# jurgisp/pydreamer

Measured on AMD Instinct MI355X. Metric: grad-steps/sec (world-model+AC) at B=50,T=50,H=15, 64×64 obs, 1/2/4/8 GPU, higher is better.
Workload: dtype f32; 1 GPU; atari-literal: defaults+atari, batch_size 50, batch_length 50, imag_horizon 15, deter_dim 600, stoch 32x32, hidden 1000, cnn_depth 48, action_dim 18, fp32; fwd + 4 bwd + clip + 4 AdamW per step; replay resident in HBM; global_batch=50, batch_length=50, imag_horizon=15, parallelism=dp1 (batch-sharded [50])

## Files before the change

### include/dreamer_hip.h

```cpp
#ifndef DREAMER_HIP_H
#define DREAMER_HIP_H

#include <stddef.h>
#include <stdint.h>

#ifdef __cplusplus
extern "C" {
#endif

#define DM_OK 0
#define DM_E_SHAPE (-1)
#define DM_E_WORKSPACE (-2)
#define DM_E_HIP (-3)
#define DM_E_DEVICE (-4)
#define DM_E_NULL (-5)

#define DM_MAX_MLP_LAYERS 8

typedef struct dm_shape {
  int32_t T, B, I;
  int32_t H;
  int32_t D, Hd;
  int32_t S, C;
  int32_t E;
// ... 45 lines not shown
int dm_rssm_lds_status(void);
int dm_rssm_lds_status_ack(void);
int dm_rssm_lds_gave_up(void);
int dm_rssm_lds_prof(unsigned long long* out16, int reset);

int dm_ln_elu_fwd(int rows, int n, const float* x, int ldx, const float* gamma, const float* beta, float eps,
                  float* y, int ldy, float* stats, void* stream);
int dm_ln_elu_bwd(int rows, int n, const float* x, int ldx, const float* y, int ldy, const float* stats,
                  const float* gamma, const float* dy, int lddy, float* dx, int lddx,
                  float* dgamma, float* dbeta, void* ws, size_t ws_bytes, void* stream);
int dm_colsum(int rows, int n, const float* x, int ld, float* out, void* ws, size_t ws_bytes, void* stream);

int dm_gru_gates_fwd(int rows, int D, const float* gi, const float* gh, const float* h_in, int ldh,
                     float* h_out, int ldo, void* stream);
int dm_gru_gates_bwd(int rows, int D, const float* gi, const float* gh, const float* h_in, int ldh,
                     const float* dh_out, int lddh, float* dgi, float* dgh, float* dh_in, int lddi, void* stream);

int dm_sample_onehot(int rows, int groups, int C, const float* logits, int ldl, const float* u,
                     const int32_t* forced_idx, float* onehot, int ldo, int32_t* idx, void* stream);

int dm_kl_balance_fwd(int rows, int S, int C, const float* post, const float* prior,
                      float* kl, float* ent_post, float* ent_prior, void* stream);
int dm_kl_balance_bwd(int rows, int S, int C, const float* post, const float* prior,
                      float scale_post, float scale_prior, float* dpost, float* dprior, void* stream);
int dm_kl_free_fwd(int rows, int S, int C, const float* post, const float* prior, float free, float* kl, float* kl_clip,
                   float* closed, float* ent_post, float* ent_prior, void* stream);
int dm_kl_free_bwd(int rows, int S, int C, const float* post, const float* prior, const float* closed, float scale_post,
                   float scale_prior, float* dpost, float* dprior, void* stream);
int dm_st_softmax_bwd(int rows, int groups, int C, const float* logits, int ldl, const float* dz, int lddz,
                      float* dlogits, int lddl, int accum, void* stream);

int dm_kl_sampled_fwd(int rows, int S, int C, const float* post, const float* prior, const int32_t* idx, float* out, void* stream);
int dm_kl_sampled_bwd(int rows, int S, int C, const float* post, const float* prior, const int32_t* idx, float scale,
                      const float* row_w, float* dpost, float* dprior, void* stream);
int dm_kl_sampled_gauss_fwd(int rows, int S, const float* post, const float* prior, const float* z, int ldz, float* out,
                            void* stream);
int dm_kl_sampled_gauss_bwd(int rows, int S, const float* post, const float* prior, const float* z, int ldz, float scale,
                            const float* row_w, float* dpost, float* dprior, float* dz, int lddz, void* stream);
int dm_reduce_i(int TB, int I, int W, const float* x, int mode, float* out, float* w_out, void* stream);
int dm_combine_rows(int count, int64_t n, const float* const* x, const float* w, float* out, void* stream);
int dm_scale_rows(int64_t rows, int n, float* x, int ldx, const float* w, float scale, void* stream);

int dm_mask_rows(int rows, int n, const float* x, int ldx, const uint8_t* reset, float* y, int ldy, void* stream);

int dm_im2col_s2(int n, int hb, int wb, int c, int k, const float* big, int big_nchw, float* col, void* stream);
#define DM_C2I_ELU 1
int dm_col2im_s2(int n, int hb, int wb, int c, int k, const float* col, const float* bias, int flags,
                 const float* elu_ref, float* big, void* stream);

typedef struct dm_mlp_params {
  const float* w[DM_MAX_MLP_LAYERS + 1];
  const float* b[DM_MAX_MLP_LAYERS + 1];
  const float* ln_g[DM_MAX_MLP_LAYERS];
  const float* ln_b[DM_MAX_MLP_LAYERS];
  int32_t precision;
  int32_t reserved_;
} dm_mlp_params;
typedef struct dm_mlp_grads {
  float* w[DM_MAX_MLP_LAYERS + 1];
  float* b[DM_MAX_MLP_LAYERS + 1];
  float* ln_g[DM_MAX_MLP_LAYERS];
  float* ln_b[DM_MAX_MLP_LAYERS];
} dm_mlp_grads;
size_t dm_mlp_acts_floats(int rows, int hidden, int layers);
size_t dm_mlp_ws_floats(int rows, int hidden, int layers);
int dm_mlp_plan_query(int which, int rows, int in_dim, int hidden, int layers, int out_dim, int ldx, int sparse_cols,
                      int base_align, int normed, int precision, int has_acts, int has_wpack, int has_add0, int has_sample,
                      size_t ws_bytes, int32_t out[8]);
int dm_mlp_head_fwd(int rows, int in_dim, int hidden, int layers, int out_dim,
                    const float* x, int ldx, const dm_mlp_params* p, float* acts, float* out,
                    void* ws, size_t ws_bytes, void* stream);
int dm_mlp_head_fwd_sparse(int rows, int in_dim, int sparse_cols, int hidden, int layers, int out_dim,
                           const float* x, int ldx, const dm_mlp_params* p, float* acts, float* out,
                           void* ws, size_t ws_bytes, void* stream);
int dm_mlp_head_fwd_rows(int rows_total, int row0, int rows, int in_dim, int sparse_cols, int hidden, int layers, int out_dim,
                         const float* x, int ldx, const dm_mlp_params* p, float* acts, float* out,
                         void* ws, size_t ws_bytes, void* stream);

int dm_mlp_head_bwd(int rows, int in_dim, int hidden, int layers, int out_dim,
                    const float* x, int ldx, const dm_mlp_params* p, const float* acts, const float* dout,
                    const dm_mlp_grads* g, float* dx, int lddx, int dx_accum,
                    void* ws, size_t ws_bytes, void* stream);

int dm_head_loss(int kind, int rows, const float* out, const float* target, float scale, float loss_const,
                 float* loss, float* dout, float* mean_out, void* stream);

int dm_head_loss_normal_nd(int rows, int V, const float* out, const float* target, float scale, float loss_const,
                           float* loss, float* dout, float* mean_out, void* stream);

int dm_head_loss_catsup(int rows, int I, int K, const float* logits, int ld, const float* support, const float* target, float scale,
                        float* loss, float* dlogits, float* mean_out, int32_t* bin, void* stream);

int dm_disag_reward(int K, int rows, int D, const float* means, int64_t head_stride, int ld, float scale, float* reward,
                    void* stream);
int dm_ensemble_mse(int K, int rows, int D, const float* means, int64_t head_stride, int ld, const float* target, int ldt,
                    const uint8_t* skip, float scale, float* loss, float* dmeans, void* stream);

int dm_cat_target_index(int rows, int C, int cells, const float* onehot, int32_t* idx, void* stream);
int dm_cat_image_loss(int rows, int I, int C, int cells, const float* logits, int ld, const int32_t* target, float* loss,
                      float* dlogits, void* stream);
int dm_cat_image_pred(int groups, int I, int C, int cells, const float* logits, int ld, const int32_t* target,
                      const int32_t* seen, float* logp, float* acc, float* acc_seen, void* stream);
int dm_cat_concat_rows(int rows, int I, int F, int E, const float* x, int ldx, const float* extra, float* out, void* stream);

int dm_dense_image_rows(int rows, int C, int cells, const float* image_f32, const int32_t* class_i32, const float* reward,
                        const float* terminal, float* out, int ldo, void* stream);
int dm_elu_rows_fwd(int rows, int n, const float* x, int ldx, float* y, int ldy, void* stream);
int dm_elu_rows_bwd(int rows, int n, const float* y, int ldy, const float* dy, int lddy, float* dx, int lddx, void* stream);
int dm_cat_image_loss_mix(int rows, int I, int C, int cells, const float* logits, int ld, const int32_t* target, float min_prob,
                          float* loss, float* dlogits, void* stream);

size_t dm_goals_stats_ws_floats(int rows, int G);
int dm_goals_stats(int rows, int G, const float* goals, const float* pred, const float* visage, float* out, void* ws,
                   size_t ws_bytes, void* stream);

int dm_preprocess_image_u8(int64_t n, int hw, int c, const uint8_t* src, float* dst, void* stream);

typedef struct dm_conv_params { const float* w[5]; const float* b[5]; } dm_conv_params;
typedef struct dm_conv_grads { float* w[5]; float* b[5]; } dm_conv_grads;
size_t dm_conv_encoder_acts_floats(const dm_shape* shp);
int dm_conv_encoder_fwd(const dm_shape* shp, const float* image , const dm_conv_params* p,
                        float* acts, float* embed , void* ws, size_t ws_bytes, void* stream);
int dm_conv_encoder_bwd(const dm_shape* shp, const float* image, const dm_conv_params* p, const float* acts,
                        const float* dembed, const dm_conv_grads* g, void* ws, size_t ws_bytes, void* stream);
int dm_conv_encoder_fwd_planes(const dm_shape* shp, const float* image, const dm_conv_params* p, const float* reward,
                               const float* terminal, float* acts, float* embed, int ld_embed, void* ws, size_t ws_bytes,
                               void* stream);
int dm_conv_encoder_bwd_planes(const dm_shape* shp, const float* image, const dm_conv_params* p, const float* reward,
                               const float* terminal, const float* acts, const float* dembed, int ld_dembed,
                               const dm_conv_grads* g, void* ws, size_t ws_bytes, void* stream);

size_t dm_conv_decoder_acts_floats(const dm_shape* shp);
size_t dm_conv_decoder_pred_offset(const dm_shape* shp);
int dm_conv_decoder_mse_fwd(const dm_shape* shp, const float* feat, int ldf, const float* target,
                            const dm_conv_params* p, float* acts, float* loss_image, float* image_rec ,
                            void* ws, size_t ws_bytes, void* stream);
int dm_conv_decoder_mse_bwd_rows(const dm_shape* shp, const float* feat, int ldf, const float* target,
                                 const dm_conv_params* p, const float* acts, float scale, const float* row_scale,
                                 const dm_conv_grads* g, float* dfeat, int lddf, void* ws, size_t ws_bytes, void* stream);
int dm_conv_decoder_mse_bwd(const dm_shape* shp, const float* feat, int ldf, const float* target,
                            const dm_conv_params* p, const float* acts, float scale,
                            const dm_conv_grads* g, float* dfeat, int lddf, void* ws, size_t ws_bytes, void* stream);

enum {
  DM_RSSM_Z_W = 0, DM_RSSM_Z_B, DM_RSSM_A_W, DM_RSSM_IN_G, DM_RSSM_IN_B,
  DM_RSSM_GRU_WIH, DM_RSSM_GRU_WHH, DM_RSSM_GRU_BIH, DM_RSSM_GRU_BHH,
  DM_RSSM_PRIOR_H_W, DM_RSSM_PRIOR_H_B, DM_RSSM_PRIOR_G, DM_RSSM_PRIOR_B, DM_RSSM_PRIOR_W, DM_RSSM_PRIOR_OB,
  DM_RSSM_POST_H_W, DM_RSSM_POST_H_B, DM_RSSM_POST_E_W, DM_RSSM_POST_G, DM_RSSM_POST_B, DM_RSSM_POST_W, DM_RSSM_POST_OB,
  DM_RSSM_GRU_LN_G0, DM_RSSM_GRU_LN_B0, DM_RSSM_GRU_LN_G1, DM_RSSM_GRU_LN_B1, DM_RSSM_GRU_LN_G2, DM_RSSM_GRU_LN_B2,
  DM_RSSM_GRU_L1_WIH, DM_RSSM_GRU_L1_WHH, DM_RSSM_GRU_L1_BIH, DM_RSSM_GRU_L1_BHH,
  DM_RSSM_GRU_L2_WIH, DM_RSSM_GRU_L2_WHH, DM_RSSM_GRU_L2_BIH, DM_RSSM_GRU_L2_BHH,
  DM_RSSM_GRU_L3_WIH, DM_RSSM_GRU_L3_WHH, DM_RSSM_GRU_L3_BIH, DM_RSSM_GRU_L3_BHH,
  DM_RSSM_GRU_L1_LN_G0, DM_RSSM_GRU_L1_LN_B0, DM_RSSM_GRU_L1_LN_G1, DM_RSSM_GRU_L1_LN_B1, DM_RSSM_GRU_L1_LN_G2, DM_RSSM_GRU_L1_LN_B2,
  DM_RSSM_GRU_L2_LN_G0, DM_RSSM_GRU_L2_LN_B0, DM_RSSM_GRU_L2_LN_G1, DM_RSSM_GRU_L2_LN_B1, DM_RSSM_GRU_L2_LN_G2, DM_RSSM_GRU_L2_LN_B2,
  DM_RSSM_GRU_L3_LN_G0, DM_RSSM_GRU_L3_LN_B0, DM_RSSM_GRU_L3_LN_G1, DM_RSSM_GRU_L3_LN_B1, DM_RSSM_GRU_L3_LN_G2, DM_RSSM_GRU_L3_LN_B2,
  DM_RSSM_NPARAMS
};
typedef struct dm_rssm_params { const float* p[DM_RSSM_NPARAMS]; } dm_rssm_params;
typedef struct dm_rssm_grads { float* p[DM_RSSM_NPARAMS]; } dm_rssm_grads;
size_t dm_rssm_acts_floats(const dm_shape* shp);
int dm_rssm_sequence_fwd(const dm_shape* shp, const float* embed, const float* action, const uint8_t* reset,
                         const float* h0, const float* z0, const float* u, const int32_t* forced_idx,
                         const dm_rssm_params* p, float* acts, float* feat, float* post, float* prior, int32_t* idx,
                         void* ws, size_t ws_bytes, void* stream);
int dm_rssm_sequence_bwd(const dm_shape* shp, const float* embed, const float* action, const uint8_t* reset,
                         const dm_rssm_params* p, const float* acts, const float* feat, const float* post,
                         float* dfeat, float* dpost, float* dprior,
                         const dm_rssm_grads* g, float* dembed, void* ws, size_t ws_bytes, void* stream);

#define DM_SCHED_FWD_FUSE_LN 1
#define DM_SCHED_FWD_FUSE_SAMPLE 2
#define DM_SCHED_FWD_FRAG 4
#define DM_SCHED_FWD_WZT 8
#define DM_SCHED_FWD_PSYNC 16
#define DM_SCHED_BWD_FUSE_B 1
#define DM_SCHED_BWD_FOLD 2
#define DM_SCHED_BWD_FOLD_SM 4
#define DM_SCHED_BWD_FRAG 8
#define DM_SCHED_BWD_NCHUNK_SHIFT 8
#define DM_SCHED_BWD_NCHUNK_MASK (15 << DM_SCHED_BWD_NCHUNK_SHIFT)
#define DM_SCHED_ROLL_WZT 1
#define DM_SCHED_ROLL_WAT 2
#define DM_SCHED_ROLL_ACTOR_WPACK 4
#define DM_SCHED_ROLL_ACTOR_ADD0 8
#define DM_SCHED_ROLL_FUSE_ACT 16
#define DM_SCHED_ROLL_TW_ON 32
int dm_rssm_last_schedule(int which);

typedef struct dm_gru_params { const float* w_ih; const float* w_hh; const float* b_ih; const float* b_hh; } dm_gru_params;
typedef struct dm_gru_grads { float* w_ih; float* w_hh; float* b_ih; float* b_hh; } dm_gru_grads;
size_t dm_gru_sequence_acts_floats(int T, int B, int In, int D);
size_t dm_gru_sequence_ws_bytes(int T, int B, int In, int D);
int dm_gru_sequence_fwd(int T, int B, int In, int D, const float* x, int ldx, const float* h0, const uint8_t* reset0,
                        const dm_gru_params* p, float* acts, float* H, int ldh, void* ws, size_t ws_bytes, void* stream);
int dm_gru_sequence_bwd(int T, int B, int In, int D, const float* x, int ldx, const dm_gru_params* p, const float* acts,
                        const float* H, int ldh, const float* dH, int lddh, const dm_gru_grads* g, float* dx, int lddx,
                        void* ws, size_t ws_bytes, void* stream);
int dm_gru_sequence_last_schedule(void);
int dm_gru_sequence_fuse_enable(int on);

int dm_dream_rollout_marks(int n, const int* steps, void* const* events);

int dm_dream_rollout(const dm_shape* shp, int M, const float* start, const dm_rssm_params* cell,
                     const dm_mlp_params* actor, const float* u_act, const float* u_prior,
                     float* feats, float* actions, int32_t* act_idx, float* actor_acts, float* actor_logits,
                     void* ws, size_t ws_bytes, void* stream);

int dm_gae_losses(int H, int M, float gamma, float lambda, const float* reward, const float* terminal,
                  const float* value_t, float* advantage, float* advantage_gae, float* value_target, float* weight,
                  void* stream);
int dm_actor_loss(int rows, int A, const float* logits, const int32_t* act_idx, const float* adv_gae,
                  const float* weight, float ent_w, float scale, float* loss, float* entropy, float* dlogits, void* stream);
int dm_sample_continuous(int kind, int rows, int A, const float* params, const float* eps, float* action, void* stream);
int dm_actor_loss_continuous(int kind, int rows, int A, const float* params, const float* actions, const float* adv_gae,
                             const float* weight, float ent_w, float scale, float* loss, float* entropy, float* dparams,
                             void* stream);
size_t dm_policy_draw_ws_floats(int rows);
int dm_policy_draw(int kind, int rows, int A, const float* params, int ldp, const float* noise, const float* value, float* action,
                   int lda, int32_t* act_idx, float* log_prob, float* entropy, float* stats, void* ws, size_t ws_bytes,
                   void* stream);
int dm_policy_draw_mode(int kind, int mode, float amount, int rows, int A, const float* params, int ldp, const float* noise,
                        const float* noise2, const float* value, float* action, int lda, int32_t* act_idx, float* log_prob,
                        float* entropy, float* stats, void* ws, size_t ws_bytes, void* stream);
int dm_cem_draw(int kind, int B, int J, int Hp, int A, const float* prop, const float* noise, float* actions, int32_t* act_idx,
                void* stream);
int dm_cem_update(int kind, int B, int J, int K, int Hp, int A, float gamma, const float* reward, const float* terminal,
                  const float* value, const float* actions, const int32_t* act_idx, const float* prop_in, float alpha, float floor,
                  float* prop_out, float* ret, int32_t* elite, float* first_action, float* stats, void* stream);
int dm_twohot_decode(int rows, int K, const float* logits, int ld, const float* bins, float* value, void* stream);
int dm_twohot_loss(int rows, int rows_total, int K, const float* logits, int ld, const float* bins, const float* target,
                   const float* weight, float scale, float* loss, float* dlogits, float* value, void* stream);
int dm_return_norm(int n, const float* x, float q_lo, float q_hi, float decay, float limit, int update, float* state, float* out,
                   float* adv, int n_adv, void* stream);
int dm_twohot_head_loss(int rows, int I, int K, const float* logits, int ld, const float* bins, const float* target, float scale,
                        float* loss, float* dlogits, float* mean, void* stream);
int dm_critic_loss(int rows, const float* value, const float* value_target, const float* weight, float scale,
                   float* loss, float* dvalue, void* stream);

typedef struct dm_reduce_item {
  const float* x; int64_t n; float scale;
  int32_t mode;
  const float* center;
} dm_reduce_item;
int dm_multi_sum(int count, const dm_reduce_item* items , float* out, void* stream);
int dm_combine(int count, const float* x, const float* w, float* out, void* stream);

int dm_multi_tensor_norm_clip(const float* grad, int64_t n, float max_norm, float* norm_out,
                              void* ws, size_t ws_bytes, void* stream);
int dm_scale_inplace(float* x, int64_t n, const float* coef, void* stream);
int dm_adamw_step(float* param, const float* grad, float* exp_avg, float* exp_avg_sq, int64_t n,
                  float lr, float beta1, float beta2, float eps, float weight_decay, int step,
                  const float* clip_coef, void* stream);
int dm_copy_params(float* dst, const float* src, int64_t n, void* stream);
int dm_mlp_chain_min_rows(int rows);
int dm_rollout_fuse_act_enable(int on);
int dm_prof_begin(int max_launches);
int dm_prof_end(double* out, int nkinds);
int dm_prof_rows(double* rows, int max_rows);
#define DM_REPLAY_MAX_FIELDS 16
typedef struct dm_replay_field {
  void* dst; int64_t row_bytes; int32_t is_reset; int32_t reserved_;
} dm_replay_field;
int dm_replay_gather(int T, int B, int nfields, const dm_replay_field* fields , const int32_t* pieces,
                     const void* const* src, void* stream);
int dm_axpby(int64_t n, float a, const float* x, float b, float* y, void* stream);

int dm_metric_accum(int n, const float* vals, const uint8_t* rules, double* sum, double* maxv, int64_t* count, void* stream);
int dm_batch_stats(int n, const float* reward, const uint8_t* reset, const float* terminal, float* out4, void* stream);
int dm_masked_mean(int T, int B, const float* x, int ldx, int take_rows, const uint8_t* col_keep, int skip_nan, float* out,
                   void* stream);
int dm_export_image_u8(int T, int B, int take_b, int C, int H, int W, const float* src, uint8_t* dst, void* stream);

#ifdef __cplusplus
}
#endif
#endif
```

### pydreamer_amd/csrc/common.h

```cpp
#pragma once
#include <hip/hip_runtime.h>
#include <stdint.h>
#include <stddef.h>
#include "dreamer_hip.h"

int dm_fail(int code, const char* fmt, ...);

#define DM_MAX_DEVICES 16

#define DM_LAUNCH_CHECK()                                                                      \
  do {                                                                                         \
    hipError_t e__ = hipGetLastError();                                                        \
    if (e__ != hipSuccess) return dm_fail(DM_E_HIP, "%s:%d: %s", __FILE__, __LINE__, hipGetErrorString(e__)); \
  } while (0)

#define DM_TRY(expr)                 \
  do {                               \
    int rc__ = (expr);               \
    if (rc__ != DM_OK) return rc__;  \
  } while (0)

#define DM_REQUIRE(cond, code, ...)                     \
  do {                                                  \
    if (!(cond)) return dm_fail(code, __VA_ARGS__);     \
// ... 134 lines not shown
                            const float* gamma, const float* dy, int lddy, float* dx, int lddx, hipStream_t st);
int dm_ln_elu_bwd_params_launch(int rows, int n, const float* x, int ldx, const float* y, int ldy, const float* stats,
                                const float* dy, int lddy, float* dgamma, float* dbeta, void* ws, size_t ws_bytes,
                                hipStream_t st);
int dm_gru_norm_fwd_launch(int kind, int rows, int D, const float* gi, const float* gh, const float* h_in, int ldh,
                           const float* const* ln_g, const float* const* ln_b, float* h_out, int ldo, float* gs, float* gst,
                           float* h_next, const uint8_t* next_reset, hipStream_t st, int ldg = 0, int ldst = 0, int ldn = 0);
int dm_gru_norm_bwd_launch(int kind, int rows, int D, const float* gh, const float* h_in, int ldh, const float* gs,
                           const float* gst, const float* const* ln_g, const float* const* ln_b, const float* dh_out, int lddh,
                           float* dgi, float* dgh, float* dg, float* dh_in, int lddi, const uint8_t* row_zero, hipStream_t st,
                           int ldg = 0, int ldst = 0);
int dm_gru_norm_param_grads_launch(int kind, int rows, int D, const float* gs, const float* gst, const float* dg, float* dgam,
                                   float* dbet, hipStream_t st, int ldg = 0, int ldst = 0);
int dm_gru_gates_fwd_launch(int rows, int D, const float* gi, const float* gh, const float* h_in, int ldh, float* h_out,
                            int ldo, float* h_next, const uint8_t* next_reset, float* h_frag, float* h_next_frag,
                            hipStream_t st, int ldg = 0, int ldn = 0);
int dm_gru_gates_bwd_launch(int rows, int D, const float* gi, const float* gh, const float* h_in, int ldh,
                            const float* dh_out, int lddh, float* dgi, float* dgh, float* dh_in, int lddi, int accum,
                            const uint8_t* row_zero, hipStream_t st, int ldg = 0);
int dm_sample_onehot_launch(int rows, int groups, int C, const float* logits, int ldl, const float* u,
                            const int32_t* forced, float* onehot, int ldo, int32_t* idx, float* z_next,
                            const uint8_t* next_reset, hipStream_t st);
int dm_gauss_sample_bwd_launch(int rows, int S, const float* par, int ldp, const float* z, int ldz, const float* dz,
                               int lddz, float* dpar, int lddp, int accum, hipStream_t st);
int dm_kl_fwd_launch(int rows, int S, int C, const float* post, const float* prior, float* kl, float* ep, float* eq,
                     hipStream_t st);
int dm_kl_bwd_launch(int rows, int S, int C, const float* post, const float* prior, float sp, float sq, float* dpost,
                     float* dprior, hipStream_t st);
int dm_st_softmax_bwd_launch(int rows, int groups, int C, const float* logits, int ldl, const float* dz, int lddz,
                             float* dlogits, int lddl, int accum, hipStream_t st);
int dm_mask_rows_launch(int rows, int n, const float* x, int ldx, const uint8_t* reset, float* y, int ldy, hipStream_t st);
int dm_mask_rows2_launch(int rows, int n1, const float* x1, int ldx1, float* y1, int ldy1, int n2, const float* x2,
                         int ldx2, float* y2, int ldy2, const uint8_t* reset, hipStream_t st);
int dm_sample_continuous_launch(int kind, int rows, int A, const float* params, const float* eps, float* action,
                                hipStream_t st);
int dm_mul_elu_grad_launch(size_t n, const float* dy, const float* yact, float* out, hipStream_t st);

int dm_im2col_s2_launch(int n, int hb, int wb, int c, int k, const float* big, int big_nchw, float* col, hipStream_t st);
int dm_col2im_s2_launch(int n, int hb, int wb, int c, int k, const float* col, const float* bias, int flags,
                        const float* elu_ref, float* big, hipStream_t st);
int dm_permute4_launch(const float* src, float* dst, int d0, int d1, int d2, int d3, int p0, int p1, int p2, int p3,
                       hipStream_t st);

bool dm_enc_l1_direct_ok(int ch, int d, int img);
int dm_enc_l1_fwd_launch(int frames, int d, int u8, const void* image, const float* w, const float* bias, float* wt, float* y,
                         unsigned short* y_h, hipStream_t st);
size_t dm_enc_l1_wgrad_part_floats(int frames, int d);
int dm_enc_l1_wgrad_launch(int frames, int d, int u8, const void* image, const float* G, float* part, float* dW, void* ws,
                           size_t ws_bytes, hipStream_t st);
int dm_enc_l1_fwd_planes_launch(int frames, int d, int u8, const void* image, const float* w5, const float* bias,
                                const float* reward, const float* terminal, float* wt, float* fb, float* y,
                                unsigned short* y_h, hipStream_t st);
size_t dm_enc_l1_planes_part_floats(int frames, int d);
int dm_enc_l1_planes_bwd_launch(int frames, int d, const float* G, const float* reward, const float* terminal,
                                const float* dw3, float* part, float* db, float* dW5, hipStream_t st);
bool dm_dec_l4_direct_ok(int ch, int d, int hs, int k);
size_t dm_dec_l4_w4_floats(int d);
int dm_dec_l4_fwd_launch(int frames, int d, const float* x, const float* w, const float* bias, float* w4, float* out,
                         hipStream_t st);
bool dm_dec_l4_bwd_direct_ok(int ch, int d, int hs, int k);
size_t dm_dec_l4_wp_floats(int d);
size_t dm_dec_l4_wgrad_part_floats(int frames, int d);
int dm_dec_l4_dgrad_launch(int frames, int d, const float* G4, const float* w, float* wp, const float* x3, float* dx,
                           unsigned short* dx_h, hipStream_t st);
int dm_dec_l4_wgrad_launch(int frames, int d, const float* G4, const float* x3, float* part, float* dW, void* ws,
                           size_t ws_bytes, hipStream_t st);

struct DmChainSample {
  const float* u;
  float* onehot;
  int ldo;
  int32_t* idx;
};
struct DmMlpFwd {
  int rows = 0, in_dim = 0, hidden = 0, layers = 0, out_dim = 0;
  const float* x = nullptr; int ldx = 0;
  const dm_mlp_params* p = nullptr;
  float* acts = nullptr; int acts_total_rows = 0, acts_row_off = 0;
  float* out = nullptr; int ldout = 0;
  int sparse_cols = 0;
  const float* wpack = nullptr;
  const float* add0 = nullptr;
  const DmChainSample* sample = nullptr;
};
enum { DM_MLP_PANEL = 0, DM_MLP_CHAIN = 1, DM_MLP_PER_LAYER = 2 };
int dm_mlp_fwd_launch(const DmMlpFwd& q, void* ws, size_t ws_bytes, hipStream_t st);
int dm_mlp_fwd_path(const DmMlpFwd& q, int* k0 = nullptr);

bool dm_panel_ok(int rows, int hidden);
int dm_panel_count(int rows);
int dm_panel_ln_fwd_launch(int rows, int hidden, int kin, const float* x, int ldx, const float* W, const float* b,
                           const float* gamma, const float* beta, float eps, float* xpre, float* stats, float* y,
                           const float* wout, const float* bout, float* out, int out_dim, int ldout, hipStream_t st,
                           const unsigned short* Wh = nullptr, int ldw = 0, const float* addm = nullptr);
int dm_panel_bf16_weights_launch(int count, const float* const* w, unsigned short* const* dst, const int* rows, const int* cols,
                                 int transpose, hipStream_t st);
int dm_panel_ln_bwd_launch(int rows, int hidden, int kup, const float* dup, int lddup, const float* W, const float* xpre,
                           const float* stats, const float* gamma, const float* beta, float* dx, float* colpart, float* wt,
                           hipStream_t st, const unsigned short* Wth = nullptr);
int dm_panel_colsum_final_launch(int count, const float* const* part, float* const* out, int n, int npanels, int pstride,
                                 hipStream_t st);

bool dm_mlp_chain_ok(int rows, int in_dim, int hidden, int layers, int out_dim, const float* x, int ldx,
                     const dm_mlp_params* p);
size_t dm_mlp_chain_pack_floats(int in_dim, int layers);
int dm_mlp_chain_pack_launch(int in_dim, int layers, const dm_mlp_params* p, float* wpack, hipStream_t st, int k0 = 0);
int dm_mlp_chain_fwd_launch(int rows, int in_dim, int layers, int out_dim, const float* x, int ldx, const dm_mlp_params* p,
                            float* const* xpre, float* const* stats, float* const* y, float* out, int ldout, const float* wpack,
                            hipStream_t st, int k0 = 0, const float* add0 = nullptr, const DmChainSample* sample = nullptr);
bool dm_mlp_chain_sparse_ok(int in_dim, int sparse_cols);

int dm_prof_slot_begin(int kind, double flops, double bytes, hipStream_t st);
void dm_prof_slot_end(int slot, hipStream_t st);
void dm_prof_slot_shape(int slot, int M, int N, int K, int nsplit, int flags);
extern "C" int dm_mlp_chain_min_rows(int rows);
bool dm_prof_active();

static const size_t DM_SPLITK_FLOATS = (size_t)16 * 1024 * 1024;
size_t dm_conv_ws_floats(const dm_shape* s, size_t parts[4] = nullptr);
size_t dm_rssm_ws_floats(const dm_shape* s, size_t parts[2] = nullptr);
size_t dm_rollout_ws_floats(const dm_shape* s);

typedef __bf16 bf16x8 __attribute__((ext_vector_type(8)));
typedef __bf16 bf16x2 __attribute__((ext_vector_type(2)));
typedef float dm_f32x2 __attribute__((ext_vector_type(2)));
__device__ __forceinline__ unsigned dm_pack_bf16x2(float lo, float hi) {
  const dm_f32x2 v = {lo, hi};
  return __builtin_bit_cast(unsigned, __builtin_convertvector(v, bf16x2));
}
__device__ __forceinline__ unsigned dm_f2bf(float x) { return dm_pack_bf16x2(x, 0.f) & 0xFFFFu; }
__device__ __forceinline__ uint2 dm_pack_bf16x4(float4 v) {
  return make_uint2(dm_pack_bf16x2(v.x, v.y), dm_pack_bf16x2(v.z, v.w));
}

__device__ __forceinline__ float dm_elu(float v) { return v > 0.f ? v : expm1f(v); }
__device__ __forceinline__ float dm_elu_grad_from_y(float y) { return y > 0.f ? 1.f : y + 1.f; }

__device__ __forceinline__ float dm_wave_sum(float v) {
#pragma unroll
  for (int off = 32; off > 0; off >>= 1) v += __shfl_xor(v, off, 64);
  return v;
}
__device__ __forceinline__ float dm_wave_max(float v) {
#pragma unroll
  for (int off = 32; off > 0; off >>= 1) v = fmaxf(v, __shfl_xor(v, off, 64));
  return v;
}
```

### pydreamer_amd/csrc/elementwise.hip

```cpp
#include "common.h"

template <bool CACHE>
__global__ void __launch_bounds__(256) ln_elu_fwd_kernel(int rows, int n, const float* __restrict__ x, int ldx,
                                                         const float* __restrict__ gamma, const float* __restrict__ beta,
                                                         float eps, float* __restrict__ y, int ldy, float* __restrict__ stats,
                                                         unsigned short* __restrict__ y_h) {
  const int row = blockIdx.x * 4 + (threadIdx.x >> 6);
  const int lane = threadIdx.x & 63;
  if (row >= rows) return;
  const float* xr = x + (size_t)row * ldx;
  unsigned short* yh = y_h ? y_h + (size_t)row * ldy : nullptr;
  float xc[16];
  float s = 0.f;
  if (CACHE) {
#pragma unroll
    for (int j = 0; j < 16; ++j) {
      const int c = lane + 64 * j;
      xc[j] = c < n ? xr[c] : 0.f;
      s += xc[j];
    }
  } else {
    for (int c = lane; c < n; c += 64) s += xr[c];
  }
  const float mean = dm_wave_sum(s) / (float)n;
// ... 566 lines not shown
      dgir[D + d] = ds_u; dghr[D + d] = ds_u;
    }
  }
}

__global__ void __launch_bounds__(256) gru_norm_param_grads_kernel(int kind, int rows, int D, const float* __restrict__ gs,
                                                                   const float* __restrict__ gst, const float* __restrict__ dg,
                                                                   float* __restrict__ dgam, float* __restrict__ dbet, int ldg,
                                                                   int ldst) {
  __shared__ float red[2][4][64];
  const int cx = threadIdx.x & 63, ry = threadIdx.x >> 6;
  const int col = blockIdx.x * 64 + cx;
  float a = 0.f, b = 0.f;
  if (col < 3 * D) {
    const int q = kind == 1 ? col / D : 0;
    for (int r = ry; r < rows; r += 4) {
      const float v = dg[(size_t)r * ldg + col];
      const float xh = (gs[(size_t)r * ldg + col] - gst[(size_t)r * ldst + 2 * q]) * gst[(size_t)r * ldst + 2 * q + 1];
      a += v * xh;
      b += v;
    }
  }
  red[0][ry][cx] = a; red[1][ry][cx] = b;
  __syncthreads();
  if (ry == 0 && col < 3 * D) {
    dgam[col] = (red[0][0][cx] + red[0][1][cx]) + (red[0][2][cx] + red[0][3][cx]);
    dbet[col] = (red[1][0][cx] + red[1][1][cx]) + (red[1][2][cx] + red[1][3][cx]);
  }
}

int dm_gru_norm_fwd_launch(int kind, int rows, int D, const float* gi, const float* gh, const float* h_in, int ldh,
                           const float* const* ln_g, const float* const* ln_b, float* h_out, int ldo, float* gs, float* gst,
                           float* h_next, const uint8_t* next_reset, hipStream_t st, int ldg, int ldst, int ldn) {
  if (rows <= 0) return DM_OK;
  if (ldg <= 0) ldg = 3 * D;
  if (ldst <= 0) ldst = 6;
  if (ldn <= 0) ldn = D;
  GruLnParams lp;
  for (int i = 0; i < 3; ++i) { lp.g[i] = ln_g[i]; lp.b[i] = ln_b[i]; }
  if (kind == 1)
    hipLaunchKernelGGL((gru_norm_fwd_kernel<1>), dim3(dm_cdiv(rows, 4)), dim3(256), 0, st, rows, D, gi, gh, h_in, ldh, lp, h_out,
                       ldo, gs, gst, h_next, next_reset, ldg, ldst, ldn);
  else
    hipLaunchKernelGGL((gru_norm_fwd_kernel<2>), dim3(dm_cdiv(rows, 4)), dim3(256), 0, st, rows, D, gi, gh, h_in, ldh, lp, h_out,
                       ldo, gs, gst, h_next, next_reset, ldg, ldst, ldn);
  DM_LAUNCH_CHECK();
  return DM_OK;
}
int dm_gru_norm_bwd_launch(int kind, int rows, int D, const float* gh, const float* h_in, int ldh, const float* gs,
                           const float* gst, const float* const* ln_g, const float* const* ln_b, const float* dh_out, int lddh,
                           float* dgi, float* dgh, float* dg, float* dh_in, int lddi, const uint8_t* row_zero, hipStream_t st,
                           int ldg, int ldst) {
  if (rows <= 0) return DM_OK;
  if (ldg <= 0) ldg = 3 * D;
  if (ldst <= 0) ldst = 6;
  GruLnParams lp;
  for (int i = 0; i < 3; ++i) { lp.g[i] = ln_g[i]; lp.b[i] = ln_b[i]; }
  if (kind == 1)
    hipLaunchKernelGGL((gru_norm_bwd_kernel<1>), dim3(dm_cdiv(rows, 4)), dim3(256), 0, st, rows, D, gh, h_in, ldh, gs, gst, lp,
                       dh_out, lddh, dgi, dgh, dg, dh_in, lddi, row_zero, ldg, ldst);
  else
    hipLaunchKernelGGL((gru_norm_bwd_kernel<2>), dim3(dm_cdiv(rows, 4)), dim3(256), 0, st, rows, D, gh, h_in, ldh, gs, gst, lp,
                       dh_out, lddh, dgi, dgh, dg, dh_in, lddi, row_zero, ldg, ldst);
  DM_LAUNCH_CHECK();
  return DM_OK;
}
int dm_gru_norm_param_grads_launch(int kind, int rows, int D, const float* gs, const float* gst, const float* dg, float* dgam,
                                   float* dbet, hipStream_t st, int ldg, int ldst) {
  if (ldg <= 0) ldg = 3 * D;
  if (ldst <= 0) ldst = 6;
  hipLaunchKernelGGL(gru_norm_param_grads_kernel, dim3(dm_cdiv(3 * D, 64)), dim3(256), 0, st, kind, rows, D, gs, gst, dg, dgam,
                     dbet, ldg, ldst);
  DM_LAUNCH_CHECK();
  return DM_OK;
}

static inline int ew_blocks(size_t total) {
  size_t b = (total + 255) / 256;
  if (b > 4096) b = 4096;
  if (b < 1) b = 1;
  return (int)b;
}

__global__ void __launch_bounds__(256) z_embed_kernel(int rows, int n, int S, int C, const int32_t* __restrict__ idx,
                                                      const uint8_t* __restrict__ row_zero, const float* __restrict__ Wt,
                                                      const float* __restrict__ bias, const float* __restrict__ add,
                                                      int ldadd, const int32_t* __restrict__ idx2,
                                                      const float* __restrict__ Wt2, float* __restrict__ x, int ldx,
                                                      float* __restrict__ x_frag,
                                                      const float* __restrict__ gamma, const float* __restrict__ beta,
                                                      float eps, float* __restrict__ y, int ldy,
                                                      unsigned short* __restrict__ y_h) {
  const int row = blockIdx.x * 4 + (threadIdx.x >> 6);
  const int lane = threadIdx.x & 63;
  if (row >= rows) return;
  float4 acc[4];
  bool in[4];
  int off[4];
#pragma unroll
  for (int j = 0; j < 4; ++j) {
    const int c = (lane + 64 * j) * 4;
    in[j] = c < n;
    off[j] = in[j] ? c : 0;
    acc[j] = bias ? *reinterpret_cast<const float4*>(bias + off[j]) : make_float4(0.f, 0.f, 0.f, 0.f);
  }
  if (add) {
#pragma unroll
    for (int j = 0; j < 4; ++j) {
      const float4 a = *reinterpret_cast<const float4*>(add + (size_t)row * ldadd + off[j]);
      acc[j].x += a.x; acc[j].y += a.y; acc[j].z += a.z; acc[j].w += a.w;
    }
  }
  if (idx2) {
    const float* wr = Wt2 + (size_t)idx2[row] * n;
#pragma unroll
    for (int j = 0; j < 4; ++j) {
      const float4 a = *reinterpret_cast<const float4*>(wr + off[j]);
      acc[j].x += a.x; acc[j].y += a.y; acc[j].z += a.z; acc[j].w += a.w;
    }
  }
  if (!(row_zero && row_zero[row])) {
    const int32_t* ir = idx + (size_t)row * S;
    for (int s0 = 0; s0 < S; s0 += 64) {
      const int mine = ir[min(s0 + lane, S - 1)];
      const int cnt = min(64, S - s0);
      int t = 0;
      for (; t + 8 <= cnt; t += 8) {
        float4 w[8][4];
#pragma unroll
        for (int u = 0; u < 8; ++u) {
          const float* wr = Wt + ((size_t)(s0 + t + u) * C + __shfl(mine, t + u, 64)) * n;
#pragma unroll
          for (int j = 0; j < 4; ++j) w[u][j] = *reinterpret_cast<const float4*>(wr + off[j]);
        }
        __builtin_amdgcn_sched_barrier(0);
#pragma unroll
        for (int u = 0; u < 8; ++u)
#pragma unroll
          for (int j = 0; j < 4; ++j) {
            acc[j].x += w[u][j].x; acc[j].y += w[u][j].y; acc[j].z += w[u][j].z; acc[j].w += w[u][j].w;
          }
      }
      for (; t < cnt; ++t) {
        const float* wr = Wt + ((size_t)(s0 + t) * C + __shfl(mine, t, 64)) * n;
#pragma unroll
        for (int j = 0; j < 4; ++j) {
          const float4 w = *reinterpret_cast<const float4*>(wr + off[j]);
          acc[j].x += w.x; acc[j].y += w.y; acc[j].z += w.z; acc[j].w += w.w;
        }
      }
    }
  }
#pragma unroll
  for (int j = 0; j < 4; ++j)
    if (in[j]) {
      const int c = (lane + 64 * j) * 4;
      if (x) *reinterpret_cast<float4*>(x + (size_t)row * ldx + c) = acc[j];
      if (x_frag) *reinterpret_cast<float4*>(x_frag + dm_frag_off(row, c)) = acc[j];
    }
  if (!y) return;
  if (!gamma) {
#pragma unroll
    for (int j = 0; j < 4; ++j)
      if (in[j]) {
        float4 o;
        o.x = dm_elu(acc[j].x); o.y = dm_elu(acc[j].y); o.z = dm_elu(acc[j].z); o.w = dm_elu(acc[j].w);
        *reinterpret_cast<float4*>(y + (size_t)row * ldy + (lane + 64 * j) * 4) = o;
      }
    return;
  }
  float s1 = 0.f;
#pragma unroll
  for (int j = 0; j < 4; ++j)
    if (in[j]) s1 += (acc[j].x + acc[j].y) + (acc[j].z + acc[j].w);
  const float mean = dm_wave_sum(s1) / (float)n;
  float s2 = 0.f;
#pragma unroll
  for (int j = 0; j < 4; ++j)
    if (in[j]) {
      const float dx = acc[j].x - mean, dy = acc[j].y - mean, dz = acc[j].z - mean, dw = acc[j].w - mean;
      s2 += (dx * dx + dy * dy) + (dz * dz + dw * dw);
    }
  const float rstd = 1.0f / sqrtf(dm_wave_sum(s2) / (float)n + eps);
#pragma unroll
  for (int j = 0; j < 4; ++j)
    if (in[j]) {
      const int c = (lane + 64 * j) * 4;
      const float4 g = *reinterpret_cast<const float4*>(gamma + c), b = *reinterpret_cast<const float4*>(beta + c);
      float4 o;
      o.x = dm_elu((acc[j].x - mean) * rstd * g.x + b.x);
      o.y = dm_elu((acc[j].y - mean) * rstd * g.y + b.y);
      o.z = dm_elu((acc[j].z - mean) * rstd * g.z + b.z);
      o.w = dm_elu((acc[j].w - mean) * rstd * g.w + b.w);
      *reinterpret_cast<float4*>(y + (size_t)row * ldy + c) = o;
      if (y_h) *reinterpret_cast<uint2*>(y_h + (size_t)row * ldy + c) = dm_pack_bf16x4(o);
    }
}
template <int NJ>
__global__ void __launch_bounds__(256) sparse_rows_kernel(int rows, int n, int Zc, const float* __restrict__ z, int ldz,
                                                          const float* __restrict__ Wt, float* __restrict__ x, int ldx) {
  const int row = blockIdx.x * 4 + (threadIdx.x >> 6);
  const int lane = threadIdx.x & 63;
  if (row >= rows) return;
  float4 acc[NJ];
  int off[NJ];
#pragma unroll
  for (int j = 0; j < NJ; ++j) {
    const int c = (lane + 64 * j) * 4;
    off[j] = c < n ? c : 0;
    acc[j] = make_float4(0.f, 0.f, 0.f, 0.f);
  }
  const float* zr = z + (size_t)row * ldz;
  for (int e0 = 0; e0 < Zc; e0 += 256) {
    float v[4];
    unsigned long long m[4];
#pragma unroll
    for (int u = 0; u < 4; ++u) v[u] = zr[min(e0 + 64 * u + lane, Zc - 1)];
#pragma unroll
    for (int u = 0; u < 4; ++u) m[u] = __ballot(e0 + 64 * u + lane < Zc && v[u] != 0.f);
#pragma unroll
    for (int u = 0; u < 4; ++u) {
      unsigned long long mm = m[u];
      while (mm) {
        const int b = __builtin_ctzll(mm);
        mm &= mm - 1;
        const float ze = __shfl(v[u], b, 64);
        const float* wr = Wt + (size_t)(e0 + 64 * u + b) * n;
#pragma unroll
        for (int j = 0; j < NJ; ++j) {
          const float4 w = *reinterpret_cast<const float4*>(wr + off[j]);
          acc[j].x += ze * w.x; acc[j].y += ze * w.y; acc[j].z += ze * w.z; acc[j].w += ze * w.w;
        }
      }
    }
  }
#pragma unroll
  for (int j = 0; j < NJ; ++j) {
    const int c = (lane + 64 * j) * 4;
    if (c < n) *reinterpret_cast<float4*>(x + (size_t)row * ldx + c) = acc[j];
  }
}
int dm_sparse_rows_launch(int rows, int n, int Zc, const float* z, int ldz, const float* Wt, float* x, int ldx,
                          hipStream_t st) {
  if (rows <= 0) return DM_OK;
  DM_REQUIRE(n >= 4 && n <= 1024 && (n & 3) == 0 && (ldx & 3) == 0 && Zc >= 1, DM_E_SHAPE, "sparse_rows: n=%d Zc=%d", n, Zc);
  const dim3 grid(dm_cdiv(rows, 4)), blk(256);
  if (n <= 256) hipLaunchKernelGGL((sparse_rows_kernel<1>), grid, blk, 0, st, rows, n, Zc, z, ldz, Wt, x, ldx);
  else if (n <= 512) hipLaunchKernelGGL((sparse_rows_kernel<2>), grid, blk, 0, st, rows, n, Zc, z, ldz, Wt, x, ldx);
  else hipLaunchKernelGGL((sparse_rows_kernel<4>), grid, blk, 0, st, rows, n, Zc, z, ldz, Wt, x, ldx);
  DM_LAUNCH_CHECK();
  return DM_OK;
}

bool dm_z_embed_ok(int n) { return n <= 1024 && (n & 3) == 0; }
__global__ void __launch_bounds__(256) z_embed_wide_kernel(int n, int S, int C, const int32_t* __restrict__ idx,
                                                           const uint8_t* __restrict__ row_zero, const float* __restrict__ Wt,
                                                           const float* __restrict__ bias, const float* __restrict__ add, int ldadd,
                                                           const int32_t* __restrict__ idx2, const float* __restrict__ Wt2,
                                                           float* __restrict__ x, int ldx, float* __restrict__ x_frag) {
  const int row = blockIdx.x;
  const int lane = threadIdx.x & 63;
  const int c = threadIdx.x * 4;
  const bool in = c < n;
  const int off = in ? c : 0;
  float4 acc = bias ? *reinterpret_cast<const float4*>(bias + off) : make_float4(0.f, 0.f, 0.f, 0.f);
  if (add) {
    const float4 a = *reinterpret_cast<const float4*>(add + (size_t)row * ldadd + off);
    acc.x += a.x; acc.y += a.y; acc.z += a.z; acc.w += a.w;
// ... 23 lines not shown

__global__ void __launch_bounds__(256) z_embed_wide_ln_kernel(int n, int S, int C, const int32_t* __restrict__ idx,
                                                              const uint8_t* __restrict__ row_zero, const float* __restrict__ Wt,
                                                              const float* __restrict__ bias, const float* __restrict__ add, int ldadd,
                                                              const int32_t* __restrict__ idx2, const float* __restrict__ Wt2,
                                                              float* __restrict__ x, int ldx, const float* __restrict__ gamma,
                                                              const float* __restrict__ beta, float eps, float* __restrict__ y, int ldy,
                                                              float* __restrict__ y_frag, float* __restrict__ stats) {
  __shared__ float red[8];
  const int row = blockIdx.x;
  const int lane = threadIdx.x & 63, wave = threadIdx.x >> 6;
  const int c = threadIdx.x * 4;
  const bool in = c < n;
  const int off = in ? c : 0;
  float4 acc = bias ? *reinterpret_cast<const float4*>(bias + off) : make_float4(0.f, 0.f, 0.f, 0.f);
  if (add) {
    const float4 a = *reinterpret_cast<const float4*>(add + (size_t)row * ldadd + off);
    acc.x += a.x; acc.y += a.y; acc.z += a.z; acc.w += a.w;
  }
  if (idx2) {
    const float4 a = *reinterpret_cast<const float4*>(Wt2 + (size_t)idx2[row] * n + off);
    acc.x += a.x; acc.y += a.y; acc.z += a.z; acc.w += a.w;
  }
  if (!(row_zero && row_zero[row])) {
    const int mine = idx[(size_t)row * S + min(lane, S - 1)];
    float4 w[32];
#pragma unroll
    for (int s = 0; s < 32; ++s) {
      const int sc = s < S ? s : S - 1;
      w[s] = *reinterpret_cast<const float4*>(Wt + ((size_t)sc * C + __shfl(mine, sc, 64)) * n + off);
    }
    __builtin_amdgcn_sched_barrier(0);
#pragma unroll
    for (int s = 0; s < 32; ++s)
      if (s < S) { acc.x += w[s].x; acc.y += w[s].y; acc.z += w[s].z; acc.w += w[s].w; }
  }
  if (in && x) *reinterpret_cast<float4*>(x + (size_t)row * ldx + c) = acc;
  const float s1 = dm_wave_sum(in ? (acc.x + acc.y) + (acc.z + acc.w) : 0.f);
  if (lane == 0) red[wave] = s1;
  __syncthreads();
  const float mean = ((red[0] + red[1]) + (red[2] + red[3])) / (float)n;
  const float4 d = make_float4(acc.x - mean, acc.y - mean, acc.z - mean, acc.w - mean);
  const float s2 = dm_wave_sum(in ? (d.x * d.x + d.y * d.y) + (d.z * d.z + d.w * d.w) : 0.f);
  if (lane == 0) red[4 + wave] = s2;
  __syncthreads();
  const float rstd = 1.0f / sqrtf(((red[4] + red[5]) + (red[6] + red[7])) / (float)n + eps);
  if (stats && threadIdx.x == 0) { stats[2 * (size_t)row] = mean; stats[2 * (size_t)row + 1] = rstd; }
  if (in) {
    const float4 ga = make_float4(gamma[c], gamma[c + 1], gamma[c + 2], gamma[c + 3]);
    const float4 be = make_float4(beta[c], beta[c + 1], beta[c + 2], beta[c + 3]);
    const float4 o = make_float4(dm_elu(d.x * rstd * ga.x + be.x), dm_elu(d.y * rstd * ga.y + be.y), dm_elu(d.z * rstd * ga.z + be.z),
                                 dm_elu(d.w * rstd * ga.w + be.w));
    if (y) *reinterpret_cast<float4*>(y + (size_t)row * ldy + c) = o;
    if (y_frag) *reinterpret_cast<float4*>(y_frag + dm_frag_off(row, c)) = o;
  }
}

int dm_z_embed_launch(int rows, int n, int S, int C, const int32_t* idx, const uint8_t* row_zero, const float* Wt,
                      const float* bias, const float* add, int ldadd, const int32_t* idx2, const float* Wt2, float* x, int ldx,
                      float* x_frag, const float* gamma, const float* beta, float eps, float* y, int ldy, hipStream_t st,
                      float* y_frag, float* stats) {
  if (rows <= 0) return DM_OK;
  DM_REQUIRE(!idx2 || Wt2, DM_E_NULL, "z_embed: second index list without its table");
  DM_REQUIRE(dm_z_embed_ok(n) && idx && Wt && (x || y), DM_E_SHAPE, "z_embed: n=%d needs n <= 1024, n %% 4 == 0", n);
  DM_REQUIRE((ldx & 3) == 0 && (ldy & 3) == 0 && (ldadd & 3) == 0, DM_E_SHAPE, "z_embed: leading dims must be multiples of 4");
  DM_REQUIRE(!x_frag || rows <= 64, DM_E_SHAPE, "z_embed: the fragment-major copy needs rows <= 64");
  DM_REQUIRE(!y || (gamma != nullptr) == (beta != nullptr), DM_E_NULL, "z_embed: LayerNorm gain without its bias");
  if (!y && x && rows <= 64 && S <= 32) {
    hipLaunchKernelGGL(z_embed_wide_kernel, dim3(rows), dim3(256), 0, st, n, S, C, idx, row_zero, Wt, bias, add, ldadd, idx2, Wt2, x,
                       ldx, x_frag);
    DM_LAUNCH_CHECK();
    return DM_OK;
  }
  if (y_frag) {
    DM_REQUIRE(y && gamma && beta && rows <= 64 && S <= 32 && !x_frag, DM_E_SHAPE,
               "z_embed: the row-per-workgroup LayerNorm form needs y, gamma / beta, rows <= 64, S <= 32");
    hipLaunchKernelGGL(z_embed_wide_ln_kernel, dim3(rows), dim3(256), 0, st, n, S, C, idx, row_zero, Wt, bias, add, ldadd, idx2, Wt2, x,
                       ldx, gamma, beta, eps, y, ldy, y_frag, stats);
    DM_LAUNCH_CHECK();
    return DM_OK;
  }
  unsigned short* y_h = (y && gamma) ? dm_twin_of(y, false) : nullptr;
  if (y_h) dm_twin_mark(y);
  hipLaunchKernelGGL(z_embed_kernel, dim3(dm_cdiv(rows, 4)), dim3(256), 0, st, rows, n, S, C, idx, row_zero, Wt, bias, add,
                     ldadd, idx2, Wt2, x, ldx, x_frag, gamma, beta, eps, y, ldy, y_h);
  DM_LAUNCH_CHECK();
  return DM_OK;
}

int dm_frag_pack_launch(int rows, int K, const float* X, int ldx, float* Xf, hipStream_t st) {
  DM_REQUIRE(rows >= 0 && rows <= 64 && K >= 1 && X && Xf, DM_E_SHAPE, "frag_pack: rows %d (<= 64), K %d", rows, K);
  if (rows == 0) return DM_OK;
  hipLaunchKernelGGL(frag_pack_kernel, dim3(ew_blocks((size_t)rows * K)), dim3(256), 0, st, rows, K, X, ldx, Xf);
  DM_LAUNCH_CHECK();
  return DM_OK;
}
int dm_gru_gates_fwd_launch(int rows, int D, const float* gi, const float* gh, const float* h_in, int ldh, float* h_out,
                            int ldo, float* h_next, const uint8_t* next_reset, float* h_frag, float* h_next_frag,
                            hipStream_t st, int ldg, int ldn) {
  if (rows <= 0) return DM_OK;
  DM_REQUIRE((!h_frag && !h_next_frag) || rows <= 64, DM_E_SHAPE, "gru_gates_fwd: fragment-major copies need rows <= 64");
  unsigned short* h_out_h = dm_twin_of(h_out, false);
  if (h_out_h) dm_twin_mark(h_out);
  hipLaunchKernelGGL(gru_gates_fwd_kernel, dim3(ew_blocks((size_t)rows * D)), dim3(256), 0, st, rows, D, gi, gh, h_in,
                     ldh, h_out, ldo, h_next, next_reset, h_frag, h_next_frag, ldg > 0 ? ldg : 3 * D, ldn > 0 ? ldn : D, h_out_h);
  DM_LAUNCH_CHECK();
  return DM_OK;
}
int dm_gru_gates_bwd_launch(int rows, int D, const float* gi, const float* gh, const float* h_in, int ldh,
                            const float* dh_out, int lddh, float* dgi, float* dgh, float* dh_in, int lddi, int accum,
                            const uint8_t* row_zero, hipStream_t st, int ldg) {
  if (rows <= 0) return DM_OK;
  hipLaunchKernelGGL(gru_gates_bwd_kernel, dim3(ew_blocks((size_t)rows * D)), dim3(256), 0, st, rows, D, gi, gh, h_in,
                     ldh, dh_out, lddh, dgi, dgh, dh_in, lddi, accum, row_zero, ldg > 0 ? ldg : 3 * D);
  DM_LAUNCH_CHECK();
  return DM_OK;
}
extern "C" int dm_gru_gates_fwd(int rows, int D, const float* gi, const float* gh, const float* h_in, int ldh,
                                float* h_out, int ldo, void* stream) {
  DM_REQUIRE(gi && gh && h_in && h_out, DM_E_NULL, "gru_gates_fwd: null pointer");
  return dm_gru_gates_fwd_launch(rows, D, gi, gh, h_in, ldh, h_out, ldo, nullptr, nullptr, nullptr, nullptr,
                                 (hipStream_t)stream);
}
extern "C" int dm_gru_gates_bwd(int rows, int D, const float* gi, const float* gh, const float* h_in, int ldh,
                                const float* dh_out, int lddh, float* dgi, float* dgh, float* dh_in, int lddi,
                                void* stream) {
  DM_REQUIRE(gi && gh && h_in && dh_out && dgi && dgh && dh_in, DM_E_NULL, "gru_gates_bwd: null pointer");
  return dm_gru_gates_bwd_launch(rows, D, gi, gh, h_in, ldh, dh_out, lddh, dgi, dgh, dh_in, lddi, 0, nullptr,
                                 (hipStream_t)stream);
}

__global__ void __launch_bounds__(256) sample_onehot_kernel(int rows, int groups, int C, const float* __restrict__ logits,
                                                            int ldl, const float* __restrict__ u,
                                                            const int32_t* __restrict__ forced, float* __restrict__ onehot,
                                                            int ldo, int32_t* __restrict__ idx_out) {
  const int total = rows * groups;
  for (int i = blockIdx.x * 256 + threadIdx.x; i < total; i += gridDim.x * 256) {
    const int r = i / groups, gq = i % groups;
    const float* x = logits + (size_t)r * ldl + (size_t)gq * C;
    int idx;
    if (forced) {
      idx = forced[i];
    } else {
      float mx = x[0];
      for (int k = 1; k < C; ++k) mx = fmaxf(mx, x[k]);
      float sum = 0.f;
      for (int k = 0; k < C; ++k) sum += expf(x[k] - mx);
      float total_p = 0.f;
      for (int k = 0; k < C; ++k) total_p += expf(x[k] - mx) / sum;
      const float target = u[i] * total_p;
      float cdf = 0.f;
      idx = 0;
      for (int k = 0; k < C; ++k) {
        cdf += expf(x[k] - mx) / sum;
        idx += (cdf <= target) ? 1 : 0;
      }
      if (idx > C - 1) idx = C - 1;
    }
    float* o = onehot + (size_t)r * ldo + (size_t)gq * C;
    for (int k = 0; k < C; ++k) o[k] = (k == idx) ? 1.f : 0.f;
    if (idx_out) idx_out[i] = idx;
  }
}

template <int LPG>
__global__ void __launch_bounds__(256) sample_onehot_wave_kernel(int rows, int groups, int C,
                                                                 const float* __restrict__ logits, int ldl,
                                                                 const float* __restrict__ u,
// ... 1166 lines not shown
```

### pydreamer_amd/csrc/mlp.hip

```cpp
#include "common.h"

static bool al16(const void* p) { return ((uintptr_t)p & 15) == 0; }
static const size_t MLP_SKB = DM_SPLITK_FLOATS * sizeof(float);

struct MlpActs {
  float* xpre[DM_MAX_MLP_LAYERS];
  float* stats[DM_MAX_MLP_LAYERS];
  float* y[DM_MAX_MLP_LAYERS];
};
static size_t mlp_carve(int rows, int hidden, int layers, float* base, MlpActs* a) {
  DmArena ar(base, (size_t)1 << 62);
  for (int l = 0; l < layers; ++l) {
    float* xp = ar.take((size_t)rows * hidden);
    float* st = ar.take((size_t)rows * 2);
    float* yy = ar.take((size_t)rows * hidden);
    if (a) { a->xpre[l] = xp; a->stats[l] = st; a->y[l] = yy; }
  }
  return ar.off;
}
extern "C" size_t dm_mlp_acts_floats(int rows, int hidden, int layers) {
  if (rows < 0 || hidden < 0 || layers < 0 || layers > DM_MAX_MLP_LAYERS) return 0;
  return mlp_carve(rows, hidden, layers, nullptr, nullptr);
}

static size_t mlp_ws_floats(int rows, int hidden, int layers) {
  const size_t rh = dm_align_up((size_t)rows * hidden, 64);
  return DM_SPLITK_FLOATS + 3 * rh + dm_align_up((size_t)layers * dm_panel_count(rows) * 3 * hidden, 64) +
         dm_align_up((size_t)hidden * hidden, 64) + 256 +
         dm_align_up((size_t)hidden * 2048 + (size_t)layers * hidden * hidden / 2 + 64, 64) +
         rh + dm_align_up((size_t)hidden * 4096, 64);
}
extern "C" size_t dm_mlp_ws_floats(int rows, int hidden, int layers) {
  if (rows < 0 || hidden < 0 || layers < 0 || layers > DM_MAX_MLP_LAYERS) return 0;
  return mlp_ws_floats(rows, hidden, layers);
}

enum { MLP_ADD_NONE = 0, MLP_ADD_HERE = 1, MLP_ADD_CALLER = 2 };
struct MlpFwdPlan {
  int path;
  int k0;
  int addend;
  bool pack_here;
  bool bf16_copies;
  bool fuse_out;
  bool normed;
  size_t need_floats;
};
struct MlpFwdWs {
  float *splitk, *t0, *t1, *t2, *stats, *g, *w0t;
  unsigned short* wh[DM_MAX_MLP_LAYERS];
};
static size_t mlp_fwd_layout(DmArena ar, const DmMlpFwd& q, bool bf16_copies, bool addend, MlpFwdWs* w) {
  const size_t rh = (size_t)q.rows * q.hidden;
  *w = {};
  w->splitk = ar.take(DM_SPLITK_FLOATS);
  w->t0 = ar.take(rh); w->t1 = ar.take(rh); w->t2 = ar.take(rh); w->stats = ar.take((size_t)q.rows * 2);
  for (int l = 0; l < q.layers && bf16_copies; ++l)
    w->wh[l] = (unsigned short*)ar.take(dm_half_floats((size_t)q.hidden * (l == 0 ? q.in_dim : q.hidden)));
  if (addend) { w->g = ar.take(rh); w->w0t = ar.take((size_t)q.in_dim * q.hidden); }
  return ar.off;
}

static int mlp_fwd_plan(const DmMlpFwd& q, const void* ws, size_t ws_bytes, MlpFwdPlan* out) {
  const dm_mlp_params* p = q.p;
  DM_REQUIRE(q.layers >= 1 && q.layers <= DM_MAX_MLP_LAYERS, DM_E_SHAPE, "mlp: layers=%d", q.layers);
  DM_REQUIRE(q.sparse_cols >= 0 && q.sparse_cols < q.in_dim, DM_E_SHAPE, "mlp: sparse_cols=%d of in_dim=%d", q.sparse_cols, q.in_dim);
  DM_REQUIRE(!q.add0 || q.wpack, DM_E_NULL, "mlp_fwd: a caller's sparse addend comes with the weights the caller packed for it");
  DM_REQUIRE(ws_bytes >= MLP_SKB, DM_E_WORKSPACE, "mlp_fwd: workspace too small");
  const size_t cap = ws_bytes / sizeof(float);
  MlpFwdWs sized;
  MlpFwdPlan pl = {};
  pl.need_floats = q.acts ? DM_SPLITK_FLOATS : mlp_fwd_layout(DmArena(nullptr, 0), q, false, false, &sized);
  DM_REQUIRE(pl.need_floats <= cap, DM_E_WORKSPACE,
             "mlp_fwd: workspace too small for the activation ping-pong (need %zu floats)", pl.need_floats);
  pl.normed = p->ln_g[0] != nullptr;
  for (int l = 0; l < q.layers; ++l)
    DM_REQUIRE((p->ln_g[l] != nullptr) == pl.normed && (p->ln_b[l] != nullptr) == pl.normed, DM_E_NULL,
               "mlp: layer %d mixes LayerNorm and NoNorm parameters", l);
  const bool split_ok = dm_mlp_chain_sparse_ok(q.in_dim, q.sparse_cols);
  const int dense = q.in_dim - q.sparse_cols;
  bool want_copies = false, want_addend = false;
  pl.k0 = q.in_dim;
  if (pl.normed && dm_panel_ok(q.rows, q.hidden) && (q.in_dim & 3) == 0 && al16(p->w[0])) {
    pl.path = DM_MLP_PANEL;
    pl.fuse_out = q.out_dim <= 32;
    want_copies = dm_cur_precision() && q.in_dim <= 4096 && (q.in_dim & 7) == 0;
    want_addend = split_ok && (q.ldx & 3) == 0;
  } else if (dm_mlp_chain_ok(q.rows, q.in_dim, q.hidden, q.layers, q.out_dim, q.x, q.ldx, p)) {
    pl.path = DM_MLP_CHAIN;
    if (q.wpack) {
      if (q.add0 && split_ok) { pl.addend = MLP_ADD_CALLER; pl.k0 = dense; }
    } else if (dm_mlp_chain_pack_floats(q.in_dim, q.layers) <= DM_SPLITK_FLOATS && al16(ws)) {
      pl.pack_here = true;
      want_addend = split_ok;
    }
  } else {
    pl.path = DM_MLP_PER_LAYER;
  }
  DM_REQUIRE(!q.sample || pl.path == DM_MLP_CHAIN, DM_E_SHAPE,
             "mlp_fwd: the fused sampler rides in the whole-MLP kernel only (rows %d)", q.rows);
  if (want_copies || want_addend) {
    const size_t full = mlp_fwd_layout(DmArena(nullptr, 0), q, want_copies, want_addend, &sized);
    if (full <= cap) {
      pl.need_floats = full;
      pl.bf16_copies = want_copies;
      if (want_addend) { pl.addend = MLP_ADD_HERE; pl.k0 = dense; }
    }
  }
  *out = pl;
  return DM_OK;
}

int dm_mlp_fwd_path(const DmMlpFwd& q, int* k0) {
  MlpFwdPlan pl;
  DM_TRY(mlp_fwd_plan(q, nullptr, ~(size_t)0, &pl));
  if (k0) *k0 = pl.k0;
  return pl.path;
}

struct MlpFwdCtx {
  const DmMlpFwd& q;
  MlpFwdPlan pl;
  MlpFwdWs w;
  MlpActs a;
  hipStream_t st;
};

static int mlp_sparse_addend(const MlpFwdCtx& c) {
  const DmMlpFwd& q = c.q;
  DM_TRY(dm_permute4_launch(q.p->w[0], c.w.w0t, 1, 1, q.hidden, q.in_dim, 0, 1, 3, 2, c.st));
  return dm_sparse_rows_launch(q.rows, q.hidden, q.sparse_cols, q.x + c.pl.k0, q.ldx, c.w.w0t + (size_t)c.pl.k0 * q.hidden,
                               c.w.g, q.hidden, c.st);
}

static int mlp_out_layer(const MlpFwdCtx& c, const float* in) {
  const DmMlpFwd& q = c.q;
  DmGemm g;
  g.M = q.rows; g.N = q.out_dim; g.K = q.hidden;
  g.A = in; g.lda = q.hidden;
  g.B = q.p->w[q.layers]; g.ldb = q.hidden;
  g.C = q.out; g.ldc = q.ldout;
  g.bias = q.p->b[q.layers];
  return dm_gemm_launch(g, c.w.splitk, MLP_SKB, c.st);
}

static int mlp_fwd_chain(const MlpFwdCtx& c) {
  const DmMlpFwd& q = c.q;
  const float* wpack = q.wpack;
  const float* add0 = c.pl.addend == MLP_ADD_CALLER ? q.add0 : nullptr;
  if (c.pl.addend == MLP_ADD_HERE) {
    DM_TRY(mlp_sparse_addend(c));
    add0 = c.w.g;
  }
  if (c.pl.pack_here) {
    DM_TRY(dm_mlp_chain_pack_launch(q.in_dim, q.layers, q.p, c.w.splitk, c.st, c.pl.k0));
    wpack = c.w.splitk;
  }
  return dm_mlp_chain_fwd_launch(q.rows, q.in_dim, q.layers, q.out_dim, q.x, q.ldx, q.p, q.acts ? c.a.xpre : nullptr,
                                 q.acts ? c.a.stats : nullptr, q.acts ? c.a.y : nullptr, q.out, q.ldout, wpack, c.st, c.pl.k0,
                                 add0, q.sample);
}

static int mlp_fwd_panel(const MlpFwdCtx& c) {
  const DmMlpFwd& q = c.q;
  const dm_mlp_params* p = q.p;
  const int layers = q.layers;
  if (c.pl.bf16_copies) {
    const float* src[DM_MAX_MLP_LAYERS];
    int rws[DM_MAX_MLP_LAYERS], cls[DM_MAX_MLP_LAYERS];
    for (int l = 0; l < layers; ++l) { src[l] = p->w[l]; rws[l] = q.hidden; cls[l] = l == 0 ? q.in_dim : q.hidden; }
    DM_TRY(dm_panel_bf16_weights_launch(layers, src, c.w.wh, rws, cls, 0, c.st));
  }
  if (c.pl.addend == MLP_ADD_HERE) DM_TRY(mlp_sparse_addend(c));
  const float* in = q.x;
  int ldin = q.ldx, kin = c.pl.k0;
  for (int l = 0; l < layers; ++l) {
    const bool fo = l == layers - 1 && c.pl.fuse_out;
    DM_TRY(dm_panel_ln_fwd_launch(q.rows, q.hidden, kin, in, ldin, p->w[l], p->b[l], p->ln_g[l], p->ln_b[l], 1e-3f,
                                  q.acts ? c.a.xpre[l] : nullptr, q.acts ? c.a.stats[l] : nullptr,
                                  (fo && !q.acts) ? nullptr : c.a.y[l], fo ? p->w[layers] : nullptr,
                                  fo ? p->b[layers] : nullptr, q.out, q.out_dim, q.ldout, c.st, c.w.wh[l], l == 0 ? q.in_dim : 0,
                                  l == 0 ? c.w.g : nullptr));
    in = c.a.y[l]; ldin = q.hidden; kin = q.hidden;
  }
  return c.pl.fuse_out ? DM_OK : mlp_out_layer(c, in);
}

static int mlp_fwd_layers(const MlpFwdCtx& c) {
  const DmMlpFwd& q = c.q;
  const dm_mlp_params* p = q.p;
  const float* in = q.x;
  int ldin = q.ldx, kin = q.in_dim;
  for (int l = 0; l < q.layers; ++l) {
    DmGemm g;
    g.M = q.rows; g.N = q.hidden; g.K = kin;
    g.A = in; g.lda = ldin;
    g.B = p->w[l]; g.ldb = kin;
    g.C = c.a.xpre[l]; g.ldc = q.hidden;
    g.bias = p->b[l];
    DM_TRY(dm_gemm_launch(g, c.w.splitk, MLP_SKB, c.st));
    if (c.pl.normed)
      DM_TRY(dm_ln_elu_fwd_launch(q.rows, q.hidden, c.a.xpre[l], q.hidden, p->ln_g[l], p->ln_b[l], 1e-3f, c.a.y[l], q.hidden,
                                  c.a.stats[l], c.st));
    else DM_TRY(dm_elu_fwd_launch(q.rows, q.hidden, c.a.xpre[l], q.hidden, c.a.y[l], q.hidden, c.st));
    in = c.a.y[l]; ldin = q.hidden; kin = q.hidden;
  }
  return mlp_out_layer(c, in);
}

int dm_mlp_fwd_launch(const DmMlpFwd& q, void* ws, size_t ws_bytes, hipStream_t st) {
  MlpFwdCtx c = {q, {}, {}, {}, st};
  DM_TRY(mlp_fwd_plan(q, ws, ws_bytes, &c.pl));
  mlp_fwd_layout(DmArena(ws, ws_bytes), q, c.pl.bf16_copies, c.pl.addend == MLP_ADD_HERE, &c.w);
  if (q.acts) {
    DM_REQUIRE(q.acts_row_off >= 0 && q.acts_row_off + q.rows <= q.acts_total_rows, DM_E_SHAPE, "mlp_fwd: acts row window");
    mlp_carve(q.acts_total_rows, q.hidden, q.layers, q.acts, &c.a);
    for (int l = 0; l < q.layers; ++l) {
      c.a.xpre[l] += (size_t)q.acts_row_off * q.hidden;
      c.a.stats[l] += (size_t)q.acts_row_off * 2;
      c.a.y[l] += (size_t)q.acts_row_off * q.hidden;
    }
  } else {
    for (int l = 0; l < q.layers; ++l) { c.a.xpre[l] = c.w.t2; c.a.stats[l] = c.w.stats; c.a.y[l] = (l & 1) ? c.w.t1 : c.w.t0; }
  }
  switch (c.pl.path) {
    case DM_MLP_PANEL: return mlp_fwd_panel(c);
    case DM_MLP_CHAIN: return mlp_fwd_chain(c);
    default: return mlp_fwd_layers(c);
  }
}

static int mlp_head_fwd(int rows_total, int row0, int rows, int in_dim, int sparse_cols, int hidden, int layers, int out_dim,
                        const float* x, int ldx, const dm_mlp_params* p, float* acts, float* out, void* ws, size_t ws_bytes,
                        void* stream) {
  DmPrecisionScope prec(p->precision);
  DmMlpFwd q;
  q.rows = rows; q.in_dim = in_dim; q.hidden = hidden; q.layers = layers; q.out_dim = out_dim;
  q.x = x + (size_t)row0 * ldx; q.ldx = ldx; q.p = p;
  q.acts = acts; q.acts_total_rows = rows_total; q.acts_row_off = row0;
  q.out = out + (size_t)row0 * out_dim; q.ldout = out_dim;
  q.sparse_cols = sparse_cols;
  return dm_mlp_fwd_launch(q, ws, ws_bytes, (hipStream_t)stream);
}

extern "C" int dm_mlp_head_fwd(int rows, int in_dim, int hidden, int layers, int out_dim, const float* x, int ldx,
                               const dm_mlp_params* p, float* acts, float* out, void* ws, size_t ws_bytes, void* stream) {
  DM_REQUIRE(x && p && out && ws, DM_E_NULL, "mlp_head_fwd: null pointer");
  return mlp_head_fwd(rows, 0, rows, in_dim, 0, hidden, layers, out_dim, x, ldx, p, acts, out, ws, ws_bytes, stream);
}

extern "C" int dm_mlp_head_fwd_sparse(int rows, int in_dim, int sparse_cols, int hidden, int layers, int out_dim,
                                      const float* x, int ldx, const dm_mlp_params* p, float* acts, float* out, void* ws,
                                      size_t ws_bytes, void* stream) {
  DM_REQUIRE(x && p && out && ws, DM_E_NULL, "mlp_head_fwd_sparse: null pointer");
  return mlp_head_fwd(rows, 0, rows, in_dim, sparse_cols, hidden, layers, out_dim, x, ldx, p, acts, out, ws, ws_bytes, stream);
}

extern "C" int dm_mlp_head_fwd_rows(int rows_total, int row0, int rows, int in_dim, int sparse_cols, int hidden, int layers,
                                    int out_dim, const float* x, int ldx, const dm_mlp_params* p, float* acts, float* out,
                                    void* ws, size_t ws_bytes, void* stream) {
  DM_REQUIRE(x && p && out && ws, DM_E_NULL, "mlp_head_fwd_rows: null pointer");
  DM_REQUIRE(row0 >= 0 && rows >= 1 && row0 + rows <= rows_total, DM_E_SHAPE, "mlp_head_fwd_rows: window [%d, %d) of %d rows", row0,
             row0 + rows, rows_total);
  return mlp_head_fwd(rows_total, row0, rows, in_dim, sparse_cols, hidden, layers, out_dim, x, ldx, p, acts, out, ws, ws_bytes,
                      stream);
}

struct MlpBwdPlan {
  int path;
  bool normed;
  bool bf16;
  bool bf16_copies;
  size_t need_floats;
};
struct MlpBwdWs {
  float *splitk, *dy, *dxp, *colpart, *wt;
  unsigned short* wth[DM_MAX_MLP_LAYERS];
};
static size_t mlp_bwd_layout(DmArena ar, int rows, int hidden, int layers, const MlpBwdPlan& pl, MlpBwdWs* w) {
  const bool panel = pl.path == DM_MLP_PANEL;
  *w = {};
  w->splitk = ar.take(DM_SPLITK_FLOATS);
  w->dy = ar.take((size_t)rows * hidden); w->dxp = ar.take((size_t)rows * hidden);
  w->colpart = ar.take(panel ? (size_t)layers * dm_panel_count(rows) * 3 * hidden : 0);
  if (pl.bf16) w->wt = ar.take((size_t)hidden * hidden);
  for (int l = 1; l < layers && pl.bf16_copies; ++l) w->wth[l - 1] = (unsigned short*)ar.take(dm_half_floats((size_t)hidden * hidden));
  return ar.off;
}
static int mlp_bwd_plan(int rows, int hidden, int layers, const dm_mlp_params* p, size_t ws_bytes, MlpBwdPlan* out) {
  DM_REQUIRE(layers >= 1 && layers <= DM_MAX_MLP_LAYERS, DM_E_SHAPE, "mlp: layers=%d", layers);
  const size_t cap = ws_bytes / sizeof(float);
  MlpBwdWs sized;
  MlpBwdPlan pl = {};
  pl.normed = p->ln_g[0] != nullptr;
  pl.path = pl.normed && dm_panel_ok(rows, hidden) && al16(p->w[layers]) ? DM_MLP_PANEL : DM_MLP_PER_LAYER;
  pl.bf16 = pl.path == DM_MLP_PANEL && dm_cur_precision();
  pl.need_floats = mlp_bwd_layout(DmArena(nullptr, 0), rows, hidden, layers, pl, &sized);
  DM_REQUIRE(pl.need_floats <= cap, DM_E_WORKSPACE, "mlp_head_bwd: workspace too small (need %zu floats)", pl.need_floats);
  if (pl.bf16 && (hidden & 7) == 0 && layers > 1) {
    pl.bf16_copies = true;
    const size_t full = mlp_bwd_layout(DmArena(nullptr, 0), rows, hidden, layers, pl, &sized);
    if (full <= cap) pl.need_floats = full;
    else pl.bf16_copies = false;
  }
  *out = pl;
  return DM_OK;
}

struct MlpBwdCtx {
  int rows, in_dim, hidden, layers, out_dim;
  const float* x; int ldx;
  const dm_mlp_params* p; const float* dout; const dm_mlp_grads* g;
  float* dx; int lddx, dx_accum;
  hipStream_t st;
  MlpBwdPlan pl;
  MlpBwdWs w;
  MlpActs a;
};
static int mlp_wgrad(const MlpBwdCtx& c, int n_out, int n_in, const float* dy, const float* in, int ldin, float* dW) {
  DmGemm g;
  g.a_layout = 1; g.b_layout = 1;
  g.M = n_out; g.N = n_in; g.K = c.rows;
  g.A = dy; g.lda = n_out;
  g.B = in; g.ldb = ldin;
  g.C = dW; g.ldc = n_in;
  return dm_gemm_launch(g, c.w.splitk, MLP_SKB, c.st);
}
static int mlp_dgrad(const MlpBwdCtx& c, int n_out, int n_in, const float* dy, const float* W, float* din, int ldd, int accum = 0) {
  DmGemm g;
  g.a_layout = 0; g.b_layout = 1;
  g.M = c.rows; g.N = n_in; g.K = n_out;
  g.A = dy; g.lda = n_out;
  g.B = W; g.ldb = n_in;
  g.C = din; g.ldc = ldd; g.flags = accum ? DM_GEMM_ACCUM : 0;
  return dm_gemm_launch(g, c.w.splitk, MLP_SKB, c.st);
}
static int mlp_bwd_out_params(const MlpBwdCtx& c) {
  DM_TRY(mlp_wgrad(c, c.out_dim, c.hidden, c.dout, c.a.y[c.layers - 1], c.hidden, c.g->w[c.layers]));
  return dm_colsum_launch(c.rows, c.out_dim, c.dout, c.out_dim, c.g->b[c.layers], c.w.splitk, MLP_SKB, c.st);
}

static int mlp_bwd_panel(const MlpBwdCtx& c) {
  const dm_mlp_params* p = c.p;
  const int rows = c.rows, hidden = c.hidden, layers = c.layers, npanels = dm_panel_count(rows);
  const size_t cstride = (size_t)npanels * 3 * hidden;
  if (c.pl.bf16_copies) {
    const float* src[DM_MAX_MLP_LAYERS];
    int rws[DM_MAX_MLP_LAYERS], cls[DM_MAX_MLP_LAYERS];
// ... 102 lines not shown
```

### pydreamer_amd/csrc/rssm.hip

```cpp
#include "common.h"

static inline int rssm_gru_kind(const dm_shape* s) { return (s->flags & DM_FLAG_GRU_MASK) >> DM_FLAG_GRU_SHIFT; }
static inline int rssm_gru_layers(const dm_shape* s) {
  return 1 + ((s->flags & DM_FLAG_GRU_LAYERS_MASK) >> DM_FLAG_GRU_LAYERS_SHIFT);
}
struct RssmDims {
  int T, B, N, D, Hd, S, C, Z, ZP, F, E, A, kind, layers;
  bool gauss;
};
static void rssm_dims(const dm_shape* s, RssmDims* d) {
  d->T = s->T; d->B = s->B; d->N = s->T * s->B; d->D = s->D; d->Hd = s->Hd; d->S = s->S; d->C = s->C;
  d->Z = s->S * (s->C ? s->C : 1); d->ZP = s->S * (s->C ? s->C : 2); d->F = d->D + d->Z; d->E = s->E; d->A = s->A;
  d->gauss = s->C == 0; d->kind = rssm_gru_kind(s); d->layers = rssm_gru_layers(s);
}

struct RssmActs {
  float *ea, *ee, *hin, *zin, *x1, *st1, *za, *gi, *gh, *x2, *st2, *pin, *x3, *st3, *prin;
  float *gs, *gst;
};
static size_t rssm_carve(const RssmDims& d, float* base, RssmActs* a) {
  const size_t N = (size_t)d.T * d.B, Hd = d.Hd, D = d.D, Z = d.Z;
  DmArena ar(base, (size_t)1 << 62);
  RssmActs t;
  t.ea = ar.take(N * Hd); t.ee = ar.take(N * Hd);
// ... 610 lines not shown
                                    void* ws, size_t ws_bytes, void* stream) {
  DM_REQUIRE(s && embed && action && reset && P && acts && feat && post && dfeat && dpost && dprior && G && ws, DM_E_NULL,
             "rssm_sequence_bwd: null pointer");
  DmPrecisionScope prec(s->flags & DM_FLAG_BF16);
  DM_TRY(rssm_check(s));
  BpttCtx c = {};
  rssm_dims(s, &c);
  rssm_carve(c, const_cast<float*>(acts), &c.a);
  c.p = P->p; c.g = G->p; c.st = (hipStream_t)stream; c.sw = dm_wgrad_side_stream(c.st);
  c.embed = embed; c.action = action; c.feat = feat; c.post = post; c.reset = reset; c.dfeat = dfeat; c.dpost = dpost;
  DM_TRY(gru_stack(s, c.p, c.g, &c.gk));
  DM_TRY(c.plan(ws, ws_bytes));
  tl_last_schedule[1] = (c.fuse_b ? DM_SCHED_BWD_FUSE_B : 0) | (c.fold ? DM_SCHED_BWD_FOLD : 0) | (c.fold_sm ? DM_SCHED_BWD_FOLD_SM : 0) |
                        (c.dgif ? DM_SCHED_BWD_FRAG : 0) | (c.nchunk << DM_SCHED_BWD_NCHUNK_SHIFT);
  const RssmActs& a = c.a;
  const float* const* p = c.p;
  float* const* g = c.g;
  const int N = c.N, D = c.D, Hd = c.Hd, Z = c.Z, ZP = c.ZP, F = c.F;
  hipStream_t st = c.st, sw = c.sw;
  float *sk = c.sk, *sk_w = c.sk_w;
  const size_t skb = c.skb;

  DM_TRY(dgrad(st, sk, skb, N, ZP, Hd, dprior, ZP, p[DM_RSSM_PRIOR_W], c.dprin, Hd, 0, nullptr));
  DM_TRY(norm_elu_bwd_dx(N, Hd, a.x3, Hd, a.prin, Hd, a.st3, p[DM_RSSM_PRIOR_G], c.dprin, Hd, c.dx3, Hd, st));
  DM_TRY(dgrad(st, sk, skb, N, Hd, D, c.dx3, Hd, p[DM_RSSM_PRIOR_H_W], dfeat, F, 1, nullptr));
  DM_TRY(dm_wgrad_side_fork(st, sw));
  DM_TRY(wgrad(sw, sk_w, skb, N, ZP, Hd, dprior, ZP, a.prin, Hd, g[DM_RSSM_PRIOR_W]));
  DM_TRY(dm_colsum_launch(N, ZP, dprior, ZP, g[DM_RSSM_PRIOR_OB], sk_w, skb, sw));
  DM_TRY(norm_elu_bwd_params(N, Hd, a.x3, Hd, a.prin, Hd, a.st3, c.dprin, Hd, g[DM_RSSM_PRIOR_G], g[DM_RSSM_PRIOR_B], sk_w, skb, sw));
  DM_TRY(wgrad(sw, sk_w, skb, N, Hd, D, c.dx3, Hd, feat, F, g[DM_RSSM_PRIOR_H_W]));
  DM_TRY(dm_colsum_launch(N, Hd, c.dx3, Hd, g[DM_RSSM_PRIOR_H_B], sk_w, skb, sw));

  DM_TRY(transpose(st, p[DM_RSSM_POST_W], c.wt_post, ZP, Hd));
  DM_TRY(transpose(st, p[DM_RSSM_POST_H_W], c.wt_post_h, Hd, D));
  if (c.gk.L == 1) {
    DM_TRY(transpose(st, p[DM_RSSM_GRU_WIH], c.wt_ih, 3 * D, Hd));
    DM_TRY(transpose(st, p[DM_RSSM_GRU_WHH], c.wt_hh, 3 * D, D));
  }
  DM_TRY(transpose(st, p[DM_RSSM_Z_W], c.wt_z, Hd, Z));
  if (c.fold) {
    DM_TRY(dgrad(st, sk, skb, N, Hd, D, a.x2, Hd, p[DM_RSSM_POST_H_W], c.xw2, D, 0, nullptr));
    DM_TRY(dgrad(st, sk, skb, N, Hd, Z, a.x1, Hd, p[DM_RSSM_Z_W], c.xwz, Z, 0, nullptr));
    DM_TRY(dm_colsum_launch(Hd, D, p[DM_RSSM_POST_H_W], D, c.cs2, sk, skb, st));
    DM_TRY(dm_colsum_launch(Hd, Z, p[DM_RSSM_Z_W], Z, c.csz, sk, skb, st));
  }
  for (int t = c.T - 1; t >= 0; --t) {
    DM_TRY(c.fuse_b ? c.bptt_step_fused(t) : c.gk.L > 1 ? c.bptt_step_stacked(t) : c.bptt_step_single(t));
    DM_TRY(c.side_chunk(t));
  }
  if (c.fuse_b) DM_TRY(c.post_norm_bwd(0, N, c.dx2, st));
  if (dembed) DM_TRY(dgrad(st, sk, skb, N, Hd, c.E, c.dx2, Hd, p[DM_RSSM_POST_E_W], dembed, c.E, 0, nullptr));
  return c.param_tail();
}

static thread_local int tl_marks_n = 0;
static thread_local int tl_mark_step[4];
static thread_local hipEvent_t tl_mark_ev[4];
extern "C" int dm_dream_rollout_marks(int n, const int* steps, void* const* events) {
  DM_REQUIRE(n >= 0 && n <= 4 && (n == 0 || (steps && events)), DM_E_SHAPE, "dream_rollout_marks: n=%d (0..4)", n);
  for (int i = 0; i < n; ++i) {
    DM_REQUIRE(events[i], DM_E_NULL, "dream_rollout_marks: null event %d", i);
    tl_mark_step[i] = steps[i];
    tl_mark_ev[i] = (hipEvent_t)events[i];
  }
  tl_marks_n = n;
  return DM_OK;
}
struct DmRolloutMarks {
  int n;
  bool done[4] = {false, false, false, false};
  hipStream_t caller;
  explicit DmRolloutMarks(hipStream_t st) : n(tl_marks_n), caller(st) { tl_marks_n = 0; }
  void at_step(int i, hipStream_t st, bool eager) {
    if (!eager) return;
    for (int k = 0; k < n; ++k)
      if (!done[k] && tl_mark_step[k] == i) { (void)hipEventRecord(tl_mark_ev[k], st); done[k] = true; }
  }
  ~DmRolloutMarks() {
    for (int k = 0; k < n; ++k)
      if (!done[k]) (void)hipEventRecord(tl_mark_ev[k], caller);
  }
};

static int g_rollout_fuse_act = 1;
extern "C" int dm_rollout_fuse_act_enable(int on) {
  if (on >= 0) g_rollout_fuse_act = on ? 1 : 0;
  return g_rollout_fuse_act;
}

struct RolloutDims : RssmDims {
  int M, H, Hm, L, adist, AO;
};
struct RolloutWs {
  float *sk, *macts, *logits_ws, *ea, *x1, *za, *stats, *gi, *gh, *prior, *gsw, *gstw;
  unsigned short *wih_h, *whh_h, *wph_h, *wp_h, *za_h, *feats_h;
  size_t must;
  float *wzt, *wat; int32_t *pidx, *aidx;
  float *actor_wpack, *actor_w0t, *actor_add0;
};
static size_t rollout_layout(DmArena ar, const RolloutDims& d, bool keep_acts, bool tw_on, bool want_z, bool want_pack,
                             bool want_add0, RolloutWs* w) {
  const size_t M = d.M, D = d.D, Hd = d.Hd, ZP = d.ZP, F = d.F;
  *w = {};
  w->sk = ar.take(DM_SPLITK_FLOATS);
  w->macts = ar.take(keep_acts ? 0 : dm_mlp_acts_floats(d.M, d.Hm, d.L)); w->logits_ws = ar.take(keep_acts ? 0 : M * d.AO);
  w->ea = ar.take(M * Hd); w->x1 = ar.take(M * Hd); w->za = ar.take(M * Hd); w->stats = ar.take(M * 2);
  w->gi = ar.take(M * 3 * D); w->gh = ar.take(M * 3 * D); w->prior = ar.take(M * ZP);
  w->gsw = ar.take(d.kind ? M * 3 * D : 0); w->gstw = ar.take(d.kind ? M * 6 * d.layers : 0);
  w->wih_h = (unsigned short*)ar.take(tw_on ? dm_half_floats(3 * D * Hd) : 0);
  w->whh_h = (unsigned short*)ar.take(tw_on ? dm_half_floats(3 * D * D) : 0);
  w->wph_h = (unsigned short*)ar.take(tw_on ? dm_half_floats(Hd * D) : 0);
  w->wp_h = (unsigned short*)ar.take(tw_on ? dm_half_floats(ZP * Hd) : 0);
  w->za_h = (unsigned short*)ar.take(tw_on ? dm_half_floats(M * Hd) : 0);
  w->feats_h = (unsigned short*)ar.take(tw_on ? dm_half_floats((size_t)(d.H + 1) * M * F) : 0);
  w->must = ar.off;
  if (want_z) {
    const size_t mark = ar.off;
    w->wzt = ar.take((size_t)d.Z * Hd);
    w->wat = ar.take((size_t)d.A * Hd);
    w->pidx = reinterpret_cast<int32_t*>(ar.take(M * d.S));
    w->aidx = reinterpret_cast<int32_t*>(ar.take(M));
    want_z = ar.fits();
    if (!want_z) { w->wzt = nullptr; w->pidx = nullptr; ar.give_back(mark); }
    if (!want_z || d.adist != 0) { w->wat = nullptr; w->aidx = nullptr; }
  }
  if (want_pack) {
    w->actor_wpack = ar.take(dm_mlp_chain_pack_floats(d.F, d.L));
    if (ar.fits() && want_z && want_add0) {
      const size_t mark = ar.off;
      w->actor_w0t = ar.take(F * d.Hm);
      w->actor_add0 = ar.take(M * d.Hm);
      if (!ar.fits()) { w->actor_w0t = w->actor_add0 = nullptr; ar.give_back(mark); }
    }
  }
  return ar.off;
}

struct RolloutCtx : RolloutDims, RolloutWs {
  GruStack gk;
  const float* const* p; const dm_mlp_params* actor; hipStream_t st; size_t skb;
  const float *u_act, *u_prior; float *feats, *actions; int32_t* act_idx; float *actor_acts, *actor_logits;
  bool tw_on;
  bool fuse_act;

  int plan(void* ws, size_t ws_bytes) {
    tw_on = dm_twins_on() && kind == 0 && layers == 1 && p[DM_RSSM_IN_G] && p[DM_RSSM_PRIOR_G] && (F & 7) == 0;
    skb = DM_SPLITK_FLOATS * sizeof(float);
    const bool chain = dm_mlp_fwd_path(actor_call(0)) == DM_MLP_CHAIN;
    rollout_layout(DmArena(ws, ws_bytes), *this, actor_acts != nullptr, tw_on, C != 0 && H > 1 && dm_z_embed_ok(Hd), chain,
                   C != 0 && dm_z_embed_ok(Hm), this);
    DM_REQUIRE(must <= ws_bytes / sizeof(float), DM_E_WORKSPACE, "dream_rollout: workspace too small (need %zu floats)", must);
    if (actor_add0) {
      int k0 = F;
      dm_mlp_fwd_path(actor_call(0), &k0);
      if (k0 == F) actor_w0t = actor_add0 = nullptr;
    }
    fuse_act = adist == 0 && actor_wpack && g_rollout_fuse_act;
    return DM_OK;
  }

  int32_t* act_idx_of(int i) const { return act_idx ? act_idx + (size_t)i * M : aidx; }

  DmMlpFwd actor_call(int i) const {
    const bool keep = actor_acts != nullptr;
    DmMlpFwd q;
    q.rows = M; q.in_dim = F; q.hidden = Hm; q.layers = L; q.out_dim = AO;
    q.x = feats + (size_t)i * M * F; q.ldx = F; q.p = actor;
    q.acts = keep ? actor_acts : macts; q.acts_total_rows = keep ? H * M : M; q.acts_row_off = keep ? i * M : 0;
    q.out = keep ? actor_logits + (size_t)i * M * AO : logits_ws; q.ldout = AO;
    q.wpack = actor_wpack; q.add0 = actor_add0; q.sparse_cols = actor_add0 ? Z : 0;
    return q;
  }
  int rollout_actor(int i) const {
    const float* cur = feats + (size_t)i * M * F;
    float* act = actions + (size_t)i * M * A;
    if (actor_add0) {
      if (i == 0) DM_TRY(dm_sparse_rows_launch(M, Hm, Z, cur + D, F, actor_w0t + (size_t)D * Hm, actor_add0, Hm, st));
      else DM_TRY(dm_z_embed_launch(M, Hm, S, C, pidx, nullptr, actor_w0t + (size_t)D * Hm, nullptr, nullptr, 0, nullptr, nullptr,
                                    actor_add0, Hm, nullptr, nullptr, nullptr, 0.f, nullptr, 0, st));
    }
    int32_t* ai = act_idx_of(i);
    const DmChainSample samp = {u_act + (size_t)i * M, act, A, ai};
    DmMlpFwd q = actor_call(i);
    if (fuse_act) q.sample = &samp;
    const float* logits = q.out;
    DM_TRY(dm_mlp_fwd_launch(q, sk, skb, st));
    if (fuse_act) return DM_OK;
    if (adist == 0)
      return dm_sample_onehot_launch(M, 1, A, logits, A, u_act + (size_t)i * M, nullptr, act, A, ai, nullptr, nullptr, st);
    return dm_sample_continuous_launch(adist, M, A, logits, u_act + (size_t)i * M * A, act, st);
  }
  int rollout_cell(int i) const {
    const float* cur = feats + (size_t)i * M * F;
    float* nxt = feats + (size_t)(i + 1) * M * F;
    const float* act = actions + (size_t)i * M * A;
    const int32_t* ai = act_idx_of(i);
    const bool embed = wzt && i > 0, embed_a = embed && wat && ai;
    if (!embed_a) DM_TRY(linear(st, sk, skb, M, Hd, A, act, A, p[DM_RSSM_A_W], nullptr, nullptr, 0, ea, Hd));
    if (embed) {
      DM_TRY(dm_z_embed_launch(M, Hd, S, C, pidx, nullptr, wzt, p[DM_RSSM_Z_B], embed_a ? nullptr : ea, Hd,
                               embed_a ? ai : nullptr, wat, nullptr, Hd, nullptr, p[DM_RSSM_IN_G], p[DM_RSSM_IN_B], 1e-3f,
                               za, Hd, st));
    } else {
      DM_TRY(linear(st, sk, skb, M, Hd, Z, cur + D, F, p[DM_RSSM_Z_W], p[DM_RSSM_Z_B], ea, Hd, x1, Hd));
      DM_TRY(norm_elu_fwd(M, Hd, x1, Hd, p[DM_RSSM_IN_G], p[DM_RSSM_IN_B], 1e-3f, za, Hd, stats, st));
    }
    if (gk.L > 1) {
      DM_TRY(gru_stack_fwd(st, sk, skb, gk, M, Hd, D, za, cur, F, gi, gh, nxt, F, nullptr, nullptr, gsw, gstw));
    } else {
      DM_TRY(linear(st, sk, skb, M, 3 * D, Hd, za, Hd, p[DM_RSSM_GRU_WIH], p[DM_RSSM_GRU_BIH], nullptr, 0, gi, 3 * D));
      DM_TRY(linear(st, sk, skb, M, 3 * D, D, cur, F, p[DM_RSSM_GRU_WHH], p[DM_RSSM_GRU_BHH], nullptr, 0, gh, 3 * D));
      if (kind == 0) DM_TRY(dm_gru_gates_fwd_launch(M, D, gi, gh, cur, F, nxt, F, nullptr, nullptr, nullptr, nullptr, st));
      else DM_TRY(dm_gru_norm_fwd_launch(kind, M, D, gi, gh, cur, F, gk.lng[0], gk.lnb[0], nxt, F, gsw, gstw, nullptr, nullptr, st));
    }
    DM_TRY(linear(st, sk, skb, M, Hd, D, nxt, F, p[DM_RSSM_PRIOR_H_W], p[DM_RSSM_PRIOR_H_B], nullptr, 0, x1, Hd));
    DM_TRY(norm_elu_fwd(M, Hd, x1, Hd, p[DM_RSSM_PRIOR_G], p[DM_RSSM_PRIOR_B], 1e-3f, za, Hd, stats, st));
    DM_TRY(linear(st, sk, skb, M, ZP, Hd, za, Hd, p[DM_RSSM_PRIOR_W], p[DM_RSSM_PRIOR_OB], nullptr, 0, prior, ZP));
    return dm_sample_onehot_launch(M, S, C, prior, ZP, u_prior + (size_t)i * M * S, nullptr, nxt + D, F, pidx, nullptr, nullptr, st);
  }
};

extern "C" int dm_dream_rollout(const dm_shape* s, int M, const float* start, const dm_rssm_params* P,
                                const dm_mlp_params* actor, const float* u_act, const float* u_prior, float* feats,
                                float* actions, int32_t* act_idx, float* actor_acts, float* actor_logits, void* ws,
                                size_t ws_bytes, void* stream) {
  DM_REQUIRE(s && start && P && actor && u_act && u_prior && feats && actions && ws, DM_E_NULL,
             "dream_rollout: null pointer");
  DmPrecisionScope prec(s->flags & DM_FLAG_BF16);
  DM_TRY(rssm_check(s));
  DM_REQUIRE(M >= 1 && s->H >= 1, DM_E_SHAPE, "dream_rollout: M=%d H=%d", M, s->H);
  RolloutCtx c = {};
  rssm_dims(s, &c);
  c.M = M; c.H = s->H; c.Hm = s->mlp_hidden; c.L = s->mlp_layers; c.adist = s->flags & 3;
  DM_REQUIRE(c.adist <= 2, DM_E_SHAPE, "dream_rollout: unknown actor distribution %d", c.adist);
  c.AO = c.adist == 0 ? c.A : 2 * c.A;
  DM_REQUIRE((actor_acts == nullptr) == (actor_logits == nullptr), DM_E_NULL,
             "dream_rollout: actor_acts and actor_logits must be given together");
  c.p = P->p; c.actor = actor; c.st = (hipStream_t)stream;
  c.u_act = u_act; c.u_prior = u_prior; c.feats = feats; c.actions = actions; c.act_idx = act_idx;
  c.actor_acts = actor_acts; c.actor_logits = actor_logits;
  DmTwinScope tw((s->flags & DM_FLAG_BF16) != 0);
  DM_TRY(c.plan(ws, ws_bytes));
  tl_last_schedule[2] = (c.wzt ? DM_SCHED_ROLL_WZT : 0) | (c.wat ? DM_SCHED_ROLL_WAT : 0) | (c.actor_wpack ? DM_SCHED_ROLL_ACTOR_WPACK : 0) |
                        (c.actor_add0 ? DM_SCHED_ROLL_ACTOR_ADD0 : 0) | (c.fuse_act ? DM_SCHED_ROLL_FUSE_ACT : 0) |
                        (c.tw_on ? DM_SCHED_ROLL_TW_ON : 0);
  const float* const* p = c.p;
  const int H = c.H, D = c.D, Hd = c.Hd, Z = c.Z, ZP = c.ZP, F = c.F;
  hipStream_t st = c.st;
  DmRolloutMarks marks(st);
  const bool marks_eager = st == (hipStream_t)stream;
  DM_TRY(gru_stack(s, p, nullptr, &c.gk));

  if (c.tw_on) {
    const DmCvtSeg sg[4] = {{p[DM_RSSM_GRU_WIH], c.wih_h, (size_t)3 * D * Hd}, {p[DM_RSSM_GRU_WHH], c.whh_h, (size_t)3 * D * D},
                            {p[DM_RSSM_PRIOR_H_W], c.wph_h, (size_t)Hd * D}, {p[DM_RSSM_PRIOR_W], c.wp_h, (size_t)ZP * Hd}};
    DM_TRY(dm_to_bf16_multi_launch(sg, 4, st));
    for (int i = 0; i < 4; ++i) dm_twin_add(sg[i].src, sg[i].n, sg[i].dst, true);
    dm_twin_add(c.za, (size_t)M * Hd, c.za_h, false);
    for (int i = 1; i <= H && i < 40; ++i)
      dm_twin_add(feats + (size_t)i * M * F, (size_t)M * F, c.feats_h + (size_t)i * M * F, false);
  }
  if (c.wzt) DM_TRY(transpose(st, p[DM_RSSM_Z_W], c.wzt, Hd, Z));
  if (c.wat) DM_TRY(transpose(st, p[DM_RSSM_A_W], c.wat, Hd, c.A));
  if (c.actor_w0t) DM_TRY(transpose(st, actor->w[0], c.actor_w0t, c.Hm, F));
  if (c.actor_wpack) DM_TRY(dm_mlp_chain_pack_launch(F, c.L, actor, c.actor_wpack, st, c.actor_w0t ? D : 0));
  hipError_t e = hipMemcpyAsync(feats, start, (size_t)M * F * sizeof(float), hipMemcpyDeviceToDevice, st);
  if (e != hipSuccess) return dm_fail(DM_E_HIP, "dream_rollout: %s", hipGetErrorString(e));
  for (int i = 0; i < H; ++i) {
    DM_TRY(c.rollout_actor(i));
    DM_TRY(c.rollout_cell(i));
    marks.at_step(i, st, marks_eager);
  }
  return DM_OK;
}

static RolloutDims rollout_dims(const dm_shape* s) {
  dm_shape e = *s;
  e.B = s->B * (s->I > 0 ? s->I : 1); e.I = 1;
  RolloutDims d = {};
  rssm_dims(&e, &d);
  d.M = d.N; d.H = s->H > 0 ? s->H : 1; d.Hm = s->mlp_hidden; d.L = s->mlp_layers; d.adist = s->flags & 3;
  d.AO = d.adist == 0 ? d.A : 2 * d.A;
  return d;
}
size_t dm_rssm_ws_floats(const dm_shape* s, size_t parts[2]) {
  if (!s) return 0;
  const RolloutDims d = rollout_dims(s);
  const bool chain64 = !d.gauss && d.kind == 0 && d.layers == 1 && d.B <= 64;
  const bool wzt = !d.gauss && d.T > 1 && dm_z_embed_ok(d.Hd);
  PostWs pw;
  BpttWs bw;
  const size_t fwd = post_layout(DmArena(nullptr, 0), d, wzt, chain64 && d.C == 32, chain64 && wzt && (d.F & 3) == 0 && d.T >= 3, &pw);
  const size_t bwd = bptt_layout(DmArena(nullptr, 0), d, chain64, chain64, &bw);
  if (parts) { parts[0] = fwd; parts[1] = bwd; }
  return fwd > bwd ? fwd : bwd;
}
size_t dm_rollout_ws_floats(const dm_shape* s) {
  if (!s) return 0;
  const RolloutDims d = rollout_dims(s);
  const bool tw = (s->flags & DM_FLAG_BF16) && d.kind == 0 && d.layers == 1 && (d.F & 7) == 0;
  RolloutWs w;
  return rollout_layout(DmArena(nullptr, 0), d, false, tw, true, true, true, &w);
}
```

### pydreamer_amd/hip.py

```python
import ctypes
import os
from ctypes import POINTER, Structure, c_char_p, c_float, c_int, c_int32, c_int64, c_size_t, c_void_p

import torch

_HERE = os.path.dirname(os.path.abspath(__file__))
LIB_PATH = os.environ.get('DM_LIB_PATH') or os.path.join(_HERE, 'libdreamer_hip.so')

DM_MAX_MLP_LAYERS = 8
DM_GEMM_ACCUM = 1
DM_GEMM_ELU = 2
DM_C2I_ELU = 1
DM_FLAG_IMAGE_U8 = 16
DM_FLAG_BF16 = 128
DM_GEMM_BF16 = 256

RSSM_PARAM_ORDER = [
    'z_mlp.weight', 'z_mlp.bias', 'a_mlp.weight', 'in_norm.weight', 'in_norm.bias',
    'gru.layers.0.weight_ih', 'gru.layers.0.weight_hh', 'gru.layers.0.bias_ih', 'gru.layers.0.bias_hh',
    'prior_mlp_h.weight', 'prior_mlp_h.bias', 'prior_norm.weight', 'prior_norm.bias', 'prior_mlp.weight', 'prior_mlp.bias',
    'post_mlp_h.weight', 'post_mlp_h.bias', 'post_mlp_e.weight', 'post_norm.weight', 'post_norm.bias',
    'post_mlp.weight', 'post_mlp.bias',
]
GRU_KINDS = {'gru': 0, 'gru_layernorm': 1, 'gru_layernorm_dv2': 2}
DM_FLAG_GRU_SHIFT = 5
_LN_SLOTS = {
    'gru': [None] * 6,
    'gru_layernorm': ['ln_reset.weight', 'ln_reset.bias', 'ln_update.weight', 'ln_update.bias', 'ln_newval.weight', 'ln_newval.bias'],
    'gru_layernorm_dv2': ['lnorm.weight', 'lnorm.bias', None, None, None, None],
}


DM_FLAG_GRU_LAYERS_SHIFT = 8
SCHED_FWD = {'fuse_ln': 1, 'fuse_sample': 2, 'frag': 4, 'wzt': 8, 'psync': 16}
SCHED_BWD = {'fuse_b': 1, 'fold': 2, 'fold_sm': 4, 'frag': 8}
SCHED_BWD_NCHUNK_SHIFT = 8
SCHED_ROLL = {'wzt': 1, 'wat': 2, 'actor_wpack': 4, 'actor_add0': 8, 'fuse_act': 16, 'tw_on': 32}
DM_MAX_GRU_LAYERS = 4


def rssm_param_names(gru_type='gru', gru_layers=1):
    names = list(RSSM_PARAM_ORDER)
    if gru_type != 'gru':
        ren = {'gru.layers.0.weight_ih': 'gru.layers.0.weight_ih.weight', 'gru.layers.0.weight_hh': 'gru.layers.0.weight_hh.weight',
               'gru.layers.0.bias_ih': None, 'gru.layers.0.bias_hh': None}
        names = [ren.get(n, n) for n in names]
    ln = lambda i: [n and f'gru.layers.{i}.{n}' for n in _LN_SLOTS[gru_type]]
    names = names + ln(0)
    cell = ('weight_ih', 'weight_hh', 'bias_ih', 'bias_hh') if gru_type == 'gru' else ('weight_ih.weight', 'weight_hh.weight', None, None)
    for i in range(1, DM_MAX_GRU_LAYERS):
        names += [f'gru.layers.{i}.{n}' if (n and i < gru_layers) else None for n in cell]
    for i in range(1, DM_MAX_GRU_LAYERS):
        names += ln(i) if i < gru_layers else [None] * 6
    return names


DM_RSSM_NPARAMS = len(RSSM_PARAM_ORDER) + 6 + (4 + 6) * (DM_MAX_GRU_LAYERS - 1)


class DreamerHipError(RuntimeError):
    pass


class dm_shape(Structure):
    _fields_ = [(n, c_int32) for n in ('T', 'B', 'I', 'H', 'D', 'Hd', 'S', 'C', 'E', 'A', 'mlp_hidden', 'mlp_layers',
                                       'cnn_depth', 'img', 'img_ch', 'flags')]


class dm_mlp_params(Structure):
    _fields_ = [('w', c_void_p * (DM_MAX_MLP_LAYERS + 1)), ('b', c_void_p * (DM_MAX_MLP_LAYERS + 1)),
                ('ln_g', c_void_p * DM_MAX_MLP_LAYERS), ('ln_b', c_void_p * DM_MAX_MLP_LAYERS),
                ('precision', c_int32), ('reserved_', c_int32)]


class dm_mlp_grads(Structure):
    _fields_ = [('w', c_void_p * (DM_MAX_MLP_LAYERS + 1)), ('b', c_void_p * (DM_MAX_MLP_LAYERS + 1)),
                ('ln_g', c_void_p * DM_MAX_MLP_LAYERS), ('ln_b', c_void_p * DM_MAX_MLP_LAYERS)]


class dm_conv_params(Structure):
    _fields_ = [('w', c_void_p * 5), ('b', c_void_p * 5)]


dm_conv_grads = dm_conv_params


class dm_rssm_params(Structure):
    _fields_ = [('p', c_void_p * DM_RSSM_NPARAMS)]


dm_rssm_grads = dm_rssm_params


class dm_reduce_item(Structure):
    _fields_ = [('x', c_void_p), ('n', c_int64), ('scale', c_float), ('mode', c_int32), ('center', c_void_p)]


class dm_replay_field(Structure):
    _fields_ = [('dst', c_void_p), ('row_bytes', c_int64), ('is_reset', c_int32), ('reserved_', c_int32)]


DM_REPLAY_MAX_FIELDS = 16


class dm_gru_params(Structure):
    _fields_ = [('w_ih', c_void_p), ('w_hh', c_void_p), ('b_ih', c_void_p), ('b_hh', c_void_p)]


dm_gru_grads = dm_gru_params


def gru_struct(w_ih, w_hh, b_ih, b_hh):
    s = dm_gru_params()
    s.w_ih, s.w_hh, s.b_ih, s.b_hh = w_ih.data_ptr(), w_hh.data_ptr(), b_ih.data_ptr(), b_hh.data_ptr()
    return s

_P = c_void_p
_SIGNATURES = {
    'dm_version': (c_int, []),
    'dm_last_error': (c_char_p, []),
# ... 31 lines not shown
    'dm_mlp_head_fwd': (c_int, [c_int, c_int, c_int, c_int, c_int, _P, c_int, POINTER(dm_mlp_params), _P, _P, _P,
                                c_size_t, _P]),
    'dm_mlp_head_fwd_sparse': (c_int, [c_int, c_int, c_int, c_int, c_int, c_int, _P, c_int, POINTER(dm_mlp_params), _P, _P, _P, c_size_t, _P]),
    'dm_mlp_head_bwd': (c_int, [c_int, c_int, c_int, c_int, c_int, _P, c_int, POINTER(dm_mlp_params), _P, _P,
                                POINTER(dm_mlp_grads), _P, c_int, c_int, _P, c_size_t, _P]),
    'dm_head_loss': (c_int, [c_int, c_int, _P, _P, c_float, c_float, _P, _P, _P, _P]),
    'dm_head_loss_normal_nd': (c_int, [c_int, c_int, _P, _P, c_float, c_float, _P, _P, _P, _P]),
    'dm_head_loss_catsup': (c_int, [c_int, c_int, c_int, _P, c_int, _P, _P, c_float, _P, _P, _P, _P, _P]),
    'dm_disag_reward': (c_int, [c_int, c_int, c_int, _P, c_int64, c_int, c_float, _P, _P]),
    'dm_ensemble_mse': (c_int, [c_int, c_int, c_int, _P, c_int64, c_int, _P, c_int, _P, c_float, _P, _P, _P]),
    'dm_cat_target_index': (c_int, [c_int, c_int, c_int, _P, _P, _P]),
    'dm_cat_image_loss': (c_int, [c_int, c_int, c_int, c_int, _P, c_int, _P, _P, _P, _P]),
    'dm_cat_image_pred': (c_int, [c_int, c_int, c_int, c_int, _P, c_int, _P, _P, _P, _P, _P, _P]),
    'dm_cat_concat_rows': (c_int, [c_int, c_int, c_int, c_int, _P, c_int, _P, _P, _P]),
    'dm_dense_image_rows': (c_int, [c_int, c_int, c_int, _P, _P, _P, _P, _P, c_int, _P]),
    'dm_elu_rows_fwd': (c_int, [c_int, c_int, _P, c_int, _P, c_int, _P]),
    'dm_elu_rows_bwd': (c_int, [c_int, c_int, _P, c_int, _P, c_int, _P, c_int, _P]),
    'dm_cat_image_loss_mix': (c_int, [c_int, c_int, c_int, c_int, _P, c_int, _P, c_float, _P, _P, _P]),
    'dm_goals_stats_ws_floats': (c_size_t, [c_int, c_int]),
    'dm_goals_stats': (c_int, [c_int, c_int, _P, _P, _P, _P, _P, c_size_t, _P]),
    'dm_preprocess_image_u8': (c_int, [c_int64, c_int, c_int, _P, _P, _P]),
    'dm_conv_encoder_acts_floats': (c_size_t, [POINTER(dm_shape)]),
    'dm_conv_encoder_fwd': (c_int, [POINTER(dm_shape), _P, POINTER(dm_conv_params), _P, _P, _P, c_size_t, _P]),
    'dm_conv_encoder_bwd': (c_int, [POINTER(dm_shape), _P, POINTER(dm_conv_params), _P, _P, POINTER(dm_conv_grads), _P,
                                    c_size_t, _P]),
    'dm_conv_encoder_fwd_planes': (c_int, [POINTER(dm_shape), _P, POINTER(dm_conv_params), _P, _P, _P, _P, c_int, _P, c_size_t, _P]),
    'dm_conv_encoder_bwd_planes': (c_int, [POINTER(dm_shape), _P, POINTER(dm_conv_params), _P, _P, _P, _P, c_int,
                                           POINTER(dm_conv_grads), _P, c_size_t, _P]),
    'dm_conv_decoder_acts_floats': (c_size_t, [POINTER(dm_shape)]),
    'dm_conv_decoder_pred_offset': (c_size_t, [POINTER(dm_shape)]),
    'dm_conv_decoder_mse_fwd': (c_int, [POINTER(dm_shape), _P, c_int, _P, POINTER(dm_conv_params), _P, _P, _P, _P,
                                        c_size_t, _P]),
    'dm_conv_decoder_mse_bwd': (c_int, [POINTER(dm_shape), _P, c_int, _P, POINTER(dm_conv_params), _P, c_float,
                                        POINTER(dm_conv_grads), _P, c_int, _P, c_size_t, _P]),
    'dm_conv_decoder_mse_bwd_rows': (c_int, [POINTER(dm_shape), _P, c_int, _P, POINTER(dm_conv_params), _P, c_float, _P,
                                             POINTER(dm_conv_grads), _P, c_int, _P, c_size_t, _P]),
    'dm_rssm_acts_floats': (c_size_t, [POINTER(dm_shape)]),
    'dm_rssm_sequence_fwd': (c_int, [POINTER(dm_shape), _P, _P, _P, _P, _P, _P, _P, POINTER(dm_rssm_params), _P, _P, _P,
                                     _P, _P, _P, c_size_t, _P]),
    'dm_rssm_sequence_bwd': (c_int, [POINTER(dm_shape), _P, _P, _P, POINTER(dm_rssm_params), _P, _P, _P, _P, _P, _P,
                                     POINTER(dm_rssm_grads), _P, _P, c_size_t, _P]),
    'dm_dream_rollout': (c_int, [POINTER(dm_shape), c_int, _P, POINTER(dm_rssm_params), POINTER(dm_mlp_params), _P, _P,
                                 _P, _P, _P, _P, _P, _P, c_size_t, _P]),
    'dm_gae_losses': (c_int, [c_int, c_int, c_float, c_float, _P, _P, _P, _P, _P, _P, _P, _P]),
    'dm_actor_loss': (c_int, [c_int, c_int, _P, _P, _P, _P, c_float, c_float, _P, _P, _P, _P]),
    'dm_critic_loss': (c_int, [c_int, _P, _P, _P, c_float, _P, _P, _P]),
    'dm_sample_continuous': (c_int, [c_int, c_int, c_int, _P, _P, _P, _P]),
    'dm_actor_loss_continuous': (c_int, [c_int, c_int, c_int, _P, _P, _P, _P, c_float, c_float, _P, _P, _P, _P]),
    'dm_multi_sum': (c_int, [c_int, POINTER(dm_reduce_item), _P, _P]),
    'dm_combine': (c_int, [c_int, _P, POINTER(c_float), _P, _P]),
    'dm_multi_tensor_norm_clip': (c_int, [_P, c_int64, c_float, _P, _P, c_size_t, _P]),
    'dm_scale_inplace': (c_int, [_P, c_int64, _P, _P]),
    'dm_adamw_step': (c_int, [_P, _P, _P, _P, c_int64, c_float, c_float, c_float, c_float, c_float, c_int, _P, _P]),
    'dm_copy_params': (c_int, [_P, _P, c_int64, _P]),
    'dm_axpby': (c_int, [c_int64, c_float, _P, c_float, _P, _P]),
    'dm_prof_begin': (c_int, [c_int]),
    'dm_prof_end': (c_int, [POINTER(ctypes.c_double), c_int]),
    'dm_prof_rows': (c_int, [POINTER(ctypes.c_double), c_int]),
    'dm_mlp_chain_min_rows': (c_int, [c_int]),
    'dm_rollout_fuse_act_enable': (c_int, [c_int]),
    'dm_bf16_twins_enable': (c_int, [c_int]),
    'dm_gemm_dma_enable': (c_int, [c_int]),
    'dm_gemm_plan_query': (c_int, [c_int, c_int, c_int, c_int, c_int, c_int, c_int, c_int, c_int, c_int, c_int, c_int, c_size_t,
                                   POINTER(c_int32)]),
    'dm_mlp_plan_query': (c_int, [c_int] * 15 + [c_size_t, POINTER(c_int32)]),
    'dm_convt_kskip_enable': (c_int, [c_int]),
    'dm_conv_plan_query': (c_int, [c_int, POINTER(dm_shape), c_int, POINTER(c_int32), POINTER(c_size_t)]),
    'dm_kl_staged_enable': (c_int, [c_int]),
    'dm_dec_l4_bwd_direct_enable': (c_int, [c_int]),
    'dm_dec_l4_fwd_shared_enable': (c_int, [c_int]),
    'dm_rssm_lds_enable': (c_int, [c_int]),
    'dm_bptt_fold_enable': (c_int, [c_int]),
    'dm_rssm_lds_status': (c_int, []),
    'dm_rssm_lds_status_ack': (c_int, []),
    'dm_rssm_lds_gave_up': (c_int, []),
    'dm_rssm_lds_prof': (c_int, [_P, c_int]),
    'dm_rssm_last_schedule': (c_int, [c_int]),
    'dm_wgrad_side_arm': (c_int, [c_int]),
    'dm_wgrad_side_touch': (c_int, []),
    'dm_wgrad_side_join': (c_int, [_P]),
    'dm_dream_rollout_marks': (c_int, [c_int, POINTER(c_int), POINTER(c_void_p)]),
    'dm_mlp_head_fwd_rows': (c_int, [c_int, c_int, c_int, c_int, c_int, c_int, c_int, c_int, _P, c_int, POINTER(dm_mlp_params), _P, _P, _P,
                                     c_size_t, _P]),
    'dm_replay_gather': (c_int, [c_int, c_int, c_int, POINTER(dm_replay_field), _P, _P, _P]),
    'dm_gru_sequence_acts_floats': (c_size_t, [c_int, c_int, c_int, c_int]),
    'dm_gru_sequence_ws_bytes': (c_size_t, [c_int, c_int, c_int, c_int]),
    'dm_gru_sequence_fwd': (c_int, [c_int, c_int, c_int, c_int, _P, c_int, _P, _P, POINTER(dm_gru_params), _P, _P, c_int,
                                    _P, c_size_t, _P]),
    'dm_gru_sequence_bwd': (c_int, [c_int, c_int, c_int, c_int, _P, c_int, POINTER(dm_gru_params), _P, _P, c_int, _P, c_int,
                                    POINTER(dm_gru_grads), _P, c_int, _P, c_size_t, _P]),
    'dm_gru_sequence_last_schedule': (c_int, []),
    'dm_gru_sequence_fuse_enable': (c_int, [c_int]),
    'dm_policy_draw_ws_floats': (c_size_t, [c_int]),
    'dm_policy_draw': (c_int, [c_int, c_int, c_int, _P, c_int, _P, _P, _P, c_int, _P, _P, _P, _P, _P, c_size_t, _P]),
    'dm_policy_draw_mode': (c_int, [c_int, c_int, c_float, c_int, c_int, _P, c_int, _P, _P, _P, _P, c_int, _P, _P, _P, _P, _P, c_size_t,
                                    _P]),
    'dm_cem_draw': (c_int, [c_int, c_int, c_int, c_int, c_int, _P, _P, _P, _P, _P]),
    'dm_cem_update': (c_int, [c_int, c_int, c_int, c_int, c_int, c_int, c_float, _P, _P, _P, _P, _P, _P, c_float, c_float, _P, _P, _P,
                              _P, _P, _P]),
    'dm_twohot_decode': (c_int, [c_int, c_int, _P, c_int, _P, _P, _P]),
    'dm_twohot_loss': (c_int, [c_int, c_int, c_int, _P, c_int, _P, _P, _P, c_float, _P, _P, _P, _P]),
    'dm_return_norm': (c_int, [c_int, _P, c_float, c_float, c_float, c_float, c_int, _P, _P, _P, c_int, _P]),
    'dm_twohot_head_loss': (c_int, [c_int, c_int, c_int, _P, c_int, _P, _P, c_float, _P, _P, _P, _P]),
    'dm_metric_accum': (c_int, [c_int, _P, _P, _P, _P, _P, _P]),
    'dm_batch_stats': (c_int, [c_int, _P, _P, _P, _P, _P]),
    'dm_masked_mean': (c_int, [c_int, c_int, _P, c_int, c_int, _P, c_int, _P, _P]),
    'dm_export_image_u8': (c_int, [c_int, c_int, c_int, c_int, c_int, c_int, _P, _P, _P]),
}

_lib = None
DM_ABI_VERSION = 17


def lib():
    global _lib
    if _lib is None:
        if not os.path.exists(LIB_PATH):
            raise DreamerHipError(
                f'{LIB_PATH} not found: build it with `python -c "import __graft_entry__ as g; g.build()"` '
                f'(or `make -C pydreamer_amd/csrc`). There is no CPU fallback for the training path.')
        handle = ctypes.CDLL(LIB_PATH)
        for name, (restype, argtypes) in _SIGNATURES.items():
            fn = getattr(handle, name)
            fn.restype = restype
            fn.argtypes = argtypes
        if handle.dm_version() != DM_ABI_VERSION:
            raise DreamerHipError(f'{LIB_PATH} has ABI version {handle.dm_version()}, this binding is written for '
                                  f'{DM_ABI_VERSION}: rebuild it (`make -C pydreamer_amd/csrc`)')
        _lib = handle
    return _lib


def exported_symbols():
    return sorted(_SIGNATURES)


def call(name, *args):
    fn = getattr(lib(), name)
    rc = fn(*args)
    if rc != 0:
        msg = lib().dm_last_error().decode('utf-8', 'replace')
        raise DreamerHipError(f'{name} failed with code {rc}: {msg}')
    return rc


def last_schedule(which):
    word = int(lib().dm_rssm_last_schedule(which))
    if word < 0:
        raise DreamerHipError(f'dm_rssm_last_schedule({which}): no such entry point')
    bits = (SCHED_FWD, SCHED_BWD, SCHED_ROLL)[which]
    out = {k: bool(word & v) for k, v in bits.items()}
    if which == 1:
        out['nchunk'] = (word >> SCHED_BWD_NCHUNK_SHIFT) & 15
    return out


def ptr(t):
    if t is None:
        return None
    if not t.is_cuda:
        raise DreamerHipError(f'expected a CUDA/HIP tensor, got device {t.device} (no CPU path)')
    if not t.is_contiguous():
        raise DreamerHipError(f'expected a contiguous tensor, got strides {t.stride()} for shape {tuple(t.shape)}')
    return c_void_p(t.data_ptr())


# ... 62 lines not shown
```

### pydreamer_amd/models.py

```python
import contextlib
import ctypes
import math

import numpy as np
import torch
import torch.nn as nn

from . import hip as H
from .optim import FusedAdamW

MLP_HIDDEN = 400
ACTOR_KINDS = {'onehot': 0, 'tanh_normal': 1, 'normal_tanh': 2}
REWARD_STD = 0.3989422804
NORMAL_LOSS_CONST = REWARD_STD ** 2 * (math.log(REWARD_STD) + math.log(math.sqrt(2 * math.pi)))


class _Params(nn.Module):
    def forward(self, *a, **k):
        raise RuntimeError('pydreamer_amd modules hold parameters only; compute runs in libdreamer_hip.so')


class LinearP(_Params):
    def __init__(self, in_dim, out_dim, bias=True):
        super().__init__()
# ... 4 lines not shown
            bound = 1 / math.sqrt(in_dim)
            nn.init.uniform_(self.bias, -bound, bound)


class LayerNormP(_Params):
    def __init__(self, dim):
        super().__init__()
        self.weight = nn.Parameter(torch.ones(dim))
        self.bias = nn.Parameter(torch.zeros(dim))


class ConvP(_Params):
    def __init__(self, shape, bias_dim):
        super().__init__()
        self.weight = nn.Parameter(torch.empty(*shape))
        self.bias = nn.Parameter(torch.zeros(bias_dim))
        nn.init.xavier_uniform_(self.weight)


class GRUCellP(_Params):
    def __init__(self, input_size, hidden_size):
        super().__init__()
        self.weight_ih = nn.Parameter(torch.empty(3 * hidden_size, input_size))
        self.weight_hh = nn.Parameter(torch.empty(3 * hidden_size, hidden_size))
        self.bias_ih = nn.Parameter(torch.zeros(3 * hidden_size))
        self.bias_hh = nn.Parameter(torch.zeros(3 * hidden_size))


class _Slot(_Params):
    """Parameter-free placeholder keeping nn.Sequential indices aligned with the reference (LN/ELU/Flatten slots)."""


def init_weights_tf2(m):
    if isinstance(m, (LinearP, ConvP)):
        nn.init.xavier_uniform_(m.weight.data)
        if m.bias is not None:
            nn.init.zeros_(m.bias.data)
    if isinstance(m, GRUCellP):
        nn.init.xavier_uniform_(m.weight_ih.data)
        nn.init.orthogonal_(m.weight_hh.data)
        nn.init.zeros_(m.bias_ih.data)
        nn.init.zeros_(m.bias_hh.data)


class MLP(_Params):

    _base = 0

    def __init__(self, in_dim, out_dim, hidden_dim, hidden_layers, layer_norm=True):
        super().__init__()
        self.in_dim, self.out_dim, self.hidden_dim, self.hidden_layers = in_dim, out_dim, hidden_dim, hidden_layers
        self.layer_norm = bool(layer_norm)
        layers, dim = [_Slot()] * self._base, in_dim
        for _ in range(hidden_layers):
            layers += [LinearP(dim, hidden_dim), LayerNormP(hidden_dim) if layer_norm else _Slot(), _Slot()]
            dim = hidden_dim
        layers += [LinearP(dim, out_dim)]
        if out_dim == 1 or self._base:
            layers += [_Slot()]
        self.model = nn.Sequential(*layers)

    def tensors(self):
        L, o = self.hidden_layers, self._base
        w = [self.model[o + 3 * i].weight for i in range(L)] + [self.model[o + 3 * L].weight]
        b = [self.model[o + 3 * i].bias for i in range(L)] + [self.model[o + 3 * L].bias]
        g = [self.model[o + 3 * i + 1].weight for i in range(L)] if self.layer_norm else []
        be = [self.model[o + 3 * i + 1].bias for i in range(L)] if self.layer_norm else []
        return w, b, g, be

    def param_list(self):
        return list(self.parameters())

    def struct(self):
        return H.mlp_struct(*self.tensors(), precision=getattr(self, 'precision', 0))

    def grad_struct(self, grads_by_param):
        w, b, g, be = self.tensors()
        pick = lambda ts: [grads_by_param[id(t)] for t in ts]
        return H.mlp_struct(pick(w), pick(b), pick(g), pick(be), cls=H.dm_mlp_grads)

    def acts_floats(self, rows):
        return int(H.lib().dm_mlp_acts_floats(rows, self.hidden_dim, self.hidden_layers))

    def fwd(self, x2d, ldx, rows, ws, acts=None, save_acts=True, sparse_cols=0, window=None, out=None):
        need = 4 * int(H.lib().dm_mlp_ws_floats(rows, self.hidden_dim, self.hidden_layers))
        if ws.numel() < need:
            raise H.DreamerHipError(f'MLP.fwd: workspace of {ws.numel()} bytes, need {need} for {rows} rows')
        if window is not None:
            rows_total, row0 = window
            assert out is not None and out.shape[0] == rows_total and (acts is not None or not save_acts)
            st = self.struct()
            H.call('dm_mlp_head_fwd_rows', rows_total, row0, rows, self.in_dim, sparse_cols if 0 < sparse_cols < self.in_dim else 0,
                   self.hidden_dim, self.hidden_layers, self.out_dim, H.fptr(x2d), ldx, ctypes.byref(st),
                   H.fptr(acts) if save_acts else None, H.fptr(out), H.ptr(ws), ws.numel(), H.stream())
            return out, acts
        if acts is None and save_acts:
            acts = torch.empty(self.acts_floats(rows), device=x2d.device)
        out = torch.empty(rows, self.out_dim, device=x2d.device)
        st = self.struct()
        if 0 < sparse_cols < self.in_dim:
            H.call('dm_mlp_head_fwd_sparse', rows, self.in_dim, sparse_cols, self.hidden_dim, self.hidden_layers, self.out_dim,
                   H.fptr(x2d), ldx, ctypes.byref(st), H.fptr(acts), H.fptr(out), H.ptr(ws), ws.numel(), H.stream())
        else:
            H.call('dm_mlp_head_fwd', rows, self.in_dim, self.hidden_dim, self.hidden_layers, self.out_dim, H.fptr(x2d), ldx,
                   ctypes.byref(st), H.fptr(acts), H.fptr(out), H.ptr(ws), ws.numel(), H.stream())
        return out, acts

    def bwd(self, x2d, ldx, rows, acts, dout, ws, dx=None, lddx=0, dx_accum=False, scratch=False):
        plist = self.param_list()
        flat, out, direct = _flat_views(plist, x2d.device, getattr(self, '_fused', None), scratch)
        self.bwd_into({id(p): v for p, v in zip(plist, out)}, x2d, ldx, rows, acts, dout, ws, dx, lddx, dx_accum)
        return out, flat, direct

    def bwd_into(self, gof, x2d, ldx, rows, acts, dout, ws, dx=None, lddx=0, dx_accum=False):
        st, gs = self.struct(), self.grad_struct(gof)
        H.call('dm_mlp_head_bwd', rows, self.in_dim, self.hidden_dim, self.hidden_layers, self.out_dim, H.fptr(x2d), ldx,
               ctypes.byref(st), H.fptr(acts), H.fptr(dout), ctypes.byref(gs), H.fptr(dx), lddx, 1 if dx_accum else 0, H.ptr(ws),
               ws.numel(), H.stream())


class ConvEncoder(_Params):

    def __init__(self, in_channels=3, cnn_depth=32):
        super().__init__()
        self.out_dim = cnn_depth * 32
        d = cnn_depth
        chans = [(in_channels, d), (d, 2 * d), (2 * d, 4 * d), (4 * d, 8 * d)]
        layers = []
        for ci, co in chans:
            layers += [ConvP((co, ci, 4, 4), co), _Slot()]
        layers += [_Slot()]
        self.model = nn.Sequential(*layers)

    def convs(self):
        return [self.model[i] for i in (0, 2, 4, 6)]


VECOBS_EMBED = 256
DENSE_EMBED = 256
DENSE_IMAGE_MAX_SIZE = 16


def dense_image_gate(conf):
    enc, dec = conf.image_encoder, conf.image_decoder
    if enc != 'dense' and dec != 'dense':
        return False
    top = H.DM_MAX_MLP_LAYERS - 1
    min_prob = float(getattr(conf, 'image_decoder_min_prob', 0) or 0)
    checks = [
        (enc == 'dense' and dec == 'dense', f'image_encoder={enc!r} with image_decoder={dec!r} (both must be dense)'),
        (bool(getattr(conf, 'image_categorical', False)), 'image_categorical is off (the decoder is a per-cell cross-entropy)'),
        (1 <= conf.image_size <= DENSE_IMAGE_MAX_SIZE, f'image_size={conf.image_size} (1..{DENSE_IMAGE_MAX_SIZE})'),
        (conf.image_channels >= 2, f'image_channels={conf.image_channels} (>= 2 classes)'),
        (1 <= conf.image_encoder_layers <= top, f'image_encoder_layers={conf.image_encoder_layers} (1..{top})'),
        (1 <= conf.image_decoder_layers <= top, f'image_decoder_layers={conf.image_decoder_layers} (1..{top})'),
        (not conf.vecobs_size, f'vecobs_size={conf.vecobs_size} (must be 0)'),
        (not getattr(conf, 'amp', False), 'amp=True (the dense image path is fp32)'),
        (0.0 <= min_prob < 1.0, f'image_decoder_min_prob={min_prob} (must lie in [0, 1))'),
    ]
    bad = [msg for ok, msg in checks if not ok]
    if bad:
        raise NotImplementedError("image_encoder / image_decoder = 'dense' is built for a categorical image only (both dense, "
                                  f'image_categorical, image_size <= {DENSE_IMAGE_MAX_SIZE}, image_channels >= 2, 1..{top} layers '
                                  'each, vecobs_size = 0, amp off, image_decoder_min_prob in [0, 1)); outside that gate: '
                                  + '; '.join(bad))
    return True


def _empty(x):
    return x is None or x == ''


def imageless_gate(conf):
    enc, dec = _empty(conf.image_encoder), _empty(conf.image_decoder)
# ... 380 lines not shown
        if dense:
            self.image = CatImageDecoder(features_dim, (conf.image_channels, conf.image_size, conf.image_size),
                                         conf.image_decoder_layers, conf.layer_norm, conf.image_decoder_min_prob)
        elif imageless:
            self.image = None
        else:
            self.image = ConvDecoder(in_dim=features_dim, out_channels=conf.image_channels, cnn_depth=conf.cnn_depth)
        if not imageless:
            self.image_shape = (conf.image_channels, conf.image_size, conf.image_size)
        if support is not None:
            self.reward = DenseCategoricalSupportDecoder(features_dim, support, conf.reward_decoder_layers, conf.layer_norm)
        elif twohot is not None:
            self.reward = DenseTwoHotDecoder(features_dim, twohot[0], twohot[1], conf.reward_decoder_layers, conf.layer_norm)
        else:
            self.reward = DenseNormalDecoder(features_dim, conf.reward_decoder_layers, conf.layer_norm)
        self.reward_bins = 0 if support is None else len(support)
        self.terminal = DenseBernoulliDecoder(features_dim, conf.terminal_decoder_layers, conf.layer_norm)
        self.vecobs_weight = conf.vecobs_weight
        if conf.vecobs_size:
            self.vecobs = DenseNormalDecoder(features_dim, 4, conf.layer_norm, out_dim=conf.vecobs_size, nd=True)
        else:
            self.vecobs = None
        self.sparse_cols = conf.stoch_dim * conf.stoch_discrete

    def heads(self):
        hs = [('reward', self.reward, self.reward_weight), ('terminal', self.terminal, self.terminal_weight)]
        return hs + [('vecobs', self.vecobs, self.vecobs_weight)] if self.vecobs is not None else hs

    @staticmethod
    def _targets(names, obs, pk):
        y = {n: pk['vecobs'] if n == 'vecobs' else obs[n].float().contiguous() for n in names}
        return {n: (t, t if pk['I'] == 1 else t.repeat_interleave(pk['I'], dim=int(n != 'vecobs')).contiguous()) for n, t in y.items()}

    def heads_loss(self, pk, obs, ws, gw):
        feat, NE, hs, res, bwd = pk['feat'], pk['T'] * pk['B'], self.heads(), {}, []
        N = feat.shape[0]
        for group in (hs[:2], hs[2:]):
            y = self._targets([n for n, _, _ in group], obs, pk)
            outs = [head.model.fwd(feat, self.features_dim, N, ws, sparse_cols=self.sparse_cols) for _, head, _ in group]
            for (n, head, weight), (out, acts) in zip(group, outs):
                loss, dout, rec, _ = head.loss(out, y[n][head.target_rows], gw * weight / NE, grad=True, I=pk['I'])
                res[n] = (loss, rec, y[n][1])
                bwd.append((head.model, acts, dout))
        return res, bwd

    def predict(self, pk, feat, obs, ws):
        T, B, I, shp = pk['T'], pk['B'], pk['I'], pk['shp']
        NE, N, F_ = T * B, T * B * I, self.features_dim
        tb = lambda x: x.view(T, B, *x.shape[1:])
        red = (lambda x, mode: x) if I == 1 else (lambda x, mode: _reduce_i(x, NE, I, mode))
        li, image_pred = self.decode(shp, feat, pk['image'], ws, target=pk.get('target'), loss=True)
        hs, lp, pred, bins = self.heads(), {}, {}, {}
        outs = [head.model.fwd(feat, F_, N, ws, save_acts=False)[0] for _, head, _ in hs[:2]]
        for n, head, _ in hs[2:]:
            y = self._targets([n], obs, pk)[n]
            l, _, p, _ = head.loss(head.model.fwd(feat, F_, N, ws, save_acts=False)[0], y[head.target_rows], I=I)
            lp[n], pred[n] = red(l, 1), red(p, 0)
        y = self._targets([n for n, _, _ in hs[:2]], obs, pk)
        per_sample = [head.loss(out, y[n][head.target_rows], I=I, bins=True) for (n, head, _), out in zip(hs[:2], outs)]
        if li is not None:
            lp['image'] = red(li, 1)
        for mode, into, k in ((1, lp, 0), (0, pred, 2)):
            for (n, _, _), r in zip(hs[:2], per_sample):
                into[n], bins[n] = red(r[k], mode), r[3]
        if image_pred is not None:
            image_pred = image_pred.view(NE, I, *image_pred.shape[1:])
            pred['image'] = image_pred.mean(1) if I > 1 else image_pred[:, 0]
        metrics, tensors = {}, {}
        for group in ([n for n in ('image', 'reward', 'terminal') if n in lp], *([n] for n, _, _ in hs[2:])):
            tensors.update({f'logprob_{n}': tb(lp[n]) for n in group})
            tensors.update({f'{n}_pred': tb(pred[n]) for n in group})
            metrics.update({f'logprob_{n}': lp[n].mean() for n in group})
        nan = torch.full((), float('nan'), device=feat.device)
        nanmean = lambda x: torch.nansum(x) / (~torch.isnan(x)).sum()
        for n, head, _ in hs:
            for s, mask in head.buckets(obs.get(n), bins.get(n)):
                x = torch.where(mask.view(T, B), tb(lp[n]), nan)
                metrics[f'logprob_{n}{s}'], tensors[f'logprob_{n}{s}'] = nanmean(x), x
        return metrics, tensors

    def dream_buffers(self, rows, device):
        return [torch.empty(rows, head.model.out_dim, device=device) for _, head, _ in self.heads()[:2]]

    def dream_fwd(self, feat, row0, n, ws, bufs):
        for (_, head, _), out in zip(self.heads()[:2], bufs):
            head.model.fwd(feat, self.features_dim, n, ws, save_acts=False, sparse_cols=self.sparse_cols, window=(out.shape[0], row0),
                           out=out)

    def dream_means(self, bufs):
        return self.terminal.loss(bufs[1])[2], self.reward.loss(bufs[0])[2]

    def _conv_fwd(self, shp, feat, image, ws, acts, loss, pred):
        dl = self.image.layers()
        dec_p = H.conv_struct([m.weight for m in dl], [m.bias for m in dl])
        H.call('dm_conv_decoder_mse_fwd', ctypes.byref(shp), H.fptr(feat), self.features_dim, H.ptr(image), ctypes.byref(dec_p),
               H.fptr(acts), H.fptr(loss), H.fptr(pred), H.ptr(ws), ws.numel(), H.stream())

    def _conv_acts(self, shp, device):
        return torch.empty(int(H.lib().dm_conv_decoder_acts_floats(ctypes.byref(shp))), device=device)

    def image_buffers(self, shp, N, device):
        if self.imageless:
            return None, None
        return None if self.dense else self._conv_acts(shp, device), torch.empty(N, device=device)

    def image_loss(self, shp, feat, image, ws, acts, loss, gw):
        if self.imageless:
            return dict(dec_acts=None)
        if not self.dense:
            self._conv_fwd(shp, feat, image, ws, acts, loss, None)
            return dict(dec_acts=acts)
        dec, N, NE = self.image, feat.shape[0], shp.T * shp.B
        train = torch.is_grad_enabled()
        target = dec.target(image, NE)
        logits, acts = dec.fwd(feat, self.features_dim, N, ws, save_acts=train)
        dlogits = torch.empty_like(logits) if train else None
        dec.loss(logits, target, N, loss, dlogits)
        if train:
            scale = torch.full((1,), gw * self.image_weight / NE, device=feat.device)
            H.call('dm_scale_inplace', H.fptr(dlogits), dlogits.numel(), H.fptr(scale), H.stream())
        return dict(target=target, dec_acts=acts, dec_logits=logits, dlogits=dlogits)

    def image_heads(self, pk):
        return [(self.image, pk['dec_acts'], pk['dlogits'])] if self.dense else []

    def image_bwd(self, pk, gof, dfeat, scale, iw, ws):
        if self.dense or self.imageless:
            return
        dl, F_ = self.image.layers(), self.features_dim
        dec_p = H.conv_struct([m.weight for m in dl], [m.bias for m in dl])
        dec_g = H.conv_struct([gof[id(m.weight)] for m in dl], [gof[id(m.bias)] for m in dl], cls=H.dm_conv_grads)
        H.call('dm_conv_decoder_mse_bwd_rows', ctypes.byref(pk['shp']), H.fptr(pk['feat']), F_, H.ptr(pk['image']), ctypes.byref(dec_p),
               H.fptr(pk['dec_acts']), scale, H.fptr(iw), ctypes.byref(dec_g), H.fptr(dfeat), F_, H.ptr(ws), ws.numel(), H.stream())

    def decode(self, shp, feat, image, ws, target=None, loss=False, raw=False):
        if self.imageless:
            return None, None
        N, dev = feat.shape[0], feat.device
        li = torch.empty(N, device=dev) if loss else None
        if self.dense:
            logits, _ = self.image.fwd(feat, self.features_dim, N, ws, save_acts=False)
            if loss:
                self.image.loss(logits, target, N, li, None)
            pred = logits if raw else self.image.logp(logits, target, N)
        else:
            acts = self._conv_acts(shp, dev)
            pred = torch.empty(N, *self.image_shape, device=dev)
            self._conv_fwd(shp, feat, image, ws, acts, li, pred)
        return li, pred.view(N, *self.image_shape)

    def image_rec_thunk(self, pk):
        T, B, I = pk['T'], pk['B'], pk['I']
        Cc, S, _ = self.image_shape
        if self.dense:
            def thunk(logits=pk['dec_logits'], target=pk['target']):
                with torch.no_grad():
                    return self.image.logp(logits, target, T * B).view(T, B, Cc, S, S)
            return thunk
        N, hw = T * B * I, S * S
        pred_off = int(H.lib().dm_conv_decoder_pred_offset(ctypes.byref(pk['shp'])))

        def thunk(acts=pk['dec_acts']):
            with torch.no_grad():
                pred = acts[pred_off:pred_off + N * hw * Cc].view(N, hw, Cc)
                rec = pred.transpose(1, 2).contiguous().view(T, B, I, Cc, S, S)
                return rec[:, :, 0] if I == 1 else rec.mean(2)
        return thunk


class NormGRUCellP(_Params):
# ... 999 lines not shown
        flat, views, direct = _flat_views(plist, grad_loss.device, getattr(owner, '_fused', None))
        gof = {id(p): v for p, v in zip(plist, views)}
        for hp in pk['heads']:
            hp['mlp'].bwd_into(gof, hp['x'], hp['ldx'], hp['rows'], hp['acts'], hp['dout'], hp['ws'])
            for k in ('acts', 'dout', 'x'):
                hp.pop(k, None)
        pk['consumed'] = True
        return (None, None) + _finish_backward(owner, views, flat, direct, grad_loss)


class ActorCritic(_Params):

    def __init__(self, in_dim, out_actions, hidden_dim=400, hidden_layers=4, layer_norm=True, gamma=0.999, lambda_gae=0.95,
                 entropy_weight=1e-3, target_interval=100, actor_grad='reinforce', actor_dist='onehot', critic_dist='mse',
                 critic_bins=255, critic_bin_range=20.0, return_norm='none', return_norm_lo=0.05, return_norm_hi=0.95,
                 return_norm_decay=0.99, return_norm_limit=1.0):
        super().__init__()
        if actor_dist not in ACTOR_KINDS or actor_grad != 'reinforce':
            raise NotImplementedError(f'actor_dist={actor_dist!r} / actor_grad={actor_grad!r}: the HIP path builds onehot, '
                                      f'tanh_normal and normal_tanh actors with actor_grad=reinforce (actor_grad=dynamics '
                                      f'asserts in the reference itself, SURVEY 0.5)')
        if critic_dist not in CRITIC_DISTS:
            raise ValueError(f'critic_dist={critic_dist!r}: one of {CRITIC_DISTS}')
        if return_norm not in RETURN_NORMS:
            raise ValueError(f'return_norm={return_norm!r}: one of {RETURN_NORMS}')
        if int(critic_bins) != critic_bins or not 2 <= critic_bins <= 256:
            raise ValueError(f'critic_bins={critic_bins}: 2 .. 256')
        if not (math.isfinite(critic_bin_range) and critic_bin_range > 0):
            raise ValueError(f'critic_bin_range={critic_bin_range}: a finite number > 0')
        if not 0.0 <= return_norm_lo <= return_norm_hi <= 1.0:
            raise ValueError(f'return_norm_lo={return_norm_lo}, return_norm_hi={return_norm_hi}: 0 <= lo <= hi <= 1')
        if not 0.0 <= return_norm_decay < 1.0:
            raise ValueError(f'return_norm_decay={return_norm_decay}: in [0, 1)')
        if not (math.isfinite(return_norm_limit) and return_norm_limit > 0):
            raise ValueError(f'return_norm_limit={return_norm_limit}: a finite number > 0')
        self.dist_kind = ACTOR_KINDS[actor_dist]
        self.in_dim, self.out_actions = in_dim, out_actions
        self.gamma, self.lambda_, self.entropy_weight = gamma, lambda_gae, entropy_weight
        self.target_interval, self.actor_grad, self.actor_dist = target_interval, actor_grad, actor_dist
        self.critic_dist, self.critic_bins, self.critic_bin_range = critic_dist, int(critic_bins), float(critic_bin_range)
        self.return_norm, self.return_norm_q = return_norm, (float(return_norm_lo), float(return_norm_hi))
        self.return_norm_decay, self.return_norm_limit = float(return_norm_decay), float(return_norm_limit)
        actor_out_dim = out_actions if actor_dist == 'onehot' else 2 * out_actions
        critic_out_dim = self.critic_bins if critic_dist == 'twohot' else 1
        self.actor = MLP(in_dim, actor_out_dim, hidden_dim, hidden_layers, layer_norm)
        self.critic = MLP(in_dim, critic_out_dim, hidden_dim, hidden_layers, layer_norm)
        self.critic_target = MLP(in_dim, critic_out_dim, hidden_dim, hidden_layers, layer_norm)
        self.critic_target.requires_grad_(False)
        if critic_dist == 'twohot':
            out_layer = self.critic.model[3 * hidden_layers]
            nn.init.zeros_(out_layer.weight)
            nn.init.zeros_(out_layer.bias)
            self.register_buffer('bins', torch.linspace(-self.critic_bin_range, self.critic_bin_range, self.critic_bins),
                                 persistent=False)
        if return_norm == 'percentile':
            self.register_buffer('return_range', torch.zeros(2))
        self.train_steps = 0
        self.sparse_cols = 0
        self.defer_target_update = False

    def update_critic_target(self):
        with torch.no_grad():
            for dst, src in zip(self.critic_target.parameters(), self.critic.parameters()):
                H.call('dm_copy_params', H.fptr(dst), H.fptr(src), dst.numel(), H.stream())

    def begin_step(self, log_only=False):
        if not log_only and not self.defer_target_update:
            if self.train_steps % self.target_interval == 0:
                self.update_critic_target()
            self.train_steps += 1

    @staticmethod
    def split_steps(J):
        return (J * 5) // 8 if J >= 9 else J

    def value_buffers(self, rows, device):
        bufs = dict(value_t=torch.empty(rows, 1, device=device), value=torch.empty(rows, 1, device=device),
                    c_acts=torch.empty(self.critic.acts_floats(rows), device=device))
        if self.critic_dist == 'twohot':
            bufs.update(logits_t=torch.empty(rows, self.critic_bins, device=device),
                        logits=torch.empty(rows, self.critic_bins, device=device))
        return bufs

    def value(self, feats, F_, rows, ws, target=False, window=None, out=None, acts=None, save_acts=False, sparse=True, logits=None):
        mlp = self.critic_target if target else self.critic
        sp = self.sparse_cols if sparse else 0
        if self.critic_dist == 'mse':
            return mlp.fwd(feats, F_, rows, ws, acts=acts, save_acts=save_acts, sparse_cols=sp, window=window, out=out)
        K = self.critic_bins
        if window is not None:
            rows_total, row0 = window
            assert logits is not None and tuple(logits.shape) == (rows_total, K) and out is not None
            mlp.fwd(feats, F_, rows, ws, acts=acts, save_acts=save_acts, sparse_cols=sp, window=window, out=logits)
            lg, v = logits[row0:row0 + rows], out[row0:row0 + rows]
        else:
            lg, acts = mlp.fwd(feats, F_, rows, ws, acts=acts, save_acts=save_acts, sparse_cols=sp)
            out = v = torch.empty(rows, 1, device=lg.device)
        H.call('dm_twohot_decode', rows, K, H.fptr(lg), K, H.fptr(self.bins), H.fptr(v), H.stream())
        return out, acts

    def forward_values(self, feats, F_, rows_total, row0, rows, ws, bufs):
        w = (rows_total, row0)
        self.value(feats, F_, rows, ws, target=True, window=w, out=bufs['value_t'], logits=bufs.get('logits_t'))
        self.value(feats, F_, rows, ws, window=w, out=bufs['value'], acts=bufs['c_acts'], save_acts=True, logits=bufs.get('logits'))

    def training_step(self, features, actions, rewards, terminals, log_only=False, act_idx=None, ws=None,
                      actor_acts=None, actor_logits=None, overlap=None, mbuf=None, values=None, _begun=False):
        _require_cuda(features, 'features')
        if not _begun:
            self.begin_step(log_only)
        J, M, F_ = features.shape
        Hh, A, dev = J - 1, self.out_actions, features.device
        feats = features.contiguous().view(J * M, F_)
        rewards, terminals = rewards.contiguous(), terminals.contiguous()
        if self.dist_kind == 0:
            if act_idx is None:
                act_idx = actions.argmax(-1).to(torch.int32)
            act_idx = act_idx.contiguous().view(-1)
        if ws is None:
            raise H.DreamerHipError('ActorCritic.training_step needs the model workspace (called through Dreamer.training_step)')

        sp = self.sparse_cols
        if values is None:
            values = self.value_buffers(J * M, dev)
            r0 = self.split_steps(J) * M
            for a, b in ((0, r0), (r0, J * M)):
                if b > a:
                    self.forward_values(feats, F_, J * M, a, b - a, ws, values)
        value_t, value, c_acts = values['value_t'], values['value'], values['c_acts']
        if actor_acts is not None:
            logits, a_acts = actor_logits, actor_acts
        else:
            logits, a_acts = self.actor.fwd(feats, F_, Hh * M, ws, sparse_cols=sp)
        adv, agae, vtgt, wgt = (torch.empty(Hh, M, device=dev) for _ in range(4))
        H.call('dm_gae_losses', Hh, M, self.gamma, self.lambda_, H.fptr(rewards), H.fptr(terminals), H.fptr(value_t),
               H.fptr(adv), H.fptr(agae), H.fptr(vtgt), H.fptr(wgt), H.stream())
        rows = Hh * M
        lc = torch.empty(rows, device=dev)
        gw = float(getattr(self, 'grad_weight', 1.0))
        if self.critic_dist == 'twohot':
            dvalue = None if log_only else torch.empty(J * M, self.critic_bins, device=dev)
            H.call('dm_twohot_loss', rows, J * M, self.critic_bins, H.fptr(values['logits']), self.critic_bins, H.fptr(self.bins),
                   H.fptr(vtgt), H.fptr(wgt), gw / rows, H.fptr(lc), H.fptr(dvalue), None, H.stream())
        else:
            dvalue = torch.zeros(J * M, 1, device=dev)
            H.call('dm_critic_loss', rows, H.fptr(value), H.fptr(vtgt), H.fptr(wgt), gw / rows, H.fptr(lc), H.fptr(dvalue),
                   H.stream())
        agae_a = agae
        if self.return_norm == 'percentile':
            agae_a, rn_out = agae.clone(), torch.empty(5, device=dev)
            H.call('dm_return_norm', rows, H.fptr(vtgt), self.return_norm_q[0], self.return_norm_q[1], self.return_norm_decay,
                   self.return_norm_limit, int(torch.is_grad_enabled() and not log_only), H.fptr(self.return_range),
                   H.fptr(rn_out), H.fptr(agae_a), rows, H.stream())
        la, ent = torch.empty(rows, device=dev), torch.empty(rows, device=dev)
        dlogits = torch.empty(rows, self.actor.out_dim, device=dev)
        if self.dist_kind == 0:
            H.call('dm_actor_loss', rows, A, H.fptr(logits), H.ptr(act_idx), H.fptr(agae_a), H.fptr(wgt), self.entropy_weight,
                   gw / rows, H.fptr(la), H.fptr(ent), H.fptr(dlogits), H.stream())
        else:
            H.call('dm_actor_loss_continuous', self.dist_kind, rows, A, H.fptr(logits), H.fptr(actions.contiguous()),
                   H.fptr(agae_a), H.fptr(wgt), self.entropy_weight, gw / rows, H.fptr(la), H.fptr(ent), H.fptr(dlogits),
                   H.stream())
        value2d = value.view(J, M)
        reward1 = rewards.view(J, M)[1:]
        if mbuf is None:
            mbuf = torch.zeros(METRIC_BUF_FLOATS, device=dev)
        s = _multi_sum([(lc, 1.0 / rows), (la, 1.0 / rows), (ent, 1.0 / rows), (value2d[0], 1.0 / M),
                        (value2d[:-1], 1.0 / rows), (reward1, 1.0 / rows)], dev, out=mbuf[8:14])
        std = _multi_sum([(reward1, 1.0 / max(rows - 1, 1), s[5:6], 2)], dev, out=mbuf[14:15])
        loss_critic_v, loss_actor_v = s[0], s[1]
        if log_only:
            loss_actor, loss_critic = loss_actor_v, loss_critic_v
        else:
            pa = dict(loss=loss_actor_v, x=feats, ldx=F_, rows=rows, acts=a_acts, dout=dlogits, ws=ws, overlap=overlap)
            pc = dict(loss=loss_critic_v, x=feats, ldx=F_, rows=J * M, acts=c_acts, dout=dvalue, ws=ws, overlap=overlap)
            loss_actor = _HeadLoss.apply(self.actor, pa, *self.actor.param_list())
            loss_critic = _HeadLoss.apply(self.critic, pc, *self.critic.param_list())
            self._last_packs = (pa, pc)
        metrics = dict(loss_critic=loss_critic_v, loss_actor=loss_actor_v, policy_entropy=s[2], policy_value=s[3],
                       policy_value_im=s[4], policy_reward=s[5], policy_reward_std=std[0])
        if self.return_norm == 'percentile':
            s0 = RETURN_METRIC_SLOTS['policy_return_lo']
            mbuf[s0:s0 + 3].copy_(rn_out[2:5])
            metrics.update({k: mbuf[i] for k, i in RETURN_METRIC_SLOTS.items()})
        tensors = dict(value=value2d, value_target=vtgt, value_advantage=adv, value_advantage_gae=agae, value_weight=wgt)
        return (loss_actor, loss_critic), metrics, tensors

# ... 156 lines not shown
        assert 'action' in obs, 'Observation should contain previous action'
        act_shape = obs['action'].shape
        assert len(act_shape) == 3 and act_shape[0] == 1, f'Expected shape (1,B,A), got {act_shape}'
        self.join_optimizers()
        features, out_state = self.wm.forward(obs, in_state, None if noise is None else noise['u_post'])
        B = act_shape[1]
        feat = features.reshape(B, -1)
        shp = self.wm.shape(1, B, 1)
        ws = self.wm.workspace(shp, feat.device)
        logits, _ = self.ac.actor.fwd(feat, feat.shape[1], B, ws, save_acts=False)
        value, _ = self.ac.value(feat, feat.shape[1], B, ws, sparse=False)
        action_distr = _torch_actor_distribution(self.ac.actor_dist, logits.view(1, B, -1))
        return action_distr, out_state, dict(policy_value=value.mean())

    def act(self, obs, in_state, noise=None, return_rows=False, mode='sample', action_noise=0.0, ac=None):
        ac = self.ac if ac is None else ac
        assert 'action' in obs, 'Observation should contain previous action'
        act_shape = obs['action'].shape
        assert len(act_shape) == 3 and act_shape[0] == 1, f'Expected shape (1,B,A), got {act_shape}'
        B, A, kind = act_shape[1], self.conf.action_dim, ac.dist_kind
        noise = noise or {}
        u_act = noise.get('u_act')
        ua_shape = (B,) if kind == 0 else (B, A)
        if u_act is not None and tuple(u_act.shape) != ua_shape:
            raise ValueError(f'actor noise has shape {tuple(u_act.shape)}, expected {ua_shape}')
        if mode not in ('sample', 'mode'):
            raise ValueError(f"mode is {mode!r}, expected 'sample' or 'mode'")
        action_noise = float(action_noise)
        if not action_noise >= 0.0:
            raise ValueError(f'action_noise is {action_noise}, expected a number >= 0')
        if action_noise > 0.0 and mode == 'mode':
            raise ValueError("action_noise > 0 goes with mode='sample': the distribution's mode is taken without noise")
        u_expl = noise.get('u_expl')
        ue_shape = (B, 2) if kind == 0 else (B, A)
        if u_expl is not None and tuple(u_expl.shape) != ue_shape:
            raise ValueError(f'exploration noise has shape {tuple(u_expl.shape)}, expected {ue_shape}')
        draw_mode = 1 if mode == 'mode' else (2 if action_noise > 0.0 else 0)
        with torch.no_grad():
            self.join_optimizers()
            features, out_state = self.wm.forward(obs, in_state, noise.get('u_post'))
            feat = features.reshape(B, -1)
            dev = feat.device
            ws = self.wm.workspace(self.wm.shape(1, B, 1), dev)
            logits, _ = ac.actor.fwd(feat, feat.shape[1], B, ws, save_acts=False)
            value, _ = ac.value(feat, feat.shape[1], B, ws, sparse=False)
            if draw_mode == 1:
                u_act = None
            else:
                if u_act is None:
                    u_act = torch.rand(ua_shape, device=dev) if kind == 0 else torch.randn(ua_shape, device=dev)
                u_act = u_act.float().contiguous()
            if draw_mode == 2:
                if u_expl is None:
                    u_expl = torch.rand(ue_shape, device=dev) if kind == 0 else torch.randn(ue_shape, device=dev)
                u_expl = u_expl.float().contiguous()
            action = torch.empty(1, B, A, device=dev)
            stats = torch.empty(4, device=dev)
            dws = torch.empty(int(H.lib().dm_policy_draw_ws_floats(B)), device=dev)
            rows = torch.empty(2, B, device=dev) if return_rows else None
            act_idx = torch.empty(B, dtype=torch.int32, device=dev) if return_rows and kind == 0 else None
            tail = (H.fptr(value), H.fptr(action), A, H.ptr(act_idx), H.fptr(rows), None if rows is None else H.fptr(rows[1]),
                    H.fptr(stats), H.fptr(dws), dws.numel() * 4, H.stream())
            if draw_mode == 0:
                H.call('dm_policy_draw', kind, B, A, H.fptr(logits), logits.shape[1], H.fptr(u_act), *tail)
            else:
                H.call('dm_policy_draw_mode', kind, draw_mode, action_noise, B, A, H.fptr(logits), logits.shape[1], H.fptr(u_act),
                       H.fptr(u_expl) if draw_mode == 2 else None, *tail)
        metrics = dict(policy_value=stats[0], action_prob=stats[1], policy_entropy=stats[2])
        if return_rows:
            metrics.update(log_prob=rows[0], entropy=rows[1], value=value.view(B))
            if kind == 0:
                metrics['act_idx'] = act_idx
        return action, out_state, metrics

    def dream(self, in_state, imag_horizon, dynamics_gradients=False, u_act=None, u_prior=None, _pack=None):
        if dynamics_gradients:
            raise NotImplementedError('actor_grad=dynamics is not built (and not runnable in the reference, SURVEY 0.5)')
        h, z = in_state
        _require_cuda(h, 'in_state')
        Hh = int(imag_horizon)
        start = torch.cat((h, z), -1).contiguous()
        return self._dream_from_features(start, Hh, u_act, u_prior, _pack)

    def _dream_from_features(self, start, Hh, u_act=None, u_prior=None, _pack=None, early=None, ac=None):
        c = self.conf
        ac = self.ac if ac is None else ac
        M, dev = start.shape[0], start.device
        F_, A, S = self.wm.features_dim, c.action_dim, c.stoch_dim
        shp = self.wm.shape(1, M, Hh)
        ws = self.wm.workspace(shp, dev)
        kind = ac.dist_kind
        ua_shape = (Hh, M) if kind == 0 else (Hh, M, A)
        if u_act is not None and tuple(u_act.shape) != ua_shape:
            raise ValueError(f'actor noise has shape {tuple(u_act.shape)}, expected {ua_shape}')
        if u_act is None:
            u_act = torch.rand(ua_shape, device=dev) if kind == 0 else torch.randn(ua_shape, device=dev)
        if u_prior is None:
            u_prior = (torch.rand if c.stoch_discrete else torch.randn)(Hh, M, S, device=dev)
        u_act, u_prior = u_act.float().contiguous(), u_prior.reshape(Hh, M, S).float().contiguous()
        start = start.contiguous()
        feats = torch.empty(Hh + 1, M, F_, device=dev)
        actions = torch.empty(Hh, M, A, device=dev)
        act_idx = torch.empty(Hh, M, dtype=torch.int32, device=dev)
        cell_p = H.rssm_struct(self.wm.core.cell.ordered())
        actor_p = ac.actor.struct()
        a_acts = a_logits = None
        if _pack is not None:
            a_acts = torch.empty(int(ac.actor.acts_floats(Hh * M)), device=dev)
            a_logits = torch.empty(Hh * M, ac.actor.out_dim, device=dev)
        rows = (Hh + 1) * M
        r_split = ac.split_steps(Hh + 1) * M
        use_early = (early is not None and _pack is not None and r_split < rows and _HEADS_EARLY
                     and not getattr(c, 'amp', False))
        if use_early:
            H.call('dm_dream_rollout_marks', 1, (ctypes.c_int * 1)(r_split // M - 2),
                   (ctypes.c_void_p * 1)(int(early.ev_mark.cuda_event)))
        H.call('dm_dream_rollout', ctypes.byref(shp), M, H.fptr(start), ctypes.byref(cell_p), ctypes.byref(actor_p),
               H.fptr(u_act), H.fptr(u_prior), H.fptr(feats), H.fptr(actions), H.ptr(act_idx),
               H.fptr(a_acts), H.fptr(a_logits), H.ptr(ws), ws.numel(), H.stream())
        f2 = feats.view(rows, F_)
        dec = self.wm.decoder
        outs = dec.dream_buffers(rows, dev)
        values = ac.value_buffers(rows, dev) if _pack is not None else None

        def heads(a, b, wsx):
            if b <= a:
                return
            dec.dream_fwd(f2, a, b - a, wsx, outs)
            if values is not None:
                ac.forward_values(f2, F_, rows, a, b - a, wsx, values)
        if use_early:
            early.s_ac.wait_event(early.ev_mark)
            with torch.cuda.stream(early.s_ac):
                heads(0, r_split, early.ws_ac)
                early.ev_heads.record(early.s_ac)
            heads(r_split, rows, ws)
            torch.cuda.current_stream().wait_event(early.ev_heads)
        else:
            heads(0, r_split, ws)
            heads(r_split, rows, ws)
        term, mu = dec.dream_means(outs)
        if _pack is not None:
            _pack.update(act_idx=act_idx, ws=ws, actor_acts=a_acts, actor_logits=a_logits, values=values, head_outs=outs)
        return feats, actions, _Mean(mu.view(Hh + 1, M)), _Mean(term.view(Hh + 1, M))

    def training_step(self, obs, in_state, iwae_samples=None, imag_horizon=None, do_open_loop=False, do_image_pred=False,
                      do_dream_tensors=False, noise=None, forced_idx=None):
        for k in ('action', 'reward', 'reset', 'terminal'):
            assert k in obs, f'`{k}` required in observation'
        iwae_samples = int(iwae_samples or self.iwae_samples)
        imag_horizon = int(imag_horizon or self.imag_horizon)
        if self.wm.dense and iwae_samples > 1:
            raise NotImplementedError('iwae_samples > 1 is not built on the dense image path (DESIGN 4.11)')
        if self.wm.kl_free > 0 and iwae_samples > 1:
            raise NotImplementedError('kl_free > 0 with iwae_samples > 1: the sampled KL has no per-row exact KL to clip')
        T, B = obs['action'].shape[:2]
        noise = noise or {}
        I = iwae_samples
        u_post = noise.get('u_post')
        if u_post is not None:
            u_post = u_post.reshape(T, B * I, -1)

        if self._overlap is not None:
            stale = [getattr(self.wm, '_last_pack', None)] + list(getattr(self.ac, '_last_packs', None) or ())
            for old_pk in stale:
                fut = old_pk.get('pre') if isinstance(old_pk, dict) else None
                if fut is not None:
                    try:
                        fut.result()
                    except Exception:
                        pass
            cur = torch.cuda.current_stream()
            cur.wait_stream(self._overlap.s_wm)
            if not self._ac_pipelined():
                cur.wait_stream(self._overlap.s_ac)
        mbuf = torch.zeros(METRIC_BUF_FLOATS, device=obs['action'].device)
        self.metric_buffer = mbuf
        tail = None
        dev0 = obs['action'].device
        if (self.overlap_backward and torch.is_grad_enabled() and self.wm_tail_on_side and dev0.type == 'cuda'
                and not torch.cuda.is_current_stream_capturing()):
            if self._overlap is None or self._overlap.s_wm.device != dev0:
                self._overlap = _Overlap(dev0)
            tail = self._overlap
        loss_model, features, states, out_state, metrics, tensors = \
            self.wm.training_step(obs, in_state, iwae_samples=iwae_samples, do_open_loop=do_open_loop,
                                  do_image_pred=do_image_pred, u_post=u_post, forced_idx=forced_idx,
                                  imag_horizon=imag_horizon, u_pred=noise.get('u_pred'), mbuf=mbuf, _tail=tail)
        pk = self.wm._last_pack
        ov = None
        if not (self.overlap_backward and torch.is_grad_enabled()):
            self._set_ac_home(None)
        if self.overlap_backward and torch.is_grad_enabled():
            dev = pk['feat'].device
            if self._overlap is None or self._overlap.s_wm.device != dev:
                self._overlap = _Overlap(dev)
            ov = self._overlap
            pk['overlap'] = ov
            self._set_ac_home(ov)
            gens = {}
            for owner in (self.wm, self.ac.actor, self.ac.critic):
                if getattr(owner, '_fused', None) is not None:
                    gens[id(owner)] = owner._fused.claim_scratch()
            ov.ws_wm = _grow_ws(ov.ws_wm, pk['ws'].numel(), dev)
            ov.ev_wm_fwd.record(ov.s_wm if pk.get('tail') is not None else torch.cuda.current_stream())
            pk['pre'] = ov.submit(ov.s_wm, ov.ev_wm_fwd, lambda: self.wm._backward(
                pk, ov.ws_wm, scratch=gens.get(id(self.wm), True), defer_wgrad=True))
        metrics, tensors = dict(metrics), tensors.copy()
        if not isinstance(self.probe_model, NoProbeHead):
            loss_probe, metrics_probe, tensors_probe = self.probe_model.training_step(features.detach(), obs, mbuf=mbuf)
        else:
            loss_probe, metrics_probe, tensors_probe = self.probe_model.training_step(features.detach(), obs)
        metrics.update(**metrics_probe)
        tensors.update(**tensors_probe)

        dpk = {}
        if ov is not None:
            need = 4 * int(H.lib().dm_mlp_ws_floats((imag_horizon + 1) * T * B * I, MLP_HIDDEN, 4))
            ov.ws_ac = _grow_ws(ov.ws_ac, need, pk['feat'].device)
        self._await_ac_optimizers()
        self.ac.begin_step()
        features_dream, actions_dream, rewards_dream, terminals_dream = \
            self._dream_from_features(pk['feat'], imag_horizon,
                                      noise.get('u_act') if self.ac.dist_kind == 0 else noise.get('eps_act'),
                                      noise.get('u_prior'), _pack=dpk, early=ov)
        (loss_actor, loss_critic), metrics_ac, tensors_ac = \
            self.ac.training_step(features_dream, actions_dream, rewards_dream.mean, terminals_dream.mean,
                                  act_idx=dpk['act_idx'], ws=dpk['ws'], actor_acts=dpk['actor_acts'],
                                  actor_logits=dpk['actor_logits'], overlap=ov, mbuf=mbuf, values=dpk['values'], _begun=True)
        if ov is not None:
            ov.ev_fwd.record(torch.cuda.current_stream())
            for mlp, hp in zip((self.ac.actor, self.ac.critic), self.ac._last_packs):
                hp['pre'] = ov.submit(ov.s_ac, ov.ev_fwd, lambda mlp=mlp, hp=hp: mlp.bwd(
                    hp['x'], hp['ldx'], hp['rows'], hp['acts'], hp['dout'], ov.ws_ac, scratch=gens.get(id(mlp), True)))
        metrics.update(**metrics_ac)
        if I == 1:
            tensors.update(policy_value=tensors_ac['value'][0].view(T, B))
        else:
            tensors.update(policy_value=_reduce_i(tensors_ac['value'][0].contiguous().view(-1), T * B, I, 0).view(T, B))
        self.last_extras = dict(post_idx=pk['idx'].view(T, B * I, -1).clone(), act_idx=dpk['act_idx'].clone(),
                                actions=actions_dream, dream_features=features_dream, actor_logits=dpk.get('actor_logits'),
                                ac_tensors=tensors_ac, post=pk['post'], prior=pk['prior'], pred_idx=pk.get('pred_idx'),
                                dream_reward=rewards_dream.mean, dream_terminal=terminals_dream.mean,
                                dream_reward_out=dpk['head_outs'][0])
        dream_tensors = {}
        if do_dream_tensors and not self.wm.imageless:
            with torch.no_grad():
                kind, dpk2 = self.ac.dist_kind, {}
                f2, a2, r2, t2 = self._dream_from_features(
                    pk['feat'][:B * I:I].contiguous(), T - 1,
                    noise.get('u_act_log') if kind == 0 else noise.get('eps_act_log'), noise.get('u_prior_log'), _pack=dpk2)
                shp = pk['shp_e']
                ws = self.wm.workspace(shp, pk['feat'].device)
                _, image_dream = self.wm.decoder.decode(shp, f2.view(T * B, -1), pk['image'], ws, raw=True)
                _, _, t_ac2 = self.ac.training_step(f2, a2, r2.mean, t2.mean, log_only=True, act_idx=dpk2['act_idx'],
                                                    ws=dpk2['ws'], actor_acts=dpk2['actor_acts'],
                                                    actor_logits=dpk2['actor_logits'], values=dpk2['values'])
                dream_tensors = dict(action_pred=torch.cat([obs['action'][:1].float(), a2]), reward_pred=r2.mean,
                                     terminal_pred=t2.mean, image_pred=image_dream.view(T, B, *image_dream.shape[-3:]),
                                     **t_ac2)
                self.last_extras.update(dream_log_act_idx=dpk2['act_idx'].clone(), dream_log_reward_out=dpk2['head_outs'][0])
        if pk.get('tail') is not None:
            cur = torch.cuda.current_stream()
            cur.wait_event(pk['tail'].ev_tail)
            leaving = [loss_model, pk.get('dec_acts'), pk.get('dec_logits'), pk.get('target'), pk.get('closed')] + [v for v in dict.values(pk['tensors']) if torch.is_tensor(v)]
            for t in leaving:
                if torch.is_tensor(t) and t.is_cuda:
                    t.record_stream(cur)
        if self.probe_gradients:
            losses = (loss_model + loss_probe, loss_actor, loss_critic)
        else:
            losses = (loss_model, loss_probe, loss_actor, loss_critic)
        return losses, out_state, metrics, tensors, dream_tensors

    def __str__(self):
        count = lambda m: sum(p.numel() for p in m.parameters())
        s = [f'Model: {count(self)} parameters']
        for sub in (self.wm.encoder, self.wm.decoder, self.wm.core, self.ac, self.probe_model):
            s.append(f'  {type(sub).__name__:<15}: {count(sub)} parameters')
        return '\n'.join(s)



def __getattr__(name):
    if name == 'WorldModelProbe':
        from .baselines import WorldModelProbe
        return WorldModelProbe
    raise AttributeError(f'module {__name__!r} has no attribute {name!r}')
```

Before: 31.03 grad-steps/s.

## Keep one-hot indices through dream rollout and gather head first-layer rows by index

The dream rollout now records the sampled categorical indices for every imagined step, seeded from the posterior indices. The reward, terminal and critic heads use those indices to gather and sum rows of the first-layer weight for the stochastic part, instead of scanning the dense one-hot columns. The step-0 actor addend also uses the index gather. The z_embed kernel is templated on width so that narrower hidden sizes use fewer registers. In exchange, an index buffer is allocated per call and the index pointers are handed over through thread-local state.

```diff
diff --git a/include/dreamer_hip.h b/include/dreamer_hip.h
--- a/include/dreamer_hip.h
+++ b/include/dreamer_hip.h
@@ -151,6 +151,11 @@
                     const dm_mlp_grads* g, float* dx, int lddx, int dx_accum,
                     void* ws, size_t ws_bytes, void* stream);
 
+int dm_mlp_head_fwd_rows_idx(int rows_total, int row0, int rows, int in_dim, int S, int C, const int32_t* idx, int hidden,
+                             int layers, int out_dim, const float* x, int ldx, const dm_mlp_params* p, float* acts, float* out,
+                             void* ws, size_t ws_bytes, void* stream);
+int dm_onehot_heads_enable(int on);
+
 int dm_head_loss(int kind, int rows, const float* out, const float* target, float scale, float loss_const,
                  float* loss, float* dout, float* mean_out, void* stream);
 
@@ -254,6 +259,8 @@
 #define DM_SCHED_ROLL_ACTOR_ADD0 8
 #define DM_SCHED_ROLL_FUSE_ACT 16
 #define DM_SCHED_ROLL_TW_ON 32
+#define DM_SCHED_ROLL_ADD0_IDX0 64
+#define DM_SCHED_ROLL_KEEP_IDX 128
 int dm_rssm_last_schedule(int which);
 
 typedef struct dm_gru_params { const float* w_ih; const float* w_hh; const float* b_ih; const float* b_hh; } dm_gru_params;
@@ -269,6 +276,8 @@
 int dm_gru_sequence_fuse_enable(int on);
 
 int dm_dream_rollout_marks(int n, const int* steps, void* const* events);
+
+int dm_dream_rollout_indices(const int32_t* start_idx, int32_t* feat_idx);
 
 int dm_dream_rollout(const dm_shape* shp, int M, const float* start, const dm_rssm_params* cell,
                      const dm_mlp_params* actor, const float* u_act, const float* u_prior,
diff --git a/pydreamer_amd/csrc/common.h b/pydreamer_amd/csrc/common.h
--- a/pydreamer_amd/csrc/common.h
+++ b/pydreamer_amd/csrc/common.h
@@ -240,6 +240,7 @@
   const float* wpack = nullptr;
   const float* add0 = nullptr;
   const DmChainSample* sample = nullptr;
+  const int32_t* idx = nullptr; int S = 0, C = 0;
 };
 enum { DM_MLP_PANEL = 0, DM_MLP_CHAIN = 1, DM_MLP_PER_LAYER = 2 };
 int dm_mlp_fwd_launch(const DmMlpFwd& q, void* ws, size_t ws_bytes, hipStream_t st);
diff --git a/pydreamer_amd/csrc/elementwise.hip b/pydreamer_amd/csrc/elementwise.hip
--- a/pydreamer_amd/csrc/elementwise.hip
+++ b/pydreamer_amd/csrc/elementwise.hip
@@ -672,6 +672,7 @@
   return (int)b;
 }
 
+template <int NJ>
 __global__ void __launch_bounds__(256) z_embed_kernel(int rows, int n, int S, int C, const int32_t* __restrict__ idx,
                                                       const uint8_t* __restrict__ row_zero, const float* __restrict__ Wt,
                                                       const float* __restrict__ bias, const float* __restrict__ add,
@@ -684,11 +685,11 @@
   const int row = blockIdx.x * 4 + (threadIdx.x >> 6);
   const int lane = threadIdx.x & 63;
   if (row >= rows) return;
-  float4 acc[4];
-  bool in[4];
-  int off[4];
-#pragma unroll
-  for (int j = 0; j < 4; ++j) {
+  float4 acc[NJ];
+  bool in[NJ];
+  int off[NJ];
+#pragma unroll
+  for (int j = 0; j < NJ; ++j) {
     const int c = (lane + 64 * j) * 4;
     in[j] = c < n;
     off[j] = in[j] ? c : 0;
@@ -696,7 +697,7 @@
   }
   if (add) {
 #pragma unroll
-    for (int j = 0; j < 4; ++j) {
+    for (int j = 0; j < NJ; ++j) {
       const float4 a = *reinterpret_cast<const float4*>(add + (size_t)row * ldadd + off[j]);
       acc[j].x += a.x; acc[j].y += a.y; acc[j].z += a.z; acc[j].w += a.w;
     }
@@ -704,7 +705,7 @@
   if (idx2) {
     const float* wr = Wt2 + (size_t)idx2[row] * n;
 #pragma unroll
-    for (int j = 0; j < 4; ++j) {
+    for (int j = 0; j < NJ; ++j) {
       const float4 a = *reinterpret_cast<const float4*>(wr + off[j]);
       acc[j].x += a.x; acc[j].y += a.y; acc[j].z += a.z; acc[j].w += a.w;
     }
@@ -716,25 +717,25 @@
       const int cnt = min(64, S - s0);
       int t = 0;
       for (; t + 8 <= cnt; t += 8) {
-        float4 w[8][4];
+        float4 w[8][NJ];
 #pragma unroll
         for (int u = 0; u < 8; ++u) {
           const float* wr = Wt + ((size_t)(s0 + t + u) * C + __shfl(mine, t + u, 64)) * n;
 #pragma unroll
-          for (int j = 0; j < 4; ++j) w[u][j] = *reinterpret_cast<const float4*>(wr + off[j]);
+          for (int j = 0; j < NJ; ++j) w[u][j] = *reinterpret_cast<const float4*>(wr + off[j]);
         }
         __builtin_amdgcn_sched_barrier(0);
 #pragma unroll
         for (int u = 0; u < 8; ++u)
 #pragma unroll
-          for (int j = 0; j < 4; ++j) {
+          for (int j = 0; j < NJ; ++j) {
             acc[j].x += w[u][j].x; acc[j].y += w[u][j].y; acc[j].z += w[u][j].z; acc[j].w += w[u][j].w;
           }
       }
       for (; t < cnt; ++t) {
         const float* wr = Wt + ((size_t)(s0 + t) * C + __shfl(mine, t, 64)) * n;
 #pragma unroll
-        for (int j = 0; j < 4; ++j) {
+        for (int j = 0; j < NJ; ++j) {
           const float4 w = *reinterpret_cast<const float4*>(wr + off[j]);
           acc[j].x += w.x; acc[j].y += w.y; acc[j].z += w.z; acc[j].w += w.w;
         }
@@ -742,7 +743,7 @@
     }
   }
 #pragma unroll
-  for (int j = 0; j < 4; ++j)
+  for (int j = 0; j < NJ; ++j)
     if (in[j]) {
       const int c = (lane + 64 * j) * 4;
       if (x) *reinterpret_cast<float4*>(x + (size_t)row * ldx + c) = acc[j];
@@ -751,7 +752,7 @@
   if (!y) return;
   if (!gamma) {
 #pragma unroll
-    for (int j = 0; j < 4; ++j)
+    for (int j = 0; j < NJ; ++j)
       if (in[j]) {
         float4 o;
         o.x = dm_elu(acc[j].x); o.y = dm_elu(acc[j].y); o.z = dm_elu(acc[j].z); o.w = dm_elu(acc[j].w);
@@ -761,19 +762,19 @@
   }
   float s1 = 0.f;
 #pragma unroll
-  for (int j = 0; j < 4; ++j)
+  for (int j = 0; j < NJ; ++j)
     if (in[j]) s1 += (acc[j].x + acc[j].y) + (acc[j].z + acc[j].w);
   const float mean = dm_wave_sum(s1) / (float)n;
   float s2 = 0.f;
 #pragma unroll
-  for (int j = 0; j < 4; ++j)
+  for (int j = 0; j < NJ; ++j)
     if (in[j]) {
       const float dx = acc[j].x - mean, dy = acc[j].y - mean, dz = acc[j].z - mean, dw = acc[j].w - mean;
       s2 += (dx * dx + dy * dy) + (dz * dz + dw * dw);
     }
   const float rstd = 1.0f / sqrtf(dm_wave_sum(s2) / (float)n + eps);
 #pragma unroll
-  for (int j = 0; j < 4; ++j)
+  for (int j = 0; j < NJ; ++j)
     if (in[j]) {
       const int c = (lane + 64 * j) * 4;
       const float4 g = *reinterpret_cast<const float4*>(gamma + c), b = *reinterpret_cast<const float4*>(beta + c);
@@ -963,8 +964,16 @@
   }
   unsigned short* y_h = (y && gamma) ? dm_twin_of(y, false) : nullptr;
   if (y_h) dm_twin_mark(y);
-  hipLaunchKernelGGL(z_embed_kernel, dim3(dm_cdiv(rows, 4)), dim3(256), 0, st, rows, n, S, C, idx, row_zero, Wt, bias, add,
-                     ldadd, idx2, Wt2, x, ldx, x_frag, gamma, beta, eps, y, ldy, y_h);
+  const dim3 grid(dm_cdiv(rows, 4)), blk(256);
+  if (n <= 256)
+    hipLaunchKernelGGL((z_embed_kernel<1>), grid, blk, 0, st, rows, n, S, C, idx, row_zero, Wt, bias, add, ldadd, idx2, Wt2, x, ldx,
+                       x_frag, gamma, beta, eps, y, ldy, y_h);
+  else if (n <= 512)
+    hipLaunchKernelGGL((z_embed_kernel<2>), grid, blk, 0, st, rows, n, S, C, idx, row_zero, Wt, bias, add, ldadd, idx2, Wt2, x, ldx,
+                       x_frag, gamma, beta, eps, y, ldy, y_h);
+  else
+    hipLaunchKernelGGL((z_embed_kernel<4>), grid, blk, 0, st, rows, n, S, C, idx, row_zero, Wt, bias, add, ldadd, idx2, Wt2, x, ldx,
+                       x_frag, gamma, beta, eps, y, ldy, y_h);
   DM_LAUNCH_CHECK();
   return DM_OK;
 }
diff --git a/pydreamer_amd/csrc/mlp.hip b/pydreamer_amd/csrc/mlp.hip
--- a/pydreamer_amd/csrc/mlp.hip
+++ b/pydreamer_amd/csrc/mlp.hip
@@ -1,6 +1,11 @@
 #include "common.h"
 
 static bool al16(const void* p) { return ((uintptr_t)p & 15) == 0; }
+static int g_onehot_heads = 1;
+extern "C" int dm_onehot_heads_enable(int on) {
+  if (on >= 0) g_onehot_heads = on ? 1 : 0;
+  return g_onehot_heads;
+}
 static const size_t MLP_SKB = DM_SPLITK_FLOATS * sizeof(float);
 
 struct MlpActs {
@@ -129,6 +134,9 @@
 static int mlp_sparse_addend(const MlpFwdCtx& c) {
   const DmMlpFwd& q = c.q;
   DM_TRY(dm_permute4_launch(q.p->w[0], c.w.w0t, 1, 1, q.hidden, q.in_dim, 0, 1, 3, 2, c.st));
+  if (q.idx && g_onehot_heads && q.S >= 1 && q.C >= 1 && q.S * q.C == q.sparse_cols && dm_z_embed_ok(q.hidden))
+    return dm_z_embed_launch(q.rows, q.hidden, q.S, q.C, q.idx, nullptr, c.w.w0t + (size_t)c.pl.k0 * q.hidden, nullptr, nullptr, 0,
+                             nullptr, nullptr, c.w.g, q.hidden, nullptr, nullptr, nullptr, 0.f, nullptr, 0, c.st);
   return dm_sparse_rows_launch(q.rows, q.hidden, q.sparse_cols, q.x + c.pl.k0, q.ldx, c.w.w0t + (size_t)c.pl.k0 * q.hidden,
                                c.w.g, q.hidden, c.st);
 }
@@ -232,7 +240,7 @@
 
 static int mlp_head_fwd(int rows_total, int row0, int rows, int in_dim, int sparse_cols, int hidden, int layers, int out_dim,
                         const float* x, int ldx, const dm_mlp_params* p, float* acts, float* out, void* ws, size_t ws_bytes,
-                        void* stream) {
+                        void* stream, const int32_t* idx = nullptr, int S = 0, int C = 0) {
   DmPrecisionScope prec(p->precision);
   DmMlpFwd q;
   q.rows = rows; q.in_dim = in_dim; q.hidden = hidden; q.layers = layers; q.out_dim = out_dim;
@@ -240,6 +248,7 @@
   q.acts = acts; q.acts_total_rows = rows_total; q.acts_row_off = row0;
   q.out = out + (size_t)row0 * out_dim; q.ldout = out_dim;
   q.sparse_cols = sparse_cols;
+  if (idx) { q.idx = idx + (size_t)row0 * S; q.S = S; q.C = C; }
   return dm_mlp_fwd_launch(q, ws, ws_bytes, (hipStream_t)stream);
 }
 
@@ -264,6 +273,18 @@
              row0 + rows, rows_total);
   return mlp_head_fwd(rows_total, row0, rows, in_dim, sparse_cols, hidden, layers, out_dim, x, ldx, p, acts, out, ws, ws_bytes,
                       stream);
+}
+
+extern "C" int dm_mlp_head_fwd_rows_idx(int rows_total, int row0, int rows, int in_dim, int S, int C, const int32_t* idx,
+                                        int hidden, int layers, int out_dim, const float* x, int ldx, const dm_mlp_params* p,
+                                        float* acts, float* out, void* ws, size_t ws_bytes, void* stream) {
+  DM_REQUIRE(x && p && out && ws && idx, DM_E_NULL, "mlp_head_fwd_rows_idx: null pointer");
+  DM_REQUIRE(row0 >= 0 && rows >= 1 && row0 + rows <= rows_total, DM_E_SHAPE, "mlp_head_fwd_rows_idx: window [%d, %d) of %d rows",
+             row0, row0 + rows, rows_total);
+  DM_REQUIRE(S >= 1 && C >= 1 && (long long)S * C < in_dim, DM_E_SHAPE, "mlp_head_fwd_rows_idx: %d groups of %d in %d columns", S, C,
+             in_dim);
+  return mlp_head_fwd(rows_total, row0, rows, in_dim, S * C, hidden, layers, out_dim, x, ldx, p, acts, out, ws, ws_bytes, stream,
+                      idx, S, C);
 }
 
 struct MlpBwdPlan {
diff --git a/pydreamer_amd/csrc/rssm.hip b/pydreamer_amd/csrc/rssm.hip
--- a/pydreamer_amd/csrc/rssm.hip
+++ b/pydreamer_amd/csrc/rssm.hip
@@ -716,6 +716,14 @@
   }
 };
 
+static thread_local const int32_t* tl_roll_start_idx = nullptr;
+static thread_local int32_t* tl_roll_feat_idx = nullptr;
+extern "C" int dm_dream_rollout_indices(const int32_t* start_idx, int32_t* feat_idx) {
+  tl_roll_start_idx = start_idx;
+  tl_roll_feat_idx = feat_idx;
+  return DM_OK;
+}
+
 static int g_rollout_fuse_act = 1;
 extern "C" int dm_rollout_fuse_act_enable(int on) {
   if (on >= 0) g_rollout_fuse_act = on ? 1 : 0;
@@ -775,6 +783,9 @@
   const float* const* p; const dm_mlp_params* actor; hipStream_t st; size_t skb;
   const float *u_act, *u_prior; float *feats, *actions; int32_t* act_idx; float *actor_acts, *actor_logits;
   bool tw_on;
+  const int32_t* start_idx; int32_t* feat_idx;
+  const int32_t* idx_in(int i) const { return feat_idx ? feat_idx + (size_t)i * M * S : i == 0 ? start_idx : pidx; }
+  int32_t* idx_out(int i) const { return feat_idx ? feat_idx + (size_t)(i + 1) * M * S : pidx; }
   bool fuse_act;
 
   int plan(void* ws, size_t ws_bytes) {
@@ -809,8 +820,8 @@
     const float* cur = feats + (size_t)i * M * F;
     float* act = actions + (size_t)i * M * A;
     if (actor_add0) {
-      if (i == 0) DM_TRY(dm_sparse_rows_launch(M, Hm, Z, cur + D, F, actor_w0t + (size_t)D * Hm, actor_add0, Hm, st));
-      else DM_TRY(dm_z_embed_launch(M, Hm, S, C, pidx, nullptr, actor_w0t + (size_t)D * Hm, nullptr, nullptr, 0, nullptr, nullptr,
+      if (i == 0 && !start_idx) DM_TRY(dm_sparse_rows_launch(M, Hm, Z, cur + D, F, actor_w0t + (size_t)D * Hm, actor_add0, Hm, st));
+      else DM_TRY(dm_z_embed_launch(M, Hm, S, C, idx_in(i), nullptr, actor_w0t + (size_t)D * Hm, nullptr, nullptr, 0, nullptr, nullptr,
                                     actor_add0, Hm, nullptr, nullptr, nullptr, 0.f, nullptr, 0, st));
     }
     int32_t* ai = act_idx_of(i);
@@ -832,7 +843,7 @@
     const bool embed = wzt && i > 0, embed_a = embed && wat && ai;
     if (!embed_a) DM_TRY(linear(st, sk, skb, M, Hd, A, act, A, p[DM_RSSM_A_W], nullptr, nullptr, 0, ea, Hd));
     if (embed) {
-      DM_TRY(dm_z_embed_launch(M, Hd, S, C, pidx, nullptr, wzt, p[DM_RSSM_Z_B], embed_a ? nullptr : ea, Hd,
+      DM_TRY(dm_z_embed_launch(M, Hd, S, C, idx_in(i), nullptr, wzt, p[DM_RSSM_Z_B], embed_a ? nullptr : ea, Hd,
                                embed_a ? ai : nullptr, wat, nullptr, Hd, nullptr, p[DM_RSSM_IN_G], p[DM_RSSM_IN_B], 1e-3f,
                                za, Hd, st));
     } else {
@@ -850,7 +861,7 @@
     DM_TRY(linear(st, sk, skb, M, Hd, D, nxt, F, p[DM_RSSM_PRIOR_H_W], p[DM_RSSM_PRIOR_H_B], nullptr, 0, x1, Hd));
     DM_TRY(norm_elu_fwd(M, Hd, x1, Hd, p[DM_RSSM_PRIOR_G], p[DM_RSSM_PRIOR_B], 1e-3f, za, Hd, stats, st));
     DM_TRY(linear(st, sk, skb, M, ZP, Hd, za, Hd, p[DM_RSSM_PRIOR_W], p[DM_RSSM_PRIOR_OB], nullptr, 0, prior, ZP));
-    return dm_sample_onehot_launch(M, S, C, prior, ZP, u_prior + (size_t)i * M * S, nullptr, nxt + D, F, pidx, nullptr, nullptr, st);
+    return dm_sample_onehot_launch(M, S, C, prior, ZP, u_prior + (size_t)i * M * S, nullptr, nxt + D, F, idx_out(i), nullptr, nullptr, st);
   }
 };
 
@@ -873,11 +884,16 @@
   c.p = P->p; c.actor = actor; c.st = (hipStream_t)stream;
   c.u_act = u_act; c.u_prior = u_prior; c.feats = feats; c.actions = actions; c.act_idx = act_idx;
   c.actor_acts = actor_acts; c.actor_logits = actor_logits;
+  c.start_idx = tl_roll_start_idx; c.feat_idx = tl_roll_feat_idx;
+  tl_roll_start_idx = nullptr; tl_roll_feat_idx = nullptr;
+  if (c.C == 0) c.start_idx = c.feat_idx = nullptr;
+  DM_REQUIRE(!c.feat_idx || c.start_idx, DM_E_NULL, "dream_rollout: feat_idx needs start_idx (its first M rows are a copy)");
   DmTwinScope tw((s->flags & DM_FLAG_BF16) != 0);
   DM_TRY(c.plan(ws, ws_bytes));
   tl_last_schedule[2] = (c.wzt ? DM_SCHED_ROLL_WZT : 0) | (c.wat ? DM_SCHED_ROLL_WAT : 0) | (c.actor_wpack ? DM_SCHED_ROLL_ACTOR_WPACK : 0) |
                         (c.actor_add0 ? DM_SCHED_ROLL_ACTOR_ADD0 : 0) | (c.fuse_act ? DM_SCHED_ROLL_FUSE_ACT : 0) |
-                        (c.tw_on ? DM_SCHED_ROLL_TW_ON : 0);
+                        (c.tw_on ? DM_SCHED_ROLL_TW_ON : 0) | (c.actor_add0 && c.start_idx ? DM_SCHED_ROLL_ADD0_IDX0 : 0) |
+                        (c.feat_idx ? DM_SCHED_ROLL_KEEP_IDX : 0);
   const float* const* p = c.p;
   const int H = c.H, D = c.D, Hd = c.Hd, Z = c.Z, ZP = c.ZP, F = c.F;
   hipStream_t st = c.st;
@@ -900,6 +916,10 @@
   if (c.actor_wpack) DM_TRY(dm_mlp_chain_pack_launch(F, c.L, actor, c.actor_wpack, st, c.actor_w0t ? D : 0));
   hipError_t e = hipMemcpyAsync(feats, start, (size_t)M * F * sizeof(float), hipMemcpyDeviceToDevice, st);
   if (e != hipSuccess) return dm_fail(DM_E_HIP, "dream_rollout: %s", hipGetErrorString(e));
+  if (c.feat_idx) {
+    e = hipMemcpyAsync(c.feat_idx, c.start_idx, (size_t)M * c.S * sizeof(int32_t), hipMemcpyDeviceToDevice, st);
+    if (e != hipSuccess) return dm_fail(DM_E_HIP, "dream_rollout: %s", hipGetErrorString(e));
+  }
   for (int i = 0; i < H; ++i) {
     DM_TRY(c.rollout_actor(i));
     DM_TRY(c.rollout_cell(i));
diff --git a/pydreamer_amd/hip.py b/pydreamer_amd/hip.py
--- a/pydreamer_amd/hip.py
+++ b/pydreamer_amd/hip.py
@@ -35,7 +35,8 @@
 SCHED_FWD = {'fuse_ln': 1, 'fuse_sample': 2, 'frag': 4, 'wzt': 8, 'psync': 16}
 SCHED_BWD = {'fuse_b': 1, 'fold': 2, 'fold_sm': 4, 'frag': 8}
 SCHED_BWD_NCHUNK_SHIFT = 8
-SCHED_ROLL = {'wzt': 1, 'wat': 2, 'actor_wpack': 4, 'actor_add0': 8, 'fuse_act': 16, 'tw_on': 32}
+SCHED_ROLL = {'wzt': 1, 'wat': 2, 'actor_wpack': 4, 'actor_add0': 8, 'fuse_act': 16, 'tw_on': 32, 'add0_idx0': 64,
+              'keep_idx': 128}
 DM_MAX_GRU_LAYERS = 4
 
 
@@ -233,6 +234,10 @@
     'dm_dream_rollout_marks': (c_int, [c_int, POINTER(c_int), POINTER(c_void_p)]),
     'dm_mlp_head_fwd_rows': (c_int, [c_int, c_int, c_int, c_int, c_int, c_int, c_int, c_int, _P, c_int, POINTER(dm_mlp_params), _P, _P, _P,
                                      c_size_t, _P]),
+    'dm_dream_rollout_indices': (c_int, [_P, _P]),
+    'dm_mlp_head_fwd_rows_idx': (c_int, [c_int, c_int, c_int, c_int, c_int, c_int, _P, c_int, c_int, c_int, _P, c_int,
+                                         POINTER(dm_mlp_params), _P, _P, _P, c_size_t, _P]),
+    'dm_onehot_heads_enable': (c_int, [c_int]),
     'dm_replay_gather': (c_int, [c_int, c_int, c_int, POINTER(dm_replay_field), _P, _P, _P]),
     'dm_gru_sequence_acts_floats': (c_size_t, [c_int, c_int, c_int, c_int]),
     'dm_gru_sequence_ws_bytes': (c_size_t, [c_int, c_int, c_int, c_int]),
diff --git a/pydreamer_amd/models.py b/pydreamer_amd/models.py
--- a/pydreamer_amd/models.py
+++ b/pydreamer_amd/models.py
@@ -110,7 +110,7 @@
     def acts_floats(self, rows):
         return int(H.lib().dm_mlp_acts_floats(rows, self.hidden_dim, self.hidden_layers))
 
-    def fwd(self, x2d, ldx, rows, ws, acts=None, save_acts=True, sparse_cols=0, window=None, out=None):
+    def fwd(self, x2d, ldx, rows, ws, acts=None, save_acts=True, sparse_cols=0, window=None, out=None, idx=None):
         need = 4 * int(H.lib().dm_mlp_ws_floats(rows, self.hidden_dim, self.hidden_layers))
         if ws.numel() < need:
             raise H.DreamerHipError(f'MLP.fwd: workspace of {ws.numel()} bytes, need {need} for {rows} rows')
@@ -118,6 +118,13 @@
             rows_total, row0 = window
             assert out is not None and out.shape[0] == rows_total and (acts is not None or not save_acts)
             st = self.struct()
+            if idx is not None and 0 < sparse_cols < self.in_dim:
+                S = idx.shape[-1]
+                assert idx.dtype == torch.int32 and idx.numel() == rows_total * S and sparse_cols % S == 0
+                H.call('dm_mlp_head_fwd_rows_idx', rows_total, row0, rows, self.in_dim, S, sparse_cols // S, H.ptr(idx),
+                       self.hidden_dim, self.hidden_layers, self.out_dim, H.fptr(x2d), ldx, ctypes.byref(st),
+                       H.fptr(acts) if save_acts else None, H.fptr(out), H.ptr(ws), ws.numel(), H.stream())
+                return out, acts
             H.call('dm_mlp_head_fwd_rows', rows_total, row0, rows, self.in_dim, sparse_cols if 0 < sparse_cols < self.in_dim else 0,
                    self.hidden_dim, self.hidden_layers, self.out_dim, H.fptr(x2d), ldx, ctypes.byref(st),
                    H.fptr(acts) if save_acts else None, H.fptr(out), H.ptr(ws), ws.numel(), H.stream())
@@ -664,10 +671,10 @@
     def dream_buffers(self, rows, device):
         return [torch.empty(rows, head.model.out_dim, device=device) for _, head, _ in self.heads()[:2]]
 
-    def dream_fwd(self, feat, row0, n, ws, bufs):
+    def dream_fwd(self, feat, row0, n, ws, bufs, idx=None):
         for (_, head, _), out in zip(self.heads()[:2], bufs):
             head.model.fwd(feat, self.features_dim, n, ws, save_acts=False, sparse_cols=self.sparse_cols, window=(out.shape[0], row0),
-                           out=out)
+                           out=out, idx=idx)
 
     def dream_means(self, bufs):
         return self.terminal.loss(bufs[1])[2], self.reward.loss(bufs[0])[2]
@@ -1833,16 +1840,17 @@
                         logits=torch.empty(rows, self.critic_bins, device=device))
         return bufs
 
-    def value(self, feats, F_, rows, ws, target=False, window=None, out=None, acts=None, save_acts=False, sparse=True, logits=None):
+    def value(self, feats, F_, rows, ws, target=False, window=None, out=None, acts=None, save_acts=False, sparse=True, logits=None,
+              idx=None):
         mlp = self.critic_target if target else self.critic
         sp = self.sparse_cols if sparse else 0
         if self.critic_dist == 'mse':
-            return mlp.fwd(feats, F_, rows, ws, acts=acts, save_acts=save_acts, sparse_cols=sp, window=window, out=out)
+            return mlp.fwd(feats, F_, rows, ws, acts=acts, save_acts=save_acts, sparse_cols=sp, window=window, out=out, idx=idx)
         K = self.critic_bins
         if window is not None:
             rows_total, row0 = window
             assert logits is not None and tuple(logits.shape) == (rows_total, K) and out is not None
-            mlp.fwd(feats, F_, rows, ws, acts=acts, save_acts=save_acts, sparse_cols=sp, window=window, out=logits)
+            mlp.fwd(feats, F_, rows, ws, acts=acts, save_acts=save_acts, sparse_cols=sp, window=window, out=logits, idx=idx)
             lg, v = logits[row0:row0 + rows], out[row0:row0 + rows]
         else:
             lg, acts = mlp.fwd(feats, F_, rows, ws, acts=acts, save_acts=save_acts, sparse_cols=sp)
@@ -1850,10 +1858,11 @@
         H.call('dm_twohot_decode', rows, K, H.fptr(lg), K, H.fptr(self.bins), H.fptr(v), H.stream())
         return out, acts
 
-    def forward_values(self, feats, F_, rows_total, row0, rows, ws, bufs):
+    def forward_values(self, feats, F_, rows_total, row0, rows, ws, bufs, idx=None):
         w = (rows_total, row0)
-        self.value(feats, F_, rows, ws, target=True, window=w, out=bufs['value_t'], logits=bufs.get('logits_t'))
-        self.value(feats, F_, rows, ws, window=w, out=bufs['value'], acts=bufs['c_acts'], save_acts=True, logits=bufs.get('logits'))
+        self.value(feats, F_, rows, ws, target=True, window=w, out=bufs['value_t'], logits=bufs.get('logits_t'), idx=idx)
+        self.value(feats, F_, rows, ws, window=w, out=bufs['value'], acts=bufs['c_acts'], save_acts=True, logits=bufs.get('logits'),
+                   idx=idx)
 
     def training_step(self, features, actions, rewards, terminals, log_only=False, act_idx=None, ws=None,
                       actor_acts=None, actor_logits=None, overlap=None, mbuf=None, values=None, _begun=False):
@@ -2176,7 +2185,7 @@
         start = torch.cat((h, z), -1).contiguous()
         return self._dream_from_features(start, Hh, u_act, u_prior, _pack)
 
-    def _dream_from_features(self, start, Hh, u_act=None, u_prior=None, _pack=None, early=None, ac=None):
+    def _dream_from_features(self, start, Hh, u_act=None, u_prior=None, _pack=None, early=None, ac=None, start_idx=None):
         c = self.conf
         ac = self.ac if ac is None else ac
         M, dev = start.shape[0], start.device
@@ -2206,6 +2215,11 @@
         r_split = ac.split_steps(Hh + 1) * M
         use_early = (early is not None and _pack is not None and r_split < rows and _HEADS_EARLY
                      and not getattr(c, 'amp', False))
+        feat_idx = None
+        if start_idx is not None and c.stoch_discrete:
+            assert start_idx.dtype == torch.int32 and tuple(start_idx.shape) == (M, S)
+            feat_idx = torch.empty(Hh + 1, M, S, dtype=torch.int32, device=dev)
+            H.call('dm_dream_rollout_indices', H.ptr(start_idx.contiguous()), H.ptr(feat_idx))
         if use_early:
             H.call('dm_dream_rollout_marks', 1, (ctypes.c_int * 1)(r_split // M - 2),
                    (ctypes.c_void_p * 1)(int(early.ev_mark.cuda_event)))
@@ -2220,9 +2234,9 @@
         def heads(a, b, wsx):
             if b <= a:
                 return
-            dec.dream_fwd(f2, a, b - a, wsx, outs)
+            dec.dream_fwd(f2, a, b - a, wsx, outs, idx=feat_idx)
             if values is not None:
-                ac.forward_values(f2, F_, rows, a, b - a, wsx, values)
+                ac.forward_values(f2, F_, rows, a, b - a, wsx, values, idx=feat_idx)
         if use_early:
             early.s_ac.wait_event(early.ev_mark)
             with torch.cuda.stream(early.s_ac):
@@ -2235,7 +2249,8 @@
             heads(r_split, rows, ws)
         term, mu = dec.dream_means(outs)
         if _pack is not None:
-            _pack.update(act_idx=act_idx, ws=ws, actor_acts=a_acts, actor_logits=a_logits, values=values, head_outs=outs)
+            _pack.update(act_idx=act_idx, ws=ws, actor_acts=a_acts, actor_logits=a_logits, values=values, head_outs=outs,
+                         feat_idx=feat_idx)
         return feats, actions, _Mean(mu.view(Hh + 1, M)), _Mean(term.view(Hh + 1, M))
 
     def training_step(self, obs, in_state, iwae_samples=None, imag_horizon=None, do_open_loop=False, do_image_pred=False,
@@ -2317,7 +2332,7 @@
         features_dream, actions_dream, rewards_dream, terminals_dream = \
             self._dream_from_features(pk['feat'], imag_horizon,
                                       noise.get('u_act') if self.ac.dist_kind == 0 else noise.get('eps_act'),
-                                      noise.get('u_prior'), _pack=dpk, early=ov)
+                                      noise.get('u_prior'), _pack=dpk, early=ov, start_idx=pk['idx'])
         (loss_actor, loss_critic), metrics_ac, tensors_ac = \
             self.ac.training_step(features_dream, actions_dream, rewards_dream.mean, terminals_dream.mean,
                                   act_idx=dpk['act_idx'], ws=dpk['ws'], actor_acts=dpk['actor_acts'],
@@ -2336,7 +2351,7 @@
                                 actions=actions_dream, dream_features=features_dream, actor_logits=dpk.get('actor_logits'),
                                 ac_tensors=tensors_ac, post=pk['post'], prior=pk['prior'], pred_idx=pk.get('pred_idx'),
                                 dream_reward=rewards_dream.mean, dream_terminal=terminals_dream.mean,
-                                dream_reward_out=dpk['head_outs'][0])
+                                dream_reward_out=dpk['head_outs'][0], dream_idx=dpk['feat_idx'])
         dream_tensors = {}
         if do_dream_tensors and not self.wm.imageless:
             with torch.no_grad():
```

Result: no change. 31.16 grad-steps/s, median of 6 (+0.4%).
